# sahhermans/vae-diffusion-toy-crystals

Measured on NVIDIA B200. Metric: samples_per_sec_64x64_sde300_cfg1.5, higher is better.
Workload: dtype bf16

## Files before the change

include/tcs.h:

```cpp
#ifndef TCS_H_
#define TCS_H_

#include <stdint.h>

#ifdef __cplusplus
extern "C" {
#endif

typedef struct tcs_handle tcs_handle;

enum tcs_status {
  TCS_OK = 0,
  TCS_ERR_BAD_ARGUMENT = -1,
  TCS_ERR_UNSUPPORTED = -2,
  TCS_ERR_CUDA = -3,
  TCS_ERR_STATE = -4
};

enum tcs_precision { TCS_FP32 = 0, TCS_BF16 = 1 };
enum tcs_engine { TCS_ENGINE_AUTO = 0, TCS_ENGINE_SIMT = 1, TCS_ENGINE_TCGEN05 = 2 };
enum tcs_sampler { TCS_SAMPLER_ODE = 0, TCS_SAMPLER_SDE = 1 };

typedef struct tcs_config {
  int32_t n_types;
// ... 2 lines not shown
  int32_t emb_dim;
  int32_t cond_ch;
  int32_t time_ch;
  double beta_min;
  double beta_max;
  int32_t precision;
  int32_t engine;
  int32_t device;
  int32_t chunk;
  int32_t use_graph;
  int32_t fuse_gn;
} tcs_config;

void tcs_default_config(tcs_config* cfg);

int tcs_create(tcs_handle** out, const tcs_config* cfg);
void tcs_destroy(tcs_handle* h);

int tcs_set_weight(tcs_handle* h, const char* key, const float* data, const int64_t* shape, int32_t ndim);

int tcs_finalize_weights(tcs_handle* h);

int tcs_score(tcs_handle* h, const float* x, const float* t, const int64_t* y_cat, const float* y_cont,
              int32_t n, float guidance, float* eps_out, void* stream);

typedef struct tcs_sample_args {
  int32_t sampler;
  int32_t n;
  int32_t steps;
  float guidance;
  double t_end;
  const int64_t* y_cat;
  const float* y_cont;
  const float* x_init;
  const float* noise;
  uint64_t seed;
  uint64_t global_index_offset;
  float* x_out;
  float* trace_eps;
  float* trace_x;
  float* x0_hat;
  double beta_min;
  double beta_max;
} tcs_sample_args;

int tcs_sample(tcs_handle* h, const tcs_sample_args* args, void* stream);

int32_t tcs_nfe(int32_t sampler, int32_t steps);

int tcs_condition_grid(tcs_handle* h, int32_t n, int64_t offset, int64_t n_total, float theta_max,
                       int64_t* y_cat, float* y_cont, void* stream);

int tcs_sde_update(tcs_handle* h, float* x, const float* eps, const float* noise, int32_t n, float t, float t_next,
                   uint64_t seed, uint64_t global_index_offset, int32_t step, void* stream);

int tcs_ode_update(tcs_handle* h, int32_t mode, float* x, float* x_pred, float* d0, const float* eps, int32_t n,
                   float t, float t_next, void* stream);

int tcs_time_grid_host(int32_t steps, double t_end, float* ts_host);
int tcs_schedule_host(double beta_min, double beta_max, float t, float* beta, float* alpha, float* sigma);

int32_t tcs_check(tcs_handle* h);
int32_t tcs_launch_mode(const tcs_handle* h);

int64_t tcs_launch_count(const tcs_handle* h);
const char* tcs_build_info(void);
const char* tcs_last_error(void);

int64_t tcs_debug_layer(tcs_handle* h, const char* name, const float* x, const float* t, const int64_t* y_cat,
                        const float* y_cont, int32_t n, int32_t uncond, float* out, int64_t out_capacity,
                        void* stream);

int tcs_score_profiled(tcs_handle* h, const float* x, const float* t, const int64_t* y_cat, const float* y_cont,
                       int32_t n, float guidance, float* eps_out, float* conv_ms_host, float* total_ms_host,
                       void* stream);

int tcs_debug_conv(int32_t engine, int32_t precision, int32_t B, int32_t H_out, int32_t W_out, int32_t cin0,
                   int32_t cin1, int32_t cout, int32_t ksize, int32_t stride, const float* in0, const float* in1,
                   const float* weight, const float* bias, float* out, float* stats, int32_t epi, void* stream);

int tcs_debug_conv_ups(int32_t B, int32_t H_out, int32_t W_out, int32_t cin, int32_t cout, const float* in_lowres,
                       const float* weight, const float* bias, float* out, void* stream);

int64_t tcs_debug_attn_pack(const float* qkv_w, const float* proj_w, uint8_t* out, int64_t capacity);

int tcs_debug_attn_block(int32_t B, const float* x, const float* gn_w, const float* gn_b, const float* qkv_w,
                         const float* qkv_b, const float* proj_w, const float* proj_b, float* out, float* dbg,
                         void* stream);

#ifdef __cplusplus
}
#endif
#endif
```

vae-diffusion-toy-crystals_b200/csrc/common.cuh:

```cuda
#pragma once
#include <cuda.h>
#include <cuda_bf16.h>
#include <cuda_fp16.h>
#include <cuda_runtime.h>
#include <stdint.h>

#include <string>
#include <vector>

#include "../../include/tcs.h"

namespace tcs {

constexpr int IMG = 64;
constexpr int IMG_PIX = IMG * IMG;
constexpr int GN_GROUPS = 8;
constexpr float GN_EPS = 1e-5f;
constexpr int N_HEADS = 4;

void set_error(const std::string& msg);
int fail(int code, const std::string& msg);

#define TCS_CUDA(expr)                                                                          \
  do {                                                                                          \
    cudaError_t _e = (expr);                                                                    \
    if (_e != cudaSuccess)                                                                      \
      return ::tcs::fail(TCS_ERR_CUDA, std::string(#expr) + ": " + cudaGetErrorString(_e));     \
  } while (0)

#define TCS_CHECK(expr)                    \
  do {                                     \
    int _s = (expr);                       \
    if (_s != TCS_OK) return _s;           \
  } while (0)

enum Epilogue : int {
  EPI_RAW_STATS = 0,
  EPI_PADDED = 1,
  EPI_PLAIN = 2,
  EPI_GN_FUSED = 3,
  EPI_EPS = 4
};

struct ConvGeom {
  int B;
  int H, W;
  int ksize;
  int stride;
  int nsrc;
  int csrc[2];
  int in_pad[2];
  int ntot;
  int split3 = 0;
  int ups = 0;
  int kx_in_n = 0;
};

struct EpiArgs {
  const float* bias;
  void* out;
  float* partials;
  const void* residual;
  int ldo;
  int slots;
  const float* gamma;
  const float* beta;
  int* overflow;
};

struct DevBuf {
  void* p = nullptr;
  size_t bytes = 0;
  uint64_t* gen = nullptr;
  DevBuf() = default;
  DevBuf(const DevBuf&) = delete;
  DevBuf& operator=(const DevBuf&) = delete;
  ~DevBuf() { if (p) cudaFree(p); }
  int ensure(size_t b) {
    if (b <= bytes) return TCS_OK;
    if (p) cudaFree(p);
    p = nullptr; bytes = 0;
    TCS_CUDA(cudaMalloc(&p, b));
    bytes = b;
    if (gen) ++*gen;
    return TCS_OK;
  }
  template <typename U> U* as() const { return static_cast<U*>(p); }
};

struct HostTensor { std::vector<float> v; std::vector<int64_t> shape; };

inline int tc_slots(int H, int W) { return (H * W / 128) * 4; }
inline int simt_slots(int H, int W) { return H * W / 64; }

}
```

vae-diffusion-toy-crystals_b200/csrc/conv_tc.cu:

```cuda
#include "conv_tc.cuh"
#include "tc_ptx.cuh"

#include <cstdio>
#include <cstdlib>
#include <cstring>
#include <type_traits>
#include <vector>

#ifndef TCS_KERNEL_PROFILE
#define TCS_KERNEL_PROFILE 0
#endif

namespace tcs {


constexpr int EPI_WARPS = 16;
constexpr int GRP_WARPS = EPI_WARPS / 2;
constexpr int UC = 96;
constexpr int BLK = 32;
constexpr int TC_THREADS = 64 + 32 * EPI_WARPS + 32;
constexpr int UPS_EXTRA_THREADS = 4 * 32;
constexpr int MAX_STAGES = 12;
constexpr int MAX_A_STAGES = 4;
constexpr int KB = 64;
constexpr uint32_t ROWB = KB * 2;
constexpr int SLAB_BUFS = 2;
constexpr uint32_t EPI_WARP_SLAB = SLAB_BUFS * 32 * BLK * 2;
constexpr uint32_t EPI_SLAB_BYTES = EPI_WARPS * EPI_WARP_SLAB;
constexpr uint32_t EPI_BIAS_BYTES = 576 * 4;
constexpr size_t TC_SMEM_MAX = 227 * 1024 - 512;
__host__ __device__ constexpr uint32_t bias_bytes_of(int ntot) { return (static_cast<uint32_t>(ntot) * 4u + 127u) & ~127u; }
struct EpiGroupSmem {
  float scale[192], shift[192];
  float red[GRP_WARPS][16];
  float mean[8], rstd[8];
};
struct EpiFusedSmem {
  float gamma[192], beta[192];
  EpiGroupSmem grp[2];
};
constexpr uint32_t EPI_FUSED_BYTES = sizeof(EpiFusedSmem);
constexpr long long EXCHANGE_TIMEOUT_CYCLES = 1000000000LL;

__device__ __forceinline__ void st_relaxed_gpu_u64(unsigned long long* p, unsigned long long v) {
  asm volatile("st.relaxed.gpu.global.b64 [%0], %1;" ::"l"(p), "l"(v) : "memory");
}
__device__ __forceinline__ unsigned long long ld_relaxed_gpu_u64(const unsigned long long* p) {
  unsigned long long v;
  asm volatile("ld.relaxed.gpu.global.b64 %0, [%1];" : "=l"(v) : "l"(p) : "memory");
  return v;
}
__device__ __forceinline__ void epi_bar_sync(int grp) { asm volatile("bar.sync %0, %1;" ::"r"(1 + grp), "n"(32 * GRP_WARPS) : "memory"); }
__device__ __forceinline__ uint32_t pack_f16x2_sat(float a, float b) {
  uint32_t r;
  asm("cvt.rn.satfinite.f16x2.f32 %0, %1, %2;" : "=r"(r) : "f"(b), "f"(a));
  return r;
}
__device__ __forceinline__ float2 unpack_f16x2(uint32_t v) {
  return __half22float2(*reinterpret_cast<const __half2*>(&v));
}
__device__ __forceinline__ uint32_t pack_bf16x2(float a, float b) {
  const __nv_bfloat162 h = __floats2bfloat162_rn(a, b);
  return *reinterpret_cast<const uint32_t*>(&h);
}
__device__ __forceinline__ float silu_fast(float y) {
  const float h = 0.5f * y;
  float t;
  asm("tanh.approx.f32 %0, %1;" : "=f"(t) : "f"(h));
  return fmaf(h, t, h);
}
__device__ __forceinline__ void store_with_halo(__nv_bfloat16* obase, size_t pix, int wy, int wx, int Wp, int ldo,
                                                int ch, const uint32_t* pk);

__device__ __forceinline__ void fma2(float& d0, float& d1, float a0, float a1, float b0, float b1, float c0, float c1) {
  asm("{\n\t.reg .b64 ra, rb, rc, rd;\n\tmov.b64 ra, {%2, %3};\n\tmov.b64 rb, {%4, %5};\n\tmov.b64 rc, {%6, %7};\n\t"
      "fma.rn.f32x2 rd, ra, rb, rc;\n\tmov.b64 {%0, %1}, rd;\n\t}"
      : "=f"(d0), "=f"(d1) : "f"(a0), "f"(a1), "f"(b0), "f"(b1), "f"(c0), "f"(c1));
}
__device__ __forceinline__ void add2(float& d0, float& d1, float a0, float a1, float b0, float b1) {
  asm("{\n\t.reg .b64 ra, rb, rd;\n\tmov.b64 ra, {%2, %3};\n\tmov.b64 rb, {%4, %5};\n\t"
      "add.rn.f32x2 rd, ra, rb;\n\tmov.b64 {%0, %1}, rd;\n\t}"
      : "=f"(d0), "=f"(d1) : "f"(a0), "f"(a1), "f"(b0), "f"(b1));
}
__device__ __forceinline__ float tanh_fast(float x) {
#ifdef TCS_NO_TANH
  return x * 0.25f;
#else
  float t;
  asm("tanh.approx.f32 %0, %1;" : "=f"(t) : "f"(x));
  return t;
#endif
}
__device__ __forceinline__ void st_shared_u4(uint32_t addr, uint32_t a, uint32_t b, uint32_t c, uint32_t d) {
  asm volatile("st.shared.v4.b32 [%0], {%1, %2, %3, %4};" ::"r"(addr), "r"(a), "r"(b), "r"(c), "r"(d) : "memory");
}
__device__ __forceinline__ void ld_shared_u4(uint32_t addr, uint32_t& a, uint32_t& b, uint32_t& c, uint32_t& d) {
  asm volatile("ld.shared.v4.b32 {%0, %1, %2, %3}, [%4];" : "=r"(a), "=r"(b), "=r"(c), "=r"(d) : "r"(addr) : "memory");
}
__device__ __forceinline__ void tma_store_4d(const CUtensorMap* map, uint32_t src, int c0, int c1, int c2, int c3) {
  asm volatile("cp.async.bulk.tensor.4d.global.shared::cta.bulk_group [%0, {%2, %3, %4, %5}], [%1];"
               ::"l"(reinterpret_cast<uint64_t>(map)), "r"(src), "r"(c0), "r"(c1), "r"(c2), "r"(c3)
               : "memory");
}
template <int GEO = 0, int SB = SLAB_BUFS>
// ... 9 lines not shown
  long long c0 = tacc ? clock64() : 0;
  if (lane == 0) ptx::bulk_wait_read<SB - 1>();
  __syncwarp();
  if (tacc) { const long long c1 = clock64(); tacc[0] += c1 - c0; c0 = c1; }
  const uint32_t base = slab + (SB == 2 ? slab_buf * 2048 : 0);
  const uint32_t dst = base + lane * 64;
  const int sw = (lane >> 1) & 3;
#pragma unroll
  for (int j = 0; j < 4; ++j) st_shared_u4(dst + ((j ^ sw) << 4), pk[4 * j], pk[4 * j + 1], pk[4 * j + 2], pk[4 * j + 3]);
  ptx::fence_proxy_async();
  __syncwarp();
  if (tacc) { const long long c1 = clock64(); tacc[1] += c1 - c0; c0 = c1; }
  if (lane == 0) {
    if (GEO == 1) {
      tma_store_4d(mapO, base, ch, x + 1, y + 1, img);
      if (y == 0) tma_store_4d(mapO1, base, ch, x + 1, geo_H + 1, img);
      if (y + 4 == geo_H) tma_store_4d(mapO1, base + 3 * 512, ch, x + 1, 0, img);
    } else if (h16 == 0) {
      tma_store_4d(mapO, base, ch, x + 1, y + 1, img);
      if (wy) tma_store_4d(mapO, base, ch, x + 1, y + 1 + wy, img);
    } else {
      tma_store_4d(mapO, base, ch, 1, y + 1, img);
      tma_store_4d(mapO, base + 1024, ch, 1, y + 2, img);
      if (y == 0) tma_store_4d(mapO, base, ch, 1, h16 + 1, img);
      if (y + 1 == h16 - 1) tma_store_4d(mapO, base + 1024, ch, 1, 0, img);
    }
    ptx::bulk_commit();
  }
  __syncwarp();
  if (tacc) { const long long c1 = clock64(); tacc[2] += c1 - c0; c0 = c1; }
  slab_buf ^= 1;
  if (wx) {
    uint4* d0 = reinterpret_cast<uint4*>(obase + (pix + wx) * ldo + ch);
#pragma unroll
    for (int i = 0; i < 4; ++i) d0[i] = make_uint4(pk[4 * i], pk[4 * i + 1], pk[4 * i + 2], pk[4 * i + 3]);
    if (wy) {
      uint4* d1 = reinterpret_cast<uint4*>(obase + (pix + static_cast<long long>(wy) * Wp + wx) * ldo + ch);
#pragma unroll
      for (int i = 0; i < 4; ++i) d1[i] = make_uint4(pk[4 * i], pk[4 * i + 1], pk[4 * i + 2], pk[4 * i + 3]);
    }
  }
}

__device__ __forceinline__ void store_with_halo(__nv_bfloat16* obase, size_t pix, int wy, int wx, int Wp, int ldo,
                                                int ch, const uint32_t* pk) {
#pragma unroll
  for (int cy = 0; cy < 2; ++cy) {
    if (cy == 1 && wy == 0) continue;
#pragma unroll
    for (int cx = 0; cx < 2; ++cx) {
      if (cx == 1 && wx == 0) continue;
      const size_t dp = pix + static_cast<long long>(cy ? wy : 0) * Wp + (cx ? wx : 0);
      uint4* dst = reinterpret_cast<uint4*>(obase + dp * ldo + ch);
#pragma unroll
      for (int i = 0; i < BLK / 8; ++i) dst[i] = make_uint4(pk[4 * i], pk[4 * i + 1], pk[4 * i + 2], pk[4 * i + 3]);
    }
  }
}

template <int CG>
__device__ __forceinline__ void tile_to_mn(int tile, int n_ntiles, int& mt, int& nt) {
  if (CG == 2) {
    const int pt = tile >> 1;
    nt = pt % n_ntiles;
    mt = ((pt / n_ntiles) << 1) | (tile & 1);
  } else {
    mt = tile / n_ntiles;
    nt = tile - mt * n_ntiles;
  }
}

struct __align__(8) TcBarriers {
  uint64_t full[MAX_STAGES];
  uint64_t empty[MAX_STAGES];
  uint64_t fullA[MAX_A_STAGES];
  uint64_t emptyA[MAX_A_STAGES];
  uint64_t fullL[2];
  uint64_t emptyL[2];
  uint64_t tmem_full[2];
  uint64_t tmem_empty[2];
  uint32_t tmem_base;
};

template <int N, int EPI, int MSUB, int CG, int GEO, int UPS = 0>
__global__ void __launch_bounds__(TC_THREADS + UPS_EXTRA_THREADS * UPS, 1)
conv_tc_kernel(const __grid_constant__ CUtensorMap mapA0, const __grid_constant__ CUtensorMap mapA1,
               const __grid_constant__ CUtensorMap mapA2, const __grid_constant__ CUtensorMap mapA3,
               const __grid_constant__ CUtensorMap mapW, const __grid_constant__ CUtensorMap mapO,
               const __grid_constant__ CUtensorMap mapO1, const ConvTcParams p) {
  static_assert(GEO == 0 || (EPI != EPI_EPS && EPI != EPI_PLAIN), "tap-shift geometry: padded / fp32 outputs only");
  static_assert(UPS == 0 || (GEO == 1 && CG == 2 && EPI == EPI_PADDED), "fused upsample: tap-shift CTA pairs, padded output");
  constexpr int ACC_STRIDE = (N * MSUB <= 128) ? 128 : 256;
  static_assert(N * MSUB <= 256, "accumulator does not fit a double-buffered TMEM stage");

  extern __shared__ uint8_t smem_raw[];
  __shared__ TcBarriers bars;

  const int warp = __shfl_sync(0xffffffffu, threadIdx.x >> 5, 0);
  const int lane = threadIdx.x & 31;
  const uint32_t smem_base = (ptx::smem_u32(smem_raw) + 1023u) & ~1023u;
  const int n_tiles = p.n_mtiles * p.n_ntiles;
  const uint32_t l_ring = smem_base + (GEO == 1 ? p.a_stages * p.a_bytes : 0u);
  const uint32_t b_ring = l_ring + (UPS ? p.l_stages * p.l_bytes : 0u);
  const uint32_t slab_base = b_ring + p.nstage * p.stage_bytes;
  constexpr int SB = UPS ? 1 : SLAB_BUFS;
  constexpr uint32_t WARP_SLAB = SB * 32 * BLK * 2, SLAB_BYTES = EPI_WARPS * WARP_SLAB;
  float* bias_s = reinterpret_cast<float*>(smem_raw + (slab_base - ptx::smem_u32(smem_raw)) + SLAB_BYTES);
  for (int i = threadIdx.x; i < p.ntot; i += blockDim.x) {
    float b = p.epi.bias[i];
    if constexpr (EPI == EPI_GN_FUSED) {
      constexpr int CPGN = N / 8;
      const int g0 = i - i % CPGN;
      float k = 0.f;
#pragma unroll
      for (int j = 0; j < CPGN; ++j) k += p.epi.bias[g0 + j];
      b -= k * (1.0f / CPGN);
    }
    bias_s[i] = b;
  }
  EpiFusedSmem* fs = reinterpret_cast<EpiFusedSmem*>(reinterpret_cast<uint8_t*>(bias_s) + (GEO == 1 ? bias_bytes_of(p.ntot) : EPI_BIAS_BYTES));
  if constexpr (EPI == EPI_GN_FUSED)
    for (int i = threadIdx.x; i < N; i += blockDim.x) { fs->gamma[i] = p.epi.gamma[i]; fs->beta[i] = p.epi.beta[i]; }

  if (warp == 0 && lane == 0) {
    ptx::prefetch_tmap(&mapA0);
    ptx::prefetch_tmap(&mapA1);
    if (p.nsrc > 2) { ptx::prefetch_tmap(&mapA2); ptx::prefetch_tmap(&mapA3); }
    ptx::prefetch_tmap(&mapW);
    if (EPI != EPI_EPS) ptx::prefetch_tmap(&mapO);
    if (GEO == 1) ptx::prefetch_tmap(&mapO1);
    for (int s = 0; s < p.nstage; ++s) {
      ptx::mbar_init(ptx::smem_u32(&bars.full[s]), 1);
      ptx::mbar_init(ptx::smem_u32(&bars.empty[s]), p.issuers);
    }
    if (GEO == 1)
      for (int s = 0; s < p.a_stages; ++s) {
        ptx::mbar_init(ptx::smem_u32(&bars.fullA[s]), UPS ? 4 * CG : 1);
        ptx::mbar_init(ptx::smem_u32(&bars.emptyA[s]), p.issuers);
      }
    if (UPS)
      for (int s = 0; s < p.l_stages; ++s) {
        ptx::mbar_init(ptx::smem_u32(&bars.fullL[s]), 1);
        ptx::mbar_init(ptx::smem_u32(&bars.emptyL[s]), 4);
      }
    for (int a = 0; a < 2; ++a) {
      ptx::mbar_init(ptx::smem_u32(&bars.tmem_full[a]), p.issuers);
      ptx::mbar_init(ptx::smem_u32(&bars.tmem_empty[a]), GRP_WARPS * CG);
    }
    ptx::fence_barrier_init();
  }
  const uint32_t cta_rank = (CG == 2) ? ptx::cluster_ctarank() : 0u;
  constexpr int NB = N / CG;
  if (warp == 1) {
    if (CG == 2) ptx::tmem_alloc_512_2sm(ptx::smem_u32(&bars.tmem_base));
    else ptx::tmem_alloc_512(ptx::smem_u32(&bars.tmem_base));
  }
  ptx::tc_fence_before();
  __syncthreads();
  if (CG == 2) ptx::cluster_sync_all();
  ptx::tc_fence_after();
  const uint32_t tmem_base = bars.tmem_base;

  if (warp == 0 && GEO == 1) {
    uint32_t sa = 0, pa = 0, sb = 0, pb = 0;
    const int b_stages_per_kx = 3 / p.tb;
    const int b_rows_full = 3 * NB / 4;
    for (int tile = blockIdx.x; tile < n_tiles; tile += gridDim.x) {
      int mt, nt;
      tile_to_mn<CG>(tile, p.n_ntiles, mt, nt);
      const int b = mt / p.tiles_per_img, t = mt - b * p.tiles_per_img;
      const int ty = t / p.tiles_x, tx = t - ty * p.tiles_x;
      int ks = 0;
      for (int src = 0; src < p.nsrc; ++src) {
        const int ms = p.msel[src];
        const CUtensorMap* mapA = ms == 0 ? &mapA0 : (ms == 1 ? &mapA1 : (ms == 2 ? &mapA2 : &mapA3));
        for (int cb = 0; cb < p.cblk[src]; ++cb) {
          if constexpr (UPS) {
            auto issue_low = [&](int tl, int cbx) {
              int mt2, nt2;
              tile_to_mn<CG>(tl, p.n_ntiles, mt2, nt2);
              const int b2 = mt2 / p.tiles_per_img, t2 = mt2 - b2 * p.tiles_per_img;
              const int ty2 = t2 / p.tiles_x, tx2 = t2 - ty2 * p.tiles_x;
              ptx::mbar_wait(ptx::smem_u32(&bars.emptyL[sa]), pa ^ 1);
              if (lane == 0) {
                const uint32_t full = ptx::smem_u32(&bars.fullL[sa]);
                ptx::mbar_expect_tx(full, p.l_load_bytes);
                ptx::tma_load_4d(l_ring + sa * p.l_bytes, mapA, full, cbx * KB, tx2 * 4 * MSUB + p.base_off[0], ty2 * 8 + p.base_off[0], b2);
              }
              __syncwarp();
              if (++sa == static_cast<uint32_t>(p.l_stages)) { sa = 0; pa ^= 1; }
            };
            if (tile == static_cast<int>(blockIdx.x) && cb == 0) issue_low(tile, 0);
            int ntile = tile, ncb = cb + 1;
            if (ncb == p.cblk[0]) { ncb = 0; ntile = tile + static_cast<int>(gridDim.x); }
            if (ntile < n_tiles) issue_low(ntile, ncb);
          } else {
          ptx::mbar_wait(ptx::smem_u32(&bars.emptyA[sa]), pa ^ 1);
          const bool stale = (p.debug & 8) && (pa || tile != static_cast<int>(blockIdx.x));
          if (lane == 0) {
            const uint32_t full = ptx::smem_u32(&bars.fullA[sa]);
            const uint32_t a_dst = smem_base + sa * p.a_bytes;
            if (stale) {
              if (CG == 1 || cta_rank == 0) ptx::mbar_arrive(full);
            } else if (CG == 2) {
              if (cta_rank == 0) ptx::mbar_expect_tx(full, 2 * p.a_load_bytes);
              ptx::tma_load_4d_2sm(a_dst, mapA, full, cb * KB, tx * 8 * MSUB + p.base_off[src], ty * 16 + p.base_off[src], b);
            } else {
              ptx::mbar_expect_tx(full, p.a_load_bytes);
              ptx::tma_load_4d(a_dst, mapA, full, cb * KB, tx * 8 * MSUB + p.base_off[src], ty * 16 + p.base_off[src], b);
            }
          }
          __syncwarp();
          if (++sa == static_cast<uint32_t>(p.a_stages)) { sa = 0; pa ^= 1; }
          }
          for (int kx = 0; kx < 3; ++kx, ++ks)
            for (int jb = 0; jb < b_stages_per_kx; ++jb) {
              ptx::mbar_wait(ptx::smem_u32(&bars.empty[sb]), pb ^ 1);
              const bool stale_b = (p.debug & 8) && (pb || tile != static_cast<int>(blockIdx.x));
              if (lane == 0) {
                const uint32_t full = ptx::smem_u32(&bars.full[sb]);
                const uint32_t b_dst = b_ring + sb * p.stage_bytes;
                const int row0 = ((ks * p.n_ntiles + nt) * CG + static_cast<int>(cta_rank)) * b_rows_full + jb * p.b_rows;
                if (stale_b) {
                  if (CG == 1 || cta_rank == 0) ptx::mbar_arrive(full);
                } else if (CG == 2) {
                  if (cta_rank == 0) ptx::mbar_expect_tx(full, 2 * p.tb * NB * ROWB);
                  ptx::tma_load_2d_2sm(b_dst, &mapW, full, 0, row0);
                } else {
                  ptx::mbar_expect_tx(full, p.tb * NB * ROWB);
                  ptx::tma_load_2d(b_dst, &mapW, full, 0, row0);
                }
              }
              __syncwarp();
              if (++sb == static_cast<uint32_t>(p.nstage)) { sb = 0; pb ^= 1; }
            }
        }
      }
    }
  } else if (warp == 0) {
    uint32_t stage = 0, phase = 0;
    for (int tile = blockIdx.x; tile < n_tiles; tile += gridDim.x) {
      int mt, nt;
      tile_to_mn<CG>(tile, p.n_ntiles, mt, nt);
      const int rows_per_tile = p.pair ? p.Rt : p.Rt * MSUB;
      const int b = (mt / p.tiles_per_img) * (p.pair ? 2 : 1);
      const int y0 = (mt % p.tiles_per_img) * rows_per_tile;
      int ks = 0;
      for (int src = 0; src < p.nsrc; ++src) {
        const int ms = p.msel[src];
        const CUtensorMap* mapA = ms == 0 ? &mapA0 : (ms == 1 ? &mapA1 : (ms == 2 ? &mapA2 : &mapA3));
        for (int cb = 0; cb < p.cblk[src]; ++cb)
          for (int kyg = 0; kyg < p.KYG; ++kyg)
            for (int kx = 0; kx < p.KW; ++kx, ++ks) {
              ptx::mbar_wait(ptx::smem_u32(&bars.empty[stage]), phase ^ 1);
              if ((p.debug & 8) && (phase || tile != static_cast<int>(blockIdx.x))) {
                if (lane == 0 && (CG == 1 || cta_rank == 0)) ptx::mbar_arrive(ptx::smem_u32(&bars.full[stage]));
                __syncwarp();
                if (++stage == static_cast<uint32_t>(p.nstage)) { stage = 0; phase ^= 1; }
                continue;
              }
              if (lane == 0) {
                const uint32_t full = ptx::smem_u32(&bars.full[stage]);
                const uint32_t a_dst = smem_base + stage * p.stage_bytes;
                const uint32_t b_dst = a_dst + p.a_bytes;
                if (CG == 2) {
                  if (cta_rank == 0) ptx::mbar_expect_tx(full, 2 * (p.a_bytes + p.T * NB * ROWB));
                  ptx::tma_load_4d_2sm(a_dst, mapA, full, cb * KB, kx + p.kxn + p.base_off[src],
                                       p.stride * y0 + kyg + p.base_off[src], b);
                  if (p.pair)
                    ptx::tma_load_4d_2sm(a_dst + p.a_bytes / 2, mapA, full, cb * KB, kx + p.kxn + p.base_off[src],
                                         p.stride * y0 + kyg + p.base_off[src], b + 1);
                  ptx::tma_load_2d_2sm(b_dst, &mapW, full, 0,
                                       ((ks * p.n_ntiles + nt) * 2 + static_cast<int>(cta_rank)) * p.b_rows);
                } else {
                  ptx::mbar_expect_tx(full, p.a_bytes + p.T * N * ROWB);
                  ptx::tma_load_4d(a_dst, mapA, full, cb * KB, kx + p.kxn + p.base_off[src],
                                   p.stride * y0 + kyg + p.base_off[src], b);
                  if (p.pair)
                    ptx::tma_load_4d(a_dst + p.a_bytes / 2, mapA, full, cb * KB, kx + p.kxn + p.base_off[src],
                                     p.stride * y0 + kyg + p.base_off[src], b + 1);
                  ptx::tma_load_2d(b_dst, &mapW, full, 0, (ks * p.n_ntiles + nt) * p.b_rows);
                }
              }
              __syncwarp();
              if (++stage == static_cast<uint32_t>(p.nstage)) { stage = 0; phase ^= 1; }
            }
      }
    }
  } else if ((warp == 1 || (warp == 2 + EPI_WARPS && p.issuers == 2)) && cta_rank == 0) {
    constexpr uint32_t idesc = make_idesc(128 * CG, N);
    if constexpr (GEO == 1) {
      auto run1 = [&](auto sub_lo_c, auto sub_hi_c) {
        constexpr int SUB_LO = decltype(sub_lo_c)::value, SUB_HI = decltype(sub_hi_c)::value;
        uint32_t sa = 0, pa = 0, sb = 0, pb = 0, acc = 0, acc_phase = 0;
        const int b_stages_per_kx = 3 / p.tb;
        const uint32_t ky_inc = static_cast<uint32_t>(p.P) * (ROWB >> 4);
        int nblk = 0;
        for (int src = 0; src < p.nsrc; ++src) nblk += p.cblk[src];
        for (int tile = blockIdx.x; tile < n_tiles; tile += gridDim.x) {
          ptx::mbar_wait(ptx::smem_u32(&bars.tmem_empty[acc]), acc_phase ^ 1);
          ptx::tc_fence_after();
          const uint32_t d_tmem = tmem_base + acc * ACC_STRIDE;
          int blk = 0;
          for (int src = 0; src < p.nsrc; ++src)
            for (int cb = 0; cb < p.cblk[src]; ++cb, ++blk) {
              const int ksteps = (cb == p.cblk[src] - 1 && p.ctail[src]) ? 2 : 4;
              if (UPS) ptx::mbar_wait_cluster(ptx::smem_u32(&bars.fullA[sa]), pa);
              else ptx::mbar_wait(ptx::smem_u32(&bars.fullA[sa]), pa);
              const uint64_t adesc = make_desc_sw128_sbo(smem_base + sa * p.a_bytes, static_cast<uint32_t>(p.P) * ROWB) +
                                     static_cast<uint64_t>(SUB_LO * 8 * (ROWB >> 4));
              for (int kx = 0; kx < 3; ++kx)
                for (int jb = 0; jb < b_stages_per_kx; ++jb) {
                  ptx::mbar_wait(ptx::smem_u32(&bars.full[sb]), pb);
                  ptx::tc_fence_after();
                  if (lane == 0) {
                    uint64_t bdj = make_desc_sw128(b_ring + sb * p.stage_bytes);
                    uint64_t adj = adesc + static_cast<uint64_t>(kx * (ROWB >> 4) + jb * p.tb * ky_inc);
                    for (int j = 0; j < p.tb; ++j) {
                      uint64_t ad = adj;
#pragma unroll
                      for (int sub = SUB_LO; sub < SUB_HI; ++sub) {
                        const uint32_t first = (blk | kx | jb | j) != 0 ? 1u : 0u;
                        if (CG == 2) {
                          ptx::umma_bf16_2sm(d_tmem + sub * N, ad, bdj, idesc, first);
                          ptx::umma_bf16_2sm(d_tmem + sub * N, ad + 2, bdj + 2, idesc, 1u);
                          if (ksteps == 4) {
                            ptx::umma_bf16_2sm(d_tmem + sub * N, ad + 4, bdj + 4, idesc, 1u);
                            ptx::umma_bf16_2sm(d_tmem + sub * N, ad + 6, bdj + 6, idesc, 1u);
                          }
                        } else {
                          ptx::umma_bf16(d_tmem + sub * N, ad, bdj, idesc, first);
                          ptx::umma_bf16(d_tmem + sub * N, ad + 2, bdj + 2, idesc, 1u);
                          if (ksteps == 4) {
                            ptx::umma_bf16(d_tmem + sub * N, ad + 4, bdj + 4, idesc, 1u);
                            ptx::umma_bf16(d_tmem + sub * N, ad + 6, bdj + 6, idesc, 1u);
                          }
                        }
                        ad += 8 * (ROWB >> 4);
                      }
                      adj += ky_inc;
                      bdj += (NB * ROWB) >> 4;
                    }
                    const bool last_of_blk = kx == 2 && jb == b_stages_per_kx - 1;
                    if (CG == 2) {
                      ptx::umma_commit_2sm(ptx::smem_u32(&bars.empty[sb]));
                      if (last_of_blk) ptx::umma_commit_2sm(ptx::smem_u32(&bars.emptyA[sa]));
                      if (last_of_blk && blk == nblk - 1) ptx::umma_commit_2sm(ptx::smem_u32(&bars.tmem_full[acc]));
                    } else {
                      ptx::umma_commit(ptx::smem_u32(&bars.empty[sb]));
                      if (last_of_blk) ptx::umma_commit(ptx::smem_u32(&bars.emptyA[sa]));
                      if (last_of_blk && blk == nblk - 1) ptx::umma_commit(ptx::smem_u32(&bars.tmem_full[acc]));
                    }
                  }
                  __syncwarp();
                  if (++sb == static_cast<uint32_t>(p.nstage)) { sb = 0; pb ^= 1; }
                }
              if (++sa == static_cast<uint32_t>(p.a_stages)) { sa = 0; pa ^= 1; }
            }
          if (++acc == 2) { acc = 0; acc_phase ^= 1; }
        }
      };
      using J0 = std::integral_constant<int, 0>;
      using J1 = std::integral_constant<int, 1>;
      using JM = std::integral_constant<int, MSUB>;
      using JL = std::integral_constant<int, MSUB - 1>;
      if (p.issuers == 2) {
        if (warp == 1) run1(J0{}, J1{});
        else run1(JL{}, JM{});
      } else {
        run1(J0{}, JM{});
      }
    } else {
    const uint32_t row_shift = p.W * ROWB;
    const uint32_t sub_stride = p.pair ? p.a_bytes / 2 : p.Rt * row_shift;
    const uint32_t a_inc_j = row_shift >> 4, a_inc_sub = sub_stride >> 4;
    auto run = [&](auto sub_lo_c, auto sub_hi_c) {
      constexpr int SUB_LO = decltype(sub_lo_c)::value, SUB_HI = decltype(sub_hi_c)::value;
      uint32_t stage = 0, phase = 0, acc = 0, acc_phase = 0;
      const bool prof = TCS_KERNEL_PROFILE && (p.debug & 128) && blockIdx.x == 0 && warp == 1;
      long long w_empty = 0, w_full = 0, t_begin = prof ? clock64() : 0;
      int ntile = 0;
      const int stages_per_cb = p.KYG * p.KW;
      for (int tile = blockIdx.x; tile < n_tiles; tile += gridDim.x) {
        long long c0 = prof ? clock64() : 0;
        ptx::mbar_wait(ptx::smem_u32(&bars.tmem_empty[acc]), acc_phase ^ 1);
        ptx::tc_fence_after();
        if (prof) { w_empty += clock64() - c0; ++ntile; }
        int ks = 0;
        for (int src = 0; src < p.nsrc; ++src)
          for (int cb = 0; cb < p.cblk[src]; ++cb) {
// ... 55 lines not shown
    using I0 = std::integral_constant<int, 0>;
    using I1 = std::integral_constant<int, 1>;
    using IM = std::integral_constant<int, MSUB>;
    using IL = std::integral_constant<int, MSUB - 1>;
    if (p.issuers == 2) {
      if (warp == 1) run(I0{}, I1{});
      else run(IL{}, IM{});
    } else {
      run(I0{}, IM{});
    }
    }
  } else if (UPS && warp >= 3 + EPI_WARPS) {
    if constexpr (UPS) {
      constexpr int P = 8 * MSUB + 2, CW = P / 2, LP = CW + 1;
      const int t128 = (warp - (3 + EPI_WARPS)) * 32 + lane;
      uint32_t sa = 0, pa = 0, sl = 0, pl = 0;
      auto blend_cell = [&](uint32_t lbase, uint32_t abase, uint32_t k, int cm, int cn, float wy0, float wy1, float wx0, float wx1) {
        const uint32_t pa = lbase + (cm * LP + cn) * 128 + (k << 4);
        uint32_t a[4], bq[4], c[4], d[4];
        ld_shared_u4(pa, a[0], a[1], a[2], a[3]);
        ld_shared_u4(pa + 128, bq[0], bq[1], bq[2], bq[3]);
        ld_shared_u4(pa + LP * 128, c[0], c[1], c[2], c[3]);
        ld_shared_u4(pa + LP * 128 + 128, d[0], d[1], d[2], d[3]);
        uint32_t o00[4], o01[4], o10[4], o11[4];
#pragma unroll
        for (int w = 0; w < 4; ++w) {
          const float al = __uint_as_float(a[w] << 16), ah = __uint_as_float(a[w] & 0xffff0000u);
          const float bl = __uint_as_float(bq[w] << 16), bh = __uint_as_float(bq[w] & 0xffff0000u);
          const float cl = __uint_as_float(c[w] << 16), ch = __uint_as_float(c[w] & 0xffff0000u);
          const float dl = __uint_as_float(d[w] << 16), dh = __uint_as_float(d[w] & 0xffff0000u);
          float el, eh, fl, fh, t0l, t0h, t1l, t1h, u0l, u0h, u1l, u1h, gl, gh, hl, hh, r0, r1;
          add2(el, eh, bl, bh, -al, -ah);
          add2(fl, fh, dl, dh, -cl, -ch);
          fma2(t0l, t0h, wx0, wx0, el, eh, al, ah);
          fma2(t1l, t1h, wx1, wx1, el, eh, al, ah);
          fma2(u0l, u0h, wx0, wx0, fl, fh, cl, ch);
          fma2(u1l, u1h, wx1, wx1, fl, fh, cl, ch);
          add2(gl, gh, u0l, u0h, -t0l, -t0h);
          add2(hl, hh, u1l, u1h, -t1l, -t1h);
          fma2(r0, r1, wy0, wy0, gl, gh, t0l, t0h); o00[w] = pack_bf16x2(r0, r1);
          fma2(r0, r1, wy0, wy0, hl, hh, t1l, t1h); o01[w] = pack_bf16x2(r0, r1);
          fma2(r0, r1, wy1, wy1, gl, gh, t0l, t0h); o10[w] = pack_bf16x2(r0, r1);
          fma2(r0, r1, wy1, wy1, hl, hh, t1l, t1h); o11[w] = pack_bf16x2(r0, r1);
        }
        const uint32_t q00 = (2 * cm) * P + 2 * cn, q01 = q00 + 1, q10 = q00 + P, q11 = q10 + 1;
        st_shared_u4(abase + q00 * 128 + ((k ^ (q00 & 7)) << 4), o00[0], o00[1], o00[2], o00[3]);
        st_shared_u4(abase + q01 * 128 + ((k ^ (q01 & 7)) << 4), o01[0], o01[1], o01[2], o01[3]);
        st_shared_u4(abase + q10 * 128 + ((k ^ (q10 & 7)) << 4), o10[0], o10[1], o10[2], o10[3]);
        st_shared_u4(abase + q11 * 128 + ((k ^ (q11 & 7)) << 4), o11[0], o11[1], o11[2], o11[3]);
      };
      for (int tile = blockIdx.x; tile < n_tiles; tile += gridDim.x) {
        int mt, nt;
        tile_to_mn<CG>(tile, p.n_ntiles, mt, nt);
        const int t = mt % p.tiles_per_img;
        const int ty = t / p.tiles_x, tx = t - ty * p.tiles_x;
        const int edge_r0 = ty == 0 ? 0 : -1, edge_r1 = ty == p.H / 16 - 1 ? 8 : -1;
        const int edge_c0 = tx == 0 ? 0 : -1, edge_c1 = tx == p.tiles_x - 1 ? CW - 1 : -1;
        for (int src = 0; src < p.nsrc; ++src)
          for (int cb = 0; cb < p.cblk[src]; ++cb) {
            const bool tail = cb == p.cblk[src] - 1 && p.ctail[src];
            ptx::mbar_wait_sleep(ptx::smem_u32(&bars.fullL[sl]), pl);
            ptx::mbar_wait_sleep(ptx::smem_u32(&bars.emptyA[sa]), pa ^ 1);
            const uint32_t lbase = l_ring + sl * p.l_bytes, abase = smem_base + sa * p.a_bytes;
            if (!(p.debug & 64)) {
              const uint32_t k = tail ? (t128 & 3) : (t128 & 7);
              const int slot = tail ? (t128 >> 2) : (t128 >> 3), nslot = tail ? 32 : 16;
              for (int ci = slot; ci < 9 * CW; ci += nslot) {
                const int cm = ci / CW, cn = ci - cm * CW;
                const bool ey = cm == edge_r0 || cm == edge_r1, ex = cn == edge_c0 || cn == edge_c1;
                blend_cell(lbase, abase, k, cm, cn, ey ? 0.f : 0.25f, ey ? 1.f : 0.75f, ex ? 0.f : 0.25f, ex ? 1.f : 0.75f);
              }
            }
            ptx::fence_proxy_async();
            __syncwarp();
            if (lane == 0) {
              ptx::mbar_arrive(ptx::smem_u32(&bars.emptyL[sl]));
              ptx::mbar_arrive_release_rank0(ptx::smem_u32(&bars.fullA[sa]));
            }
            if (++sl == static_cast<uint32_t>(p.l_stages)) { sl = 0; pl ^= 1; }
            if (++sa == static_cast<uint32_t>(p.a_stages)) { sa = 0; pa ^= 1; }
          }
      }
    }
  } else if (warp >= 2 && warp < 2 + EPI_WARPS) {
    const int e = warp - 2, grp = e / GRP_WARPS, ew = e % GRP_WARPS, q = warp & 3, h = ew >> 2;
    const int row = q * 32 + lane;
    const int HW = p.H * p.W;
    const int Wp = p.W + 2, Hp = p.H + 2;
    (void)Hp; (void)Wp; (void)HW;
    const uint32_t acc = grp;
    uint32_t acc_phase = 0, slab_buf = 0;
    (void)slab_buf;
    EpiGroupSmem* gsm = &fs->grp[grp];
    (void)gsm;
    const uint32_t slab = slab_base + static_cast<uint32_t>(e) * WARP_SLAB;
    const bool use_tma_out = !(p.debug & 4);
    const int h16 = p.W == 16 ? p.H : 0;
    (void)h16;
    (void)use_tma_out; (void)slab;
    const int sub = (MSUB == 2) ? h : 0;
    const int col0 = (MSUB == 2) ? 0 : h * UC;
    auto pixel_of = [&](int mt_, int& img_, int& y_, int& x_) {
      if (GEO == 1) {
        img_ = mt_ / p.tiles_per_img;
        const int t_ = mt_ - img_ * p.tiles_per_img;
        const int ty_ = t_ / p.tiles_x, tx_ = t_ - ty_ * p.tiles_x;
        y_ = ty_ * 16 + (row >> 3);
        x_ = (tx_ * MSUB + sub) * 8 + (row & 7);
      } else {
        const int m_ = (mt_ * MSUB + sub) * 128 + row;
        img_ = m_ / HW;
        const int rem_ = m_ - img_ * HW;
        y_ = rem_ / p.W;
        x_ = rem_ - y_ * p.W;
      }
    };
    uint32_t it = 0;
    const bool prof = TCS_KERNEL_PROFILE && (p.debug & 128) && blockIdx.x == 0 && e == 0;
    long long pw_full = 0, p_ld = 0, p_a = 0, p_b = 0, p_c = 0, pc0 = 0, pc1 = 0, q_post = 0, q_poll = 0, q_npoll = 0, r_math = 0;
    (void)p_ld;
    long long tacc[3] = {0, 0, 0};
    auto release_tmem = [&]() {
      ptx::tc_fence_before();
      __syncwarp();
      if (lane == 0) {
        if (CG == 2) ptx::mbar_arrive_rank0(ptx::smem_u32(&bars.tmem_empty[acc]));
        else ptx::mbar_arrive(ptx::smem_u32(&bars.tmem_empty[acc]));
      }
    };
    for (int tile = blockIdx.x + grp * gridDim.x; tile < n_tiles; tile += 2 * gridDim.x, acc_phase ^= 1, ++it) {
      int mt, nt;
      tile_to_mn<CG>(tile, p.n_ntiles, mt, nt);
      const uint32_t tbase = tmem_base + (static_cast<uint32_t>(q * 32) << 16) + acc * ACC_STRIDE;
      const uint32_t taddr = tbase + h * UC;
      if (prof) { pc1 = clock64(); if (it) p_c += pc1 - pc0; pc0 = pc1; }
      ptx::mbar_wait(ptx::smem_u32(&bars.tmem_full[acc]), acc_phase);
      ptx::tc_fence_after();
      if (prof) { pc1 = clock64(); pw_full += pc1 - pc0; pc0 = pc1; }
      if (p.debug & 16) { release_tmem(); continue; }

      if constexpr (EPI == EPI_EPS) {
        float e0 = 0.f, e1 = 0.f;
        if (h == 0) {
          if (p.kxn) {
            float a0[4], a1[4];
            ptx::tmem_ld4(tbase, a0);
            ptx::tmem_ld4(tbase + N, a1);
            ptx::tmem_ld_wait();
            release_tmem();
            float* xch = reinterpret_cast<float*>(fs) + grp * 32;
            const int qq = q;
            if (lane == 31) { xch[qq * 4 + 0] = a0[0]; xch[qq * 4 + 1] = a1[0]; }
            if (lane == 0) { xch[qq * 4 + 2] = a0[2]; xch[qq * 4 + 3] = a1[2]; }
            asm volatile("bar.sync %0, 128;" ::"r"(3 + grp) : "memory");
            float l0 = __shfl_up_sync(0xffffffffu, a0[0], 1), l1 = __shfl_up_sync(0xffffffffu, a1[0], 1);
            float r0 = __shfl_down_sync(0xffffffffu, a0[2], 1), r1 = __shfl_down_sync(0xffffffffu, a1[2], 1);
            const int pq = qq ^ 1;
            if (lane == 0) { l0 = xch[pq * 4 + 0]; l1 = xch[pq * 4 + 1]; }
            if (lane == 31) { r0 = xch[pq * 4 + 2]; r1 = xch[pq * 4 + 3]; }
            e0 = (l0 + a0[1]) + r0;
            e1 = (l1 + a1[1]) + r1;
            asm volatile("bar.sync %0, 128;" ::"r"(3 + grp) : "memory");
          } else {
            ptx::tmem_ld1(tbase, &e0);
            ptx::tmem_ld1(tbase + N, &e1);
            ptx::tmem_ld_wait();
// ... 401 lines not shown

typedef CUresult (*PFN_encodeTiled)(CUtensorMap*, CUtensorMapDataType, cuuint32_t, void*, const cuuint64_t*,
                                    const cuuint64_t*, const cuuint32_t*, const cuuint32_t*, CUtensorMapInterleave,
                                    CUtensorMapSwizzle, CUtensorMapL2promotion, CUtensorMapFloatOOBfill);

static PFN_encodeTiled get_encode() {
  static PFN_encodeTiled fn = nullptr;
  if (!fn) {
    void* p = nullptr;
    cudaDriverEntryPointQueryResult q;
    if (cudaGetDriverEntryPoint("cuTensorMapEncodeTiled", &p, cudaEnableDefault, &q) == cudaSuccess &&
        q == cudaDriverEntryPointSuccess)
      fn = reinterpret_cast<PFN_encodeTiled>(p);
  }
  return fn;
}

int conv_tc_make_pair(ConvTcPlan* pl, const void* src, int B) {
  ConvTcParams& p = pl->p;
  if (pl->epi != EPI_EPS || pl->msub != 2 || B % 2) return fail(TCS_ERR_BAD_ARGUMENT, "conv_tc_make_pair: needs the eps plan and an even batch");
  PFN_encodeTiled encode = get_encode();
  p.pair = 1;
  p.WR = p.Rt + p.T - 1;
  p.tiles_per_img = p.H / p.Rt;
  p.n_mtiles = (B / 2) * p.tiles_per_img;
  p.a_bytes = 2u * static_cast<uint32_t>(p.WR) * p.W * ROWB;
  p.stage_bytes = (p.a_bytes + p.T * (pl->N / pl->cg) * ROWB + 1023u) & ~1023u;
  const size_t budget = 227 * 1024 - 2048 - 1024 - EPI_SLAB_BYTES - EPI_BIAS_BYTES - EPI_FUSED_BYTES;
  p.nstage = static_cast<int>(budget / p.stage_bytes);
  if (p.nstage > MAX_STAGES) p.nstage = MAX_STAGES;
  pl->smem = static_cast<size_t>(p.nstage) * p.stage_bytes + 1024 + EPI_SLAB_BYTES + EPI_BIAS_BYTES + EPI_FUSED_BYTES;
  const cuuint64_t C = static_cast<cuuint64_t>(pl->cin[0]);
  const int Hin = p.H + 2, Win = p.W + 2;
  cuuint64_t dims[4] = {C, static_cast<cuuint64_t>(Win), static_cast<cuuint64_t>(Hin), static_cast<cuuint64_t>(B)};
  cuuint64_t strides[3] = {C * 2, C * 2 * Win, C * 2 * Win * Hin};
  cuuint32_t box[4] = {KB, static_cast<cuuint32_t>(p.W), static_cast<cuuint32_t>(p.WR), 1};
  cuuint32_t estr[4] = {1, 1, 1, 1};
  CUresult r = encode(&pl->mapA[0], CU_TENSOR_MAP_DATA_TYPE_BFLOAT16, 4, const_cast<void*>(src), dims, strides, box, estr,
                      CU_TENSOR_MAP_INTERLEAVE_NONE, CU_TENSOR_MAP_SWIZZLE_128B, CU_TENSOR_MAP_L2_PROMOTION_L2_256B,
                      CU_TENSOR_MAP_FLOAT_OOB_FILL_NONE);
  if (r != CUDA_SUCCESS) return fail(TCS_ERR_CUDA, "cuTensorMapEncodeTiled(A pair) failed: " + std::to_string(r));
  for (int i = 1; i < 4; ++i) pl->mapA[i] = pl->mapA[0];
  return TCS_OK;
}

int conv_tc_grid(const ConvTcPlan& pl, int B, int sm_count) {
  const int tiles = (pl.p.pair ? B / 2 : B) * pl.p.tiles_per_img * pl.p.n_ntiles;
  int grid = tiles < sm_count ? tiles : sm_count;
  if (pl.max_ctas > 0 && grid > pl.max_ctas) grid = pl.max_ctas;
  static const bool group_grid = getenv("TCS_GN_GROUP_GRID") && atoi(getenv("TCS_GN_GROUP_GRID")) == 1;
  if (pl.epi == EPI_GN_FUSED && (group_grid || grid < pl.p.tiles_per_img * 2))
    grid = grid / pl.p.tiles_per_img * pl.p.tiles_per_img;
  if (pl.cg == 2) grid &= ~1;
  return grid;
}

__global__ void coop_cluster_probe_kernel() {}
static bool coop_cluster_supported() {
  static int state = -1;
  if (state < 0) {
    cudaLaunchConfig_t cfg{};
    cfg.gridDim = dim3(2); cfg.blockDim = dim3(32); cfg.dynamicSmemBytes = 0; cfg.stream = nullptr;
    cudaLaunchAttribute at[2];
    at[0].id = cudaLaunchAttributeCooperative; at[0].val.cooperative = 1;
    at[1].id = cudaLaunchAttributeClusterDimension;
    at[1].val.clusterDim.x = 2; at[1].val.clusterDim.y = 1; at[1].val.clusterDim.z = 1;
    cfg.attrs = at; cfg.numAttrs = 2;
    cudaStreamCaptureStatus cs = cudaStreamCaptureStatusNone;
    if (cudaStreamIsCapturing(nullptr, &cs) != cudaSuccess || cs != cudaStreamCaptureStatusNone) { cudaGetLastError(); return false; }
    const cudaError_t e = cudaLaunchKernelEx(&cfg, coop_cluster_probe_kernel);
    cudaGetLastError();
    state = (e == cudaSuccess && cudaDeviceSynchronize() == cudaSuccess) ? 1 : 0;
    if (getenv("TCS_NO_COOP_CLUSTER")) state = 0;
  }
  return state == 1;
}

static int conv_tc_geo(const ConvGeom& g, int epi) {
  const char* e = getenv("TCS_GEO");
  if (e && atoi(e) == 0) return 0;
  return (g.ksize == 3 && g.stride == 1 && !g.kx_in_n && epi != EPI_EPS && epi != EPI_PLAIN && g.H % 16 == 0) ? 1 : 0;
}

template <int N, int EPI, int MSUB, int CG, int GEO, int UPS = 0>
static int set_smem_attr() {
  static bool attr_done = false;
  if (!attr_done) {
    TCS_CUDA(cudaFuncSetAttribute(conv_tc_kernel<N, EPI, MSUB, CG, GEO, UPS>, cudaFuncAttributeMaxDynamicSharedMemorySize, static_cast<int>(TC_SMEM_MAX)));
    attr_done = true;
  }
  return TCS_OK;
}

template <int N, int EPI, int MSUB, int CG, int GEO, int UPS = 0>
static int max_ctas_t(const ConvTcPlan& pl, int* out) {
  TCS_CHECK((set_smem_attr<N, EPI, MSUB, CG, GEO, UPS>()));
  auto kern = conv_tc_kernel<N, EPI, MSUB, CG, GEO, UPS>;
  if (CG == 2) {
    cudaLaunchConfig_t cfg{};
    cfg.gridDim = dim3(2); cfg.blockDim = dim3(TC_THREADS + UPS_EXTRA_THREADS * UPS); cfg.dynamicSmemBytes = pl.smem; cfg.stream = nullptr;
    cudaLaunchAttribute at[1];
    at[0].id = cudaLaunchAttributeClusterDimension;
    at[0].val.clusterDim.x = 2; at[0].val.clusterDim.y = 1; at[0].val.clusterDim.z = 1;
    cfg.attrs = at; cfg.numAttrs = 1;
    int nclusters = 0;
    TCS_CUDA(cudaOccupancyMaxActiveClusters(&nclusters, kern, &cfg));
    *out = 2 * nclusters;
  } else {
    int per_sm = 0, dev = 0, sms = 0;
    TCS_CUDA(cudaOccupancyMaxActiveBlocksPerMultiprocessor(&per_sm, kern, TC_THREADS, pl.smem));
    TCS_CUDA(cudaGetDevice(&dev));
    TCS_CUDA(cudaDeviceGetAttribute(&sms, cudaDevAttrMultiProcessorCount, dev));
    *out = per_sm * sms;
  }
  return TCS_OK;
}

template <int N, int EPI, int MSUB, int CG, int GEO, int UPS = 0>
static int launch_t(const ConvTcPlan& pl, cudaStream_t st) {
  auto kern = conv_tc_kernel<N, EPI, MSUB, CG, GEO, UPS>;
  TCS_CHECK((set_smem_attr<N, EPI, MSUB, CG, GEO, UPS>()));
  if (EPI == EPI_GN_FUSED)
    TCS_CUDA(cudaMemsetAsync(pl.p.epi.partials, 0, sizeof(unsigned long long) * 16 * pl.p.n_mtiles, st));
  cudaLaunchConfig_t cfg{};
  cfg.gridDim = dim3(pl.grid); cfg.blockDim = dim3(TC_THREADS + UPS_EXTRA_THREADS * UPS); cfg.dynamicSmemBytes = pl.smem; cfg.stream = st;
  cudaLaunchAttribute at[2];
  int na = 0;
  if (EPI == EPI_GN_FUSED && (CG == 1 || pl.coop_cluster)) {
    at[na].id = cudaLaunchAttributeCooperative;
    at[na].val.cooperative = 1;
    ++na;
  }
  if (CG == 2) {
    at[na].id = cudaLaunchAttributeClusterDimension;
    at[na].val.clusterDim.x = 2; at[na].val.clusterDim.y = 1; at[na].val.clusterDim.z = 1;
    ++na;
  }
  cfg.attrs = at; cfg.numAttrs = na;
  TCS_CUDA(cudaLaunchKernelEx(&cfg, kern, pl.mapA[0], pl.mapA[1], pl.mapA[2], pl.mapA[3], pl.mapW, pl.mapO, pl.mapO1, pl.p));
  TCS_CUDA(cudaGetLastError());
  return TCS_OK;
}

static int conv_tc_max_ctas(const ConvTcPlan& pl, int* out) {
#define TCS_TC_CASE(NN, EE, MM)                                                        \
  if (pl.geo == 0 && pl.N == NN && pl.epi == EE && pl.msub == MM) {                     \
    if (pl.cg == 2) { if constexpr (NN >= 96 || EE == EPI_EPS) return max_ctas_t<NN, EE, MM, 2, 0>(pl, out); } \
    else return max_ctas_t<NN, EE, MM, 1, 0>(pl, out);                                  \
  }
#define TCS_TC_GEO1(NN, EE, MM)                                                        \
  if (pl.geo == 1 && pl.cg == 2 && !pl.ups && pl.N == NN && pl.epi == EE && pl.msub == MM) return max_ctas_t<NN, EE, MM, 2, 1>(pl, out);
  if (pl.geo == 1 && pl.cg == 2 && pl.ups && pl.epi == EPI_PADDED && pl.N == 96 && pl.msub == 2) return max_ctas_t<96, EPI_PADDED, 2, 2, 1, 1>(pl, out);
  if (pl.geo == 1 && pl.cg == 2 && pl.ups && pl.epi == EPI_PADDED && pl.N == 192 && pl.msub == 1) return max_ctas_t<192, EPI_PADDED, 1, 2, 1, 1>(pl, out);
  TCS_TC_CASE(96, EPI_RAW_STATS, 2)
  TCS_TC_CASE(96, EPI_PADDED, 2)
  TCS_TC_CASE(96, EPI_PLAIN, 2)
  TCS_TC_CASE(96, EPI_GN_FUSED, 2)
  TCS_TC_CASE(192, EPI_RAW_STATS, 1)
  TCS_TC_CASE(192, EPI_PADDED, 1)
  TCS_TC_CASE(192, EPI_PLAIN, 1)
  TCS_TC_CASE(192, EPI_GN_FUSED, 1)
  TCS_TC_CASE(16, EPI_EPS, 2)
  TCS_TC_GEO1(96, EPI_RAW_STATS, 2)
  TCS_TC_GEO1(96, EPI_PADDED, 2)
  TCS_TC_GEO1(96, EPI_GN_FUSED, 2)
  TCS_TC_GEO1(192, EPI_RAW_STATS, 1)
  TCS_TC_GEO1(192, EPI_PADDED, 1)
  TCS_TC_GEO1(192, EPI_GN_FUSED, 1)
#undef TCS_TC_CASE
#undef TCS_TC_GEO1
  return fail(TCS_ERR_UNSUPPORTED, "conv_tc: no kernel instance for this (N, epilogue, msub)");
}

int conv_tc_launch(const ConvTcPlan& pl, cudaStream_t st) {
  if (!pl.valid) return fail(TCS_ERR_STATE, "conv_tc_launch: plan not built");
#define TCS_TC_CASE(NN, EE, MM)                                                        \
  if (pl.geo == 0 && pl.N == NN && pl.epi == EE && pl.msub == MM) {                     \
    if (pl.cg == 2) { if constexpr (NN >= 96 || EE == EPI_EPS) return launch_t<NN, EE, MM, 2, 0>(pl, st); } \
    else return launch_t<NN, EE, MM, 1, 0>(pl, st);                                     \
  }
#define TCS_TC_GEO1(NN, EE, MM)                                                        \
  if (pl.geo == 1 && pl.cg == 2 && !pl.ups && pl.N == NN && pl.epi == EE && pl.msub == MM) return launch_t<NN, EE, MM, 2, 1>(pl, st);
  if (pl.geo == 1 && pl.cg == 2 && pl.ups && pl.epi == EPI_PADDED && pl.N == 96 && pl.msub == 2) return launch_t<96, EPI_PADDED, 2, 2, 1, 1>(pl, st);
  if (pl.geo == 1 && pl.cg == 2 && pl.ups && pl.epi == EPI_PADDED && pl.N == 192 && pl.msub == 1) return launch_t<192, EPI_PADDED, 1, 2, 1, 1>(pl, st);
  TCS_TC_CASE(96, EPI_RAW_STATS, 2)
  TCS_TC_CASE(96, EPI_PADDED, 2)
  TCS_TC_CASE(96, EPI_PLAIN, 2)
  TCS_TC_CASE(96, EPI_GN_FUSED, 2)
  TCS_TC_CASE(192, EPI_RAW_STATS, 1)
  TCS_TC_CASE(192, EPI_PADDED, 1)
  TCS_TC_CASE(192, EPI_PLAIN, 1)
  TCS_TC_CASE(192, EPI_GN_FUSED, 1)
  TCS_TC_CASE(16, EPI_EPS, 2)
  TCS_TC_GEO1(96, EPI_RAW_STATS, 2)
  TCS_TC_GEO1(96, EPI_PADDED, 2)
  TCS_TC_GEO1(96, EPI_GN_FUSED, 2)
  TCS_TC_GEO1(192, EPI_RAW_STATS, 1)
  TCS_TC_GEO1(192, EPI_PADDED, 1)
  TCS_TC_GEO1(192, EPI_GN_FUSED, 1)
#undef TCS_TC_CASE
#undef TCS_TC_GEO1
  return fail(TCS_ERR_UNSUPPORTED, "conv_tc_launch: no kernel instance for this (N, epilogue, msub)");
}

int conv_tc_make_plan(ConvTcPlan* plan, const ConvGeom& g, const void* src0, const void* src1,
                      const __nv_bfloat16* wpacked, int epi, const EpiArgs& ea, int sm_count, const void* lo0,
                      const void* lo1) {
  PFN_encodeTiled encode = get_encode();
  if (!encode) return fail(TCS_ERR_CUDA, "cuTensorMapEncodeTiled entry point not available");
  if (g.W != 64 && g.W != 32 && g.W != 16) return fail(TCS_ERR_UNSUPPORTED, "conv_tc: output width must be 64/32/16");
  if ((g.H * g.W) % 128) return fail(TCS_ERR_UNSUPPORTED, "conv_tc: image must be a multiple of 128 pixels");
  ConvTcPlan& pl = *plan;
  pl = ConvTcPlan();
  ConvTcParams& p = pl.p;
  conv_tc_tile_shape(g, epi, &pl.N, &pl.cg);
  if (g.ntot % pl.N) return fail(TCS_ERR_UNSUPPORTED, "conv_tc: C_out must be a multiple of 96");
  pl.epi = epi;
  pl.msub = pl.N == 192 ? 1 : 2;
  if (epi == EPI_EPS && pl.cg == 2 && (g.B * (g.H / (2 * (128 / g.W)))) % 2)
    return fail(TCS_ERR_UNSUPPORTED, "conv_tc: the output conv runs as CTA pairs and needs an even number of tiles");
  if (g.H % (pl.msub * (128 / g.W))) return fail(TCS_ERR_UNSUPPORTED, "conv_tc: image height not a multiple of the tile");
  p.debug = getenv("TCS_DEBUG") ? atoi(getenv("TCS_DEBUG")) : 0;
  p.gn_inv_cnt = 1.0 / (static_cast<double>(g.H) * g.W * (pl.N / 8));
  p.exch_timeout = getenv("TCS_EXCHANGE_TIMEOUT") ? atoll(getenv("TCS_EXCHANGE_TIMEOUT")) : EXCHANGE_TIMEOUT_CYCLES;
  {
    const char* e = getenv("TCS_ISSUERS");
    p.issuers = (pl.msub == 2 && !(e && atoi(e) == 1)) ? 2 : 1;
  }
  stage_shape(g, &p.T, &p.KYG, &p.KW);
  p.H = g.H; p.W = g.W; p.Rt = 128 / g.W;
  p.stride = g.stride;
  p.pair = 0;
  p.kxn = g.kx_in_n ? 1 : 0;
  p.guidance = 0.f;
  p.WR = p.Rt * pl.msub + p.T - 1;
  p.nsrc = g.nsrc * (g.split3 ? 3 : 1);
  pl.cin[0] = g.csrc[0]; pl.cin[1] = g.csrc[g.nsrc > 1 ? 1 : 0];
  if (g.split3 && (!lo0 || (g.nsrc == 2 && !lo1))) return fail(TCS_ERR_BAD_ARGUMENT, "conv_tc: bf16x3 mode needs the lo parts of its sources");
  if (g.split3 && epi != EPI_RAW_STATS) return fail(TCS_ERR_UNSUPPORTED, "conv_tc: bf16x3 mode writes fp32 (EPI_RAW_STATS) only");
  p.ntot = g.ntot;
  p.tiles_per_img = g.H / (p.Rt * pl.msub);
  p.n_mtiles = g.B * p.tiles_per_img;
  p.n_ntiles = g.ntot / pl.N;
  p.kstages = conv_tc_kstages(g);
  p.a_bytes = static_cast<uint32_t>(p.WR) * g.W * ROWB;
  p.stage_bytes = (p.a_bytes + p.T * (pl.N / pl.cg) * ROWB + 1023u) & ~1023u;
  const size_t budget = 227 * 1024 - 2048 - 1024 - EPI_SLAB_BYTES - EPI_BIAS_BYTES - EPI_FUSED_BYTES;
  p.nstage = static_cast<int>(budget / p.stage_bytes);
  if (p.nstage > MAX_STAGES) p.nstage = MAX_STAGES;
  pl.geo = (pl.cg == 2) ? conv_tc_geo(g, epi) : 0;
  if (!pl.geo && p.nstage < 2) return fail(TCS_ERR_UNSUPPORTED, "conv_tc: stage does not fit shared memory twice");
  pl.smem = static_cast<size_t>(p.nstage) * p.stage_bytes + 1024 + EPI_SLAB_BYTES + EPI_BIAS_BYTES + EPI_FUSED_BYTES;
  p.geo = pl.geo;
  p.P = p.tiles_x = p.a_stages = p.tb = 0;
  p.a_load_bytes = 0;
  p.ups = p.l_stages = 0;
  p.l_bytes = p.l_load_bytes = 0;
  if (pl.geo) {
    if (g.W % (8 * pl.msub) || g.H % 16) return fail(TCS_ERR_UNSUPPORTED, "conv_tc: image is not a multiple of the 16 x 8 tile");
    const int NB = pl.N / pl.cg;
    p.P = 8 * pl.msub + 2;
    p.tiles_x = g.W / (8 * pl.msub);
    p.WR = 18;
    p.tiles_per_img = (g.H / 16) * p.tiles_x;
    p.n_mtiles = g.B * p.tiles_per_img;
    p.a_load_bytes = static_cast<uint32_t>(p.WR) * p.P * ROWB;
    p.a_bytes = (p.a_load_bytes + 1023u) & ~1023u;
    p.a_stages = 2;
    if (g.ups) {
      p.ups = pl.ups = 1;
      p.l_stages = 2;
      p.l_load_bytes = 10u * static_cast<uint32_t>(p.P / 2 + 1) * ROWB;
      p.l_bytes = (p.l_load_bytes + 1023u) & ~1023u;
    }
    const size_t slab_bytes = g.ups ? EPI_SLAB_BYTES / SLAB_BUFS : EPI_SLAB_BYTES;
    const size_t budget1 = TC_SMEM_MAX - 1024 - slab_bytes - bias_bytes_of(g.ntot) - EPI_FUSED_BYTES -
                           static_cast<size_t>(p.l_stages) * p.l_bytes;
    const bool want3 = getenv("TCS_UPS_A_STAGES") ? atoi(getenv("TCS_UPS_A_STAGES")) == 3 : pl.msub == 2;
    if (g.ups && want3 && budget1 >= 3 * static_cast<size_t>(p.a_bytes) + 2 * static_cast<size_t>(3u * NB * ROWB))
      p.a_stages = 3;
    const size_t rest = budget1 - static_cast<size_t>(p.a_stages) * p.a_bytes;
    p.tb = (rest / (3u * NB * ROWB) >= (g.ups ? 2u : 3u)) ? 3 : 1;
    if (getenv("TCS_TB")) p.tb = atoi(getenv("TCS_TB")) == 3 ? 3 : 1;
    p.stage_bytes = (static_cast<uint32_t>(p.tb) * NB * ROWB + 1023u) & ~1023u;
    p.nstage = static_cast<int>(rest / p.stage_bytes);
    if (p.nstage > MAX_STAGES) p.nstage = MAX_STAGES;
    if (getenv("TCS_NSTAGE") && atoi(getenv("TCS_NSTAGE")) < p.nstage) p.nstage = atoi(getenv("TCS_NSTAGE"));
    if (getenv("TCS_PLAN_LOG")) fprintf(stderr, "[conv_tc plan] H=%d N=%d K=%d ups=%d tb=%d nstage=%d stage_bytes=%u a_bytes=%u l_bytes=%u\n", g.H, pl.N, p.kstages, p.ups, p.tb, p.nstage, p.stage_bytes, p.a_bytes, p.l_bytes);
    if (p.nstage < 2) return fail(TCS_ERR_UNSUPPORTED, "conv_tc: weight stage does not fit shared memory twice");
    pl.smem = static_cast<size_t>(p.a_stages) * p.a_bytes + static_cast<size_t>(p.l_stages) * p.l_bytes +
              static_cast<size_t>(p.nstage) * p.stage_bytes + 1024 + slab_bytes + bias_bytes_of(g.ntot) + EPI_FUSED_BYTES;
  }
  if (g.ups && !(pl.geo == 1 && pl.cg == 2 && epi == EPI_PADDED && g.nsrc == 1 && !g.split3))
    return fail(TCS_ERR_UNSUPPORTED, "conv_tc: the fused upsample needs a 3x3 stride-1 layer with one padded bf16 source and a padded output");
  p.epi = ea;
  TCS_CHECK(conv_tc_max_ctas(pl, &pl.max_ctas));
  if (getenv("TCS_MAX_CTAS")) pl.max_ctas = atoi(getenv("TCS_MAX_CTAS"));
  pl.coop_cluster = pl.cg == 2 && epi == EPI_GN_FUSED && coop_cluster_supported();
  pl.grid = conv_tc_grid(pl, g.B, sm_count);
  if (epi == EPI_GN_FUSED && (p.n_ntiles != 1 || pl.grid < p.tiles_per_img))
    return fail(TCS_ERR_UNSUPPORTED,
                "conv_tc: fused GroupNorm needs one N tile and a whole image group (" + std::to_string(p.tiles_per_img) +
                    " CTAs) resident at once; the device can hold " + std::to_string(pl.max_ctas));

  const void* srcs[4] = {src0, src1, src0, src1};
  int lsrc[4] = {0, 1, 0, 1};
  if (g.split3) {
    srcs[0] = src0; srcs[1] = lo0; srcs[2] = src1; srcs[3] = lo1;
    lsrc[0] = lsrc[1] = 0; lsrc[2] = lsrc[3] = 1;
  }
  for (int ps = 0; ps < 6; ++ps) {
    const int ls = g.split3 ? ps / 3 : ps;
    const int li = ls < g.nsrc ? ls : 0;
    const int conv_pad = (g.ksize == 1) ? 0 : 1;
    p.base_off[ps] = g.in_pad[li] - conv_pad;
    if (p.base_off[ps] < 0) return fail(TCS_ERR_BAD_ARGUMENT, "conv_tc: a 3x3/4x4 conv needs a padded source");
    p.cblk[ps] = (g.csrc[li] + KB - 1) / KB;
    p.ctail[ps] = (g.csrc[li] % KB) ? 1 : 0;
    if (g.csrc[li] % 32) return fail(TCS_ERR_UNSUPPORTED, "conv_tc: source channels must be a multiple of 32");
    p.msel[ps] = g.split3 ? 2 * li + (ps % 3 == 2 ? 1 : 0) : li;
  }
  for (int s = 0; s < 4; ++s) {
    int si = lsrc[s] < g.nsrc ? lsrc[s] : 0;
    if (!srcs[s] || lsrc[s] >= g.nsrc) { srcs[s] = srcs[0]; si = 0; }
    const int pad = g.in_pad[si];
    const int Hin = g.H * g.stride + 2 * pad, Win = g.W * g.stride + 2 * pad;
    const cuuint64_t C = g.csrc[si];
    cuuint64_t dims[4] = {C, static_cast<cuuint64_t>(Win), static_cast<cuuint64_t>(Hin), static_cast<cuuint64_t>(g.B)};
    cuuint64_t strides[3] = {C * 2, C * 2 * Win, C * 2 * Win * Hin};
    cuuint32_t box[4] = {KB, static_cast<cuuint32_t>(g.W * g.stride), static_cast<cuuint32_t>(p.WR * g.stride), 1};
    cuuint32_t estr[4] = {1, static_cast<cuuint32_t>(g.stride), static_cast<cuuint32_t>(g.stride), 1};
    if (pl.geo) { box[1] = static_cast<cuuint32_t>(p.P); box[2] = static_cast<cuuint32_t>(p.WR); }
    if (pl.ups) {
      dims[1] = static_cast<cuuint64_t>(g.W / 2 + 2); dims[2] = static_cast<cuuint64_t>(g.H / 2 + 2);
      strides[1] = C * 2 * dims[1]; strides[2] = strides[1] * dims[2];
      box[1] = static_cast<cuuint32_t>(p.P / 2 + 1); box[2] = 10;
    }
    CUresult r = encode(&pl.mapA[s], CU_TENSOR_MAP_DATA_TYPE_BFLOAT16, 4, const_cast<void*>(srcs[s]), dims, strides,
                        box, estr, CU_TENSOR_MAP_INTERLEAVE_NONE, pl.ups ? CU_TENSOR_MAP_SWIZZLE_NONE : CU_TENSOR_MAP_SWIZZLE_128B,
                        CU_TENSOR_MAP_L2_PROMOTION_L2_256B, CU_TENSOR_MAP_FLOAT_OOB_FILL_NONE);
    if (r != CUDA_SUCCESS) return fail(TCS_ERR_CUDA, "cuTensorMapEncodeTiled(A) failed: " + std::to_string(r));
  }
  {
    const uint32_t stage_b = static_cast<uint32_t>(p.T) * (pl.N / pl.cg) * ROWB;
    if (stage_b % 512) return fail(TCS_ERR_UNSUPPORTED, "conv_tc: weight stage is not a multiple of 512 bytes");
    p.b_rows = static_cast<int>(stage_b / 512);
    const cuuint64_t total_rows = static_cast<cuuint64_t>(p.kstages) * p.n_ntiles * pl.cg * p.b_rows;
    if (pl.geo) p.b_rows = p.b_rows * p.tb / 3;
    cuuint64_t dims[2] = {256, total_rows};
    cuuint64_t strides[1] = {512};
    cuuint32_t box[2] = {256, static_cast<cuuint32_t>(p.b_rows)};
    cuuint32_t estr[2] = {1, 1};
    CUresult r = encode(&pl.mapW, CU_TENSOR_MAP_DATA_TYPE_BFLOAT16, 2, const_cast<__nv_bfloat16*>(wpacked), dims,
                        strides, box, estr, CU_TENSOR_MAP_INTERLEAVE_NONE, CU_TENSOR_MAP_SWIZZLE_NONE,
                        CU_TENSOR_MAP_L2_PROMOTION_L2_256B, CU_TENSOR_MAP_FLOAT_OOB_FILL_NONE);
    if (r != CUDA_SUCCESS) return fail(TCS_ERR_CUDA, "cuTensorMapEncodeTiled(W) failed: " + std::to_string(r));
  }
  pl.mapO = pl.mapW;
  pl.mapO1 = pl.mapW;
  if (epi == EPI_PLAIN) {
    const cuuint64_t C = static_cast<cuuint64_t>(ea.ldo);
    cuuint64_t dims[2] = {C, static_cast<cuuint64_t>(g.B) * g.H * g.W};
    cuuint64_t strides[1] = {C * 2};
    cuuint32_t box[2] = {BLK, 32};
    cuuint32_t estr[2] = {1, 1};
    CUresult r = encode(&pl.mapO, CU_TENSOR_MAP_DATA_TYPE_BFLOAT16, 2, ea.out, dims, strides, box, estr,
                        CU_TENSOR_MAP_INTERLEAVE_NONE, CU_TENSOR_MAP_SWIZZLE_64B, CU_TENSOR_MAP_L2_PROMOTION_L2_256B,
                        CU_TENSOR_MAP_FLOAT_OOB_FILL_NONE);
    if (r != CUDA_SUCCESS) return fail(TCS_ERR_CUDA, "cuTensorMapEncodeTiled(O plain) failed: " + std::to_string(r));
  }
  if (epi == EPI_GN_FUSED || epi == EPI_PADDED) {
    const cuuint64_t C = static_cast<cuuint64_t>(ea.ldo);
    cuuint64_t dims[4] = {C, static_cast<cuuint64_t>(g.W + 2), static_cast<cuuint64_t>(g.H + 2), static_cast<cuuint64_t>(g.B)};
    cuuint64_t strides[3] = {C * 2, C * 2 * (g.W + 2), C * 2 * (g.W + 2) * (g.H + 2)};
    cuuint32_t box[4] = {BLK, static_cast<cuuint32_t>(g.W >= 32 ? 32 : 16), 1, 1};
// ... 19 lines not shown
```

vae-diffusion-toy-crystals_b200/csrc/conv_tc.cuh:

```cuda
#pragma once
#include <vector>

#include "common.cuh"

namespace tcs {

struct ConvTcParams {
  int n_mtiles, n_ntiles;
  int tiles_per_img;
  int H, W;
  int Rt;
  int T, KYG, KW;
  int stride, WR;
  int nsrc, cblk[6], base_off[6];
  int msel[6];
  int ctail[6];
  int ntot;
  int kstages;
  int b_rows;
  int nstage;
  uint32_t a_bytes, stage_bytes;
  int pair;
  int kxn;
  float guidance;
  double gn_inv_cnt;
  long long exch_timeout;
  int issuers;
  int geo;
  int P;
  int tiles_x;
  int a_stages, tb;
  uint32_t a_load_bytes;
  int ups;
  int l_stages;
  uint32_t l_bytes, l_load_bytes;
  int debug;
  EpiArgs epi;
};

struct ConvTcPlan {
  CUtensorMap mapA[4];
  CUtensorMap mapW;
  CUtensorMap mapO;
  CUtensorMap mapO1;
  int geo = 0;
  int ups = 0;
  ConvTcParams p;
  int N;
  int epi;
  int msub;
  int cg;
  int grid;
  int cin[2] = {0, 0};
  int max_ctas = 0;
  bool coop_cluster = false;
  size_t smem;
  bool valid = false;
};

int conv_tc_kstages(const ConvGeom& g);
size_t conv_tc_packed_elems(const ConvGeom& g);
void conv_tc_pack_weights(const ConvGeom& g, int epi, const float* w, __nv_bfloat16* out_host);
void conv_tc_tile_shape(const ConvGeom& g, int epi, int* N, int* cg);

int conv_tc_make_plan(ConvTcPlan* plan, const ConvGeom& g, const void* src0, const void* src1,
                      const __nv_bfloat16* wpacked, int epi, const EpiArgs& ea, int sm_count,
                      const void* lo0 = nullptr, const void* lo1 = nullptr);
int conv_tc_launch(const ConvTcPlan& plan, cudaStream_t stream);
int conv_tc_make_pair(ConvTcPlan* plan, const void* src, int B);
int conv_tc_grid(const ConvTcPlan& plan, int B, int sm_count);

}
```

vae-diffusion-toy-crystals_b200/csrc/kernels.cuh:

```cuda
#pragma once
#include "common.cuh"

namespace tcs {

struct EmbedWeights {
  const float *cat_emb;
  const float *cm0_w, *cm0_b;
  const float *cm2_w, *cm2_b;
  const float *co_w, *co_b;
  const float *tm0_w, *tm0_b;
  const float *tm2_w, *tm2_b;
  const float *tc_w, *tc_b;
  const float *tt_w, *tt_b;
  const float *wsum;
  const float *b0;
  int n_types, y_cont_dim;
};
int launch_cond_embed(const EmbedWeights& w, const int64_t* y_cat, const float* y_cont, int n, int dup, float* cvec,
                      cudaStream_t st);
int launch_time_embed(const EmbedWeights& w, const float* t, int nt, float* tvec, cudaStream_t st);

int launch_first_conv(const float* x, const float* w9 , const float* tvec, int tvec_stride,
                      const int* step_ptr, int trow_off, const float* cvec, int n, int dup, float* raw,
                      float* partials, cudaStream_t st);
constexpr int FIRST_CONV_SLOTS = 32;
template <typename T>
int launch_first_conv_gn(const float* x, const float* w9, const float* tvec, int tvec_stride, const int* step_ptr,
                         int trow_off, const float* cvec, int n, int dup, const float* gamma, const float* beta, T* out,
                         cudaStream_t st);

template <typename T>
int launch_gn_apply(const void* in, int in_padded, const float* partials, int slots, const float* gamma,
                    const float* beta, int B, int H, int W, int C, int silu, T* out_padded, float2* stats_scratch ,
                    cudaStream_t st);
template <typename T>
int launch_gn_image16(const T* in_padded, int B, const float* gamma, const float* beta, T* out_padded, cudaStream_t st);
template <typename T>
int launch_gn_stats(const T* in_padded, int B, int H, int W, int C, float* partials, cudaStream_t st);

template <typename T>
int launch_upsample2x(const T* in, int B, int h, int w, int C, T* out, cudaStream_t st);

template <typename T>
int launch_attention(const T* qkv, int B, T* y, cudaStream_t st);

template <typename T>
int launch_conv_simt(const ConvGeom& g, const T* src0, const T* src1, const float* wpacked, int epi,
                     const EpiArgs& ea, cudaStream_t st);
void conv_simt_pack_weights(const ConvGeom& g, const float* w, float* out_host, bool round_bf16);

template <typename T>
int launch_out_conv(const T* act, const float* w , float bias, int n, int dup, float guidance,
                    float* eps, cudaStream_t st);

template <typename T>
int launch_pad_from_plain(const float* in, int B, int H, int W, int C, int pad, T* out, cudaStream_t st);
template <typename T>
int launch_unpad_to_f32(const T* in, int B, int H, int W, int C, int pad, float* out, cudaStream_t st);

int launch_split(const float* in, size_t elems, __nv_bfloat16* out, size_t lo_off, cudaStream_t st);
int launch_raw_to_padded(int mode, const float* raw, const float2* stats, const float* gamma, const float* beta,
                         const float* residual, int B, int H, int W, int C, void* out, size_t lo_off, cudaStream_t st);
int launch_unsplit_to_f32(const __nv_bfloat16* in, size_t lo_off, int B, int H, int W, int C, int pad, float* out,
                          cudaStream_t st);
int launch_gn_finalize(const float* partials, int slots, int B, int H, int W, int C, float2* stats, cudaStream_t st);

struct StepCoef {
  float t, beta, sigma, alpha, dt, g_sqrt_dt, pad0, pad1;
};
enum StepMode : int { STEP_SDE = 0, STEP_ODE_PREDICT = 1, STEP_ODE_CORRECT = 2, STEP_FINAL = 3 };
struct StepArgs {
  const StepCoef* coef;
  const int* step_ptr;
  int row_off;
  int mode;
  float* x;
  float* x_pred;
  float* d0;
  const float* eps;
  const float* noise;
  long long noise_step_stride;
  float* out_img;
  float* out_x0;
  unsigned long long seed, gidx0;
  int n;
};
int launch_step(const StepArgs& a, cudaStream_t st);
int launch_philox_normal(float* x, int n, unsigned long long seed, unsigned long long gidx0, cudaStream_t st);
int launch_advance(int* step_ptr, int delta, cudaStream_t st);
int launch_copy_f32(float* dst, const float* src, size_t n, cudaStream_t st);

}
```

vae-diffusion-toy-crystals_b200/csrc/kernels_simt.cu:

```cuda
#include "kernels.cuh"

#include <cstdlib>

namespace tcs {

template <typename T> struct Vec8;
template <> struct Vec8<float> {
  float4 a, b;
  __device__ __forceinline__ void load(const float* p) { a = *reinterpret_cast<const float4*>(p); b = *reinterpret_cast<const float4*>(p + 4); }
  __device__ __forceinline__ void store(float* p) const { *reinterpret_cast<float4*>(p) = a; *reinterpret_cast<float4*>(p + 4) = b; }
  __device__ __forceinline__ void get(float* f) const { f[0]=a.x; f[1]=a.y; f[2]=a.z; f[3]=a.w; f[4]=b.x; f[5]=b.y; f[6]=b.z; f[7]=b.w; }
  __device__ __forceinline__ void set(const float* f) { a = make_float4(f[0],f[1],f[2],f[3]); b = make_float4(f[4],f[5],f[6],f[7]); }
};
template <> struct Vec8<__nv_bfloat16> {
  uint4 u;
  __device__ __forceinline__ void load(const __nv_bfloat16* p) { u = *reinterpret_cast<const uint4*>(p); }
  __device__ __forceinline__ void store(__nv_bfloat16* p) const { *reinterpret_cast<uint4*>(p) = u; }
  __device__ __forceinline__ void get(float* f) const {
    const __nv_bfloat162* h = reinterpret_cast<const __nv_bfloat162*>(&u);
#pragma unroll
    for (int i = 0; i < 4; ++i) { const float2 t = __bfloat1622float2(h[i]); f[2*i] = t.x; f[2*i+1] = t.y; }
  }
  __device__ __forceinline__ void set(const float* f) {
    __nv_bfloat162* h = reinterpret_cast<__nv_bfloat162*>(&u);
// ... 4 lines not shown

template <typename T> __device__ __forceinline__ float to_f(T v);
template <> __device__ __forceinline__ float to_f<float>(float v) { return v; }
template <> __device__ __forceinline__ float to_f<__nv_bfloat16>(__nv_bfloat16 v) { return __bfloat162float(v); }
template <typename T> __device__ __forceinline__ T from_f(float v);
template <> __device__ __forceinline__ float from_f<float>(float v) { return v; }
template <> __device__ __forceinline__ __nv_bfloat16 from_f<__nv_bfloat16>(float v) { return __float2bfloat16(v); }

__device__ __forceinline__ int halo_wrap(int v, int n) { return v == 0 ? n : (v == n - 1 ? -n : 0); }

__global__ void __launch_bounds__(192) first_conv_kernel(const float* __restrict__ x, const float* __restrict__ w9,
                                                        const float* __restrict__ tvec, int tvec_stride,
                                                        const int* __restrict__ step_ptr, int trow_off,
                                                        const float* __restrict__ cvec, int dup,
                                                        float* __restrict__ raw, float* __restrict__ partials) {
  __shared__ float xs[4][IMG + 2];
  __shared__ float red[2][96][2][2];
  const int i = blockIdx.x >> 5, rp = blockIdx.x & 31, y0 = rp * 2;
  const int t = threadIdx.x, oc = t % 96, half = t / 96;
  for (int e = t; e < 4 * (IMG + 2); e += 192) {
    const int r = e / (IMG + 2), c = e % (IMG + 2);
    const int yy = (y0 - 1 + r + IMG) & (IMG - 1), xx = (c - 1 + IMG) & (IMG - 1);
    xs[r][c] = x[(static_cast<size_t>(i) * IMG + yy) * IMG + xx];
  }
  float w[9];
#pragma unroll
  for (int k = 0; k < 9; ++k) w[k] = w9[oc * 9 + k];
  const int trow = (step_ptr ? *step_ptr : 0) + trow_off + i * tvec_stride;
  const float tb = tvec[static_cast<size_t>(trow) * 96 + oc];
  float bias[2], s[2] = {0.f, 0.f}, q[2] = {0.f, 0.f};
  for (int u = 0; u < dup; ++u) bias[u] = tb + cvec[(static_cast<size_t>(i) * dup + u) * 96 + oc];
  __syncthreads();
  for (int p = half; p < 128; p += 2) {
    const int r = p >> 6, c = p & 63;
    float acc = 0.f;
#pragma unroll
    for (int ky = 0; ky < 3; ++ky)
#pragma unroll
      for (int kx = 0; kx < 3; ++kx) acc = fmaf(w[ky * 3 + kx], xs[r + ky][c + kx], acc);
    for (int u = 0; u < dup; ++u) {
      const float v = acc + bias[u];
      raw[((static_cast<size_t>(i) * dup + u) * IMG_PIX + (y0 + r) * IMG + c) * 96 + oc] = v;
      s[u] += v;
      q[u] += v * v;
    }
  }
  for (int u = 0; u < dup; ++u) { red[half][oc][u][0] = s[u]; red[half][oc][u][1] = q[u]; }
  __syncthreads();
  if (t < 8 * dup) {
    const int g = t % 8, u = t / 8;
    float ss = 0.f, qq = 0.f;
    for (int h = 0; h < 2; ++h)
      for (int c = 0; c < 12; ++c) { ss += red[h][g * 12 + c][u][0]; qq += red[h][g * 12 + c][u][1]; }
    float* dst = partials + ((static_cast<size_t>(i) * dup + u) * FIRST_CONV_SLOTS + rp) * 16 + 2 * g;
    dst[0] = ss;
    dst[1] = qq;
  }
}

int launch_first_conv(const float* x, const float* w9, const float* tvec, int tvec_stride, const int* step_ptr,
                      int trow_off, const float* cvec, int n, int dup, float* raw, float* partials,
                      cudaStream_t st) {
  if (n <= 0) return TCS_OK;
  first_conv_kernel<<<n * 32, 192, 0, st>>>(x, w9, tvec, tvec_stride, step_ptr, trow_off, cvec, dup, raw, partials);
  TCS_CUDA(cudaGetLastError());
  return TCS_OK;
}

template <bool FAST> __device__ __forceinline__ float silu_f(float v);

__device__ __forceinline__ float2 pk_fma2v(float2 a, float2 b, float2 c) {
  float2 d;
  asm("{\n\t.reg .b64 ra, rb, rc, rd;\n\tmov.b64 ra, {%2, %3};\n\tmov.b64 rb, {%4, %5};\n\tmov.b64 rc, {%6, %7};\n\t"
      "fma.rn.f32x2 rd, ra, rb, rc;\n\tmov.b64 {%0, %1}, rd;\n\t}"
      : "=f"(d.x), "=f"(d.y) : "f"(a.x), "f"(a.y), "f"(b.x), "f"(b.y), "f"(c.x), "f"(c.y));
  return d;
}
template <typename T> __device__ __forceinline__ void store_pair(T* p, float a, float b);
template <> __device__ __forceinline__ void store_pair<float>(float* p, float a, float b) { *reinterpret_cast<float2*>(p) = make_float2(a, b); }
template <> __device__ __forceinline__ void store_pair<__nv_bfloat16>(__nv_bfloat16* p, float a, float b) {
  *reinterpret_cast<__nv_bfloat162*>(p) = __floats2bfloat162_rn(a, b);
}

constexpr int FC_SPLIT = 2;
template <typename T>
__global__ void __launch_bounds__(384, 2) first_conv_gn_kernel(const float* __restrict__ x, const float* __restrict__ w9,
                                                           const float* __restrict__ tvec, int tvec_stride,
                                                           const int* __restrict__ step_ptr, int trow_off,
                                                           const float* __restrict__ cvec, int dup,
                                                           const float* __restrict__ gamma, const float* __restrict__ beta,
                                                           T* __restrict__ out) {
  constexpr bool FAST = sizeof(T) == 2;
  constexpr int P = IMG + 4;
  __shared__ float2 xs[P][P];
  __shared__ double racc[12][14];
  __shared__ double R[5][5];
  __shared__ double S1;
  __shared__ double csum[96][2][2];
  __shared__ float s_mean[2][GN_GROUPS], s_rstd[2][GN_GROUPS];
  const int i = blockIdx.x / FC_SPLIT, band = blockIdx.x % FC_SPLIT;
  const int t = threadIdx.x, op = t % 48, pg = t / 48, oc = 2 * op;
  const int warp = t >> 5, lane = t & 31;
  for (int e = t; e < P * P; e += 384) {
    const int r = e / P, c = e - r * P;
    const float xval = x[(static_cast<size_t>(i) * IMG + ((r - 2 + IMG) & (IMG - 1))) * IMG + ((c - 2 + IMG) & (IMG - 1))];
    xs[r][c] = make_float2(xval, xval);
  }
  __syncthreads();
  {
    double acc[14];
#pragma unroll
    for (int k = 0; k < 14; ++k) acc[k] = 0.0;
    for (int p = t; p < IMG_PIX; p += 384) {
      const int yy = (p >> 6) + 2, xx = (p & 63) + 2;
      const double x0 = xs[yy][xx].x;
      acc[13] += x0;
#pragma unroll
      for (int k = 0; k < 13; ++k) {
        const int dy = (k + 2) / 5, dx = (k + 2) % 5 - 2;
        acc[k] += x0 * static_cast<double>(xs[yy + dy][xx + dx].x);
      }
    }
#pragma unroll
    for (int k = 0; k < 14; ++k) {
#pragma unroll
      for (int o = 16; o > 0; o >>= 1) acc[k] += __shfl_xor_sync(0xffffffffu, acc[k], o);
      if (lane == 0) racc[warp][k] = acc[k];
    }
  }
  __syncthreads();
  if (t < 14) {
    double v = 0.0;
    for (int w = 0; w < 12; ++w) v += racc[w][t];
    if (t == 13) S1 = v;
    else {
      const int dy = (t + 2) / 5, dx = (t + 2) % 5 - 2;
      R[2 + dy][2 + dx] = v;
      R[2 - dy][2 - dx] = v;
    }
  }
  const int trow = (step_ptr ? *step_ptr : 0) + trow_off + i * tvec_stride;
  __syncthreads();
  if (t < 96) {
    double wk[9], A = 0.0, Q = 0.0;
#pragma unroll
    for (int k = 0; k < 9; ++k) { wk[k] = w9[t * 9 + k]; A += wk[k]; }
#pragma unroll
    for (int k = 0; k < 9; ++k)
#pragma unroll
      for (int l = 0; l < 9; ++l) Q += wk[k] * wk[l] * R[2 + k / 3 - l / 3][2 + k % 3 - l % 3];
    for (int u = 0; u < dup; ++u) {
      const double bb = static_cast<double>(tvec[static_cast<size_t>(trow) * 96 + t] + cvec[(static_cast<size_t>(i) * dup + u) * 96 + t]);
      csum[t][u][0] = A * S1 + IMG_PIX * bb;
      csum[t][u][1] = Q + 2.0 * bb * A * S1 + IMG_PIX * bb * bb;
    }
  }
  __syncthreads();
  if (t < GN_GROUPS * dup) {
    const int g = t & 7, u = t >> 3;
    double sd = 0.0, qd = 0.0;
    for (int j = 0; j < 12; ++j) { sd += csum[g * 12 + j][u][0]; qd += csum[g * 12 + j][u][1]; }
    const double cnt = static_cast<double>(IMG_PIX) * 12.0;
    const double mean = sd / cnt;
    double var = qd / cnt - mean * mean;
    var = var < 0.0 ? 0.0 : var;
    s_mean[u][g] = static_cast<float>(mean);
    s_rstd[u][g] = static_cast<float>(1.0 / sqrt(var + static_cast<double>(GN_EPS)));
  }
  float w0[9], w1[9];
#pragma unroll
  for (int k = 0; k < 9; ++k) { w0[k] = w9[oc * 9 + k]; w1[k] = w9[(oc + 1) * 9 + k]; }
  float b0[2], b1[2];
  for (int u = 0; u < 2; ++u) {
    const int uu = u < dup ? u : 0;
    b0[u] = tvec[static_cast<size_t>(trow) * 96 + oc] + cvec[(static_cast<size_t>(i) * dup + uu) * 96 + oc];
    b1[u] = tvec[static_cast<size_t>(trow) * 96 + oc + 1] + cvec[(static_cast<size_t>(i) * dup + uu) * 96 + oc + 1];
  }
  __syncthreads();
  const int g = op / 6;
  float sc0[2], sh0[2], sc1[2], sh1[2];
  {
    const float ga0 = gamma[oc], ga1 = gamma[oc + 1], be0 = beta[oc], be1 = beta[oc + 1];
#pragma unroll
    for (int u = 0; u < 2; ++u) {
      sc0[u] = s_rstd[u][g] * ga0; sh0[u] = (b0[u] - s_mean[u][g]) * sc0[u] + be0;
      sc1[u] = s_rstd[u][g] * ga1; sh1[u] = (b1[u] - s_mean[u][g]) * sc1[u] + be1;
    }
  }
  constexpr int PO = IMG + 2;
  const int p_begin = band * (IMG_PIX / FC_SPLIT), p_end = p_begin + IMG_PIX / FC_SPLIT;
  (void)p_end;
  if constexpr (FAST) {
    float2 w2[9], sc2[2], sh2[2];
#pragma unroll
    for (int k = 0; k < 9; ++k) w2[k] = make_float2(w0[k], w1[k]);
#pragma unroll
    for (int u = 0; u < 2; ++u) { sc2[u] = make_float2(0.5f * sc0[u], 0.5f * sc1[u]); sh2[u] = make_float2(0.5f * sh0[u], 0.5f * sh1[u]); }
    for (int qd = pg; qd < IMG_PIX / FC_SPLIT / 4; qd += 8) {
      const int p = p_begin + qd * 4;
      const int yy = p >> 6, xx = p & 63;
      float2 c[4];
#pragma unroll
      for (int j = 0; j < 4; ++j) c[j] = make_float2(0.f, 0.f);
#pragma unroll
      for (int ky = 0; ky < 3; ++ky) {
        float2 xv[6];
#pragma unroll
        for (int k = 0; k < 6; ++k) xv[k] = xs[yy + 1 + ky][xx + 1 + k];
#pragma unroll
        for (int kx = 0; kx < 3; ++kx)
#pragma unroll
          for (int j = 0; j < 4; ++j) c[j] = pk_fma2v(w2[ky * 3 + kx], xv[j + kx], c[j]);
      }
      T* const o_run = out + ((static_cast<size_t>(i) * dup * PO + yy + 1) * PO + xx + 1) * 96 + oc;
      constexpr long long IMG_STRIDE = static_cast<long long>(PO) * PO * 96, COL_WRAP = static_cast<long long>(IMG) * 96;
      const long long wyo = static_cast<long long>(halo_wrap(yy, IMG)) * PO * 96;
      const bool left = xx == 0, right = xx == IMG - 4;
#pragma unroll
      for (int j = 0; j < 4; ++j) {
#pragma unroll
        for (int u = 0; u < 2; ++u) {
          if (u >= dup) break;
          const float2 hh = pk_fma2v(c[j], sc2[u], sh2[u]);
          float t0, t1;
          asm("tanh.approx.f32 %0, %1;" : "=f"(t0) : "f"(hh.x));
          asm("tanh.approx.f32 %0, %1;" : "=f"(t1) : "f"(hh.y));
          const float2 yv = pk_fma2v(hh, make_float2(t0, t1), hh);
          T* const o = o_run + j * 96 + u * IMG_STRIDE;
          store_pair<T>(o, yv.x, yv.y);
          if (wyo) store_pair<T>(o + wyo, yv.x, yv.y);
          if (j == 0 && left) {
            store_pair<T>(o + COL_WRAP, yv.x, yv.y);
            if (wyo) store_pair<T>(o + wyo + COL_WRAP, yv.x, yv.y);
          }
          if (j == 3 && right) {
            store_pair<T>(o - COL_WRAP, yv.x, yv.y);
            if (wyo) store_pair<T>(o + wyo - COL_WRAP, yv.x, yv.y);
          }
        }
      }
    }
    return;
  }
  for (int qd = pg; qd < IMG_PIX / FC_SPLIT / 4; qd += 8) {
    const int p = p_begin + qd * 4;
    const int yy = p >> 6, xx = p & 63;
    float xv[3][6];
#pragma unroll
    for (int ky = 0; ky < 3; ++ky)
#pragma unroll
      for (int k = 0; k < 6; ++k) xv[ky][k] = xs[yy + 1 + ky][xx + 1 + k].x;
    float c[4][2];
#pragma unroll
    for (int j = 0; j < 4; ++j) c[j][0] = c[j][1] = 0.f;
#pragma unroll
    for (int ky = 0; ky < 3; ++ky)
#pragma unroll
      for (int kx = 0; kx < 3; ++kx)
#pragma unroll
        for (int j = 0; j < 4; ++j) {
          c[j][0] = fmaf(w0[ky * 3 + kx], xv[ky][j + kx], c[j][0]);
          c[j][1] = fmaf(w1[ky * 3 + kx], xv[ky][j + kx], c[j][1]);
        }
    const int wy = halo_wrap(yy, IMG);
#pragma unroll
    for (int j = 0; j < 4; ++j) {
      const int wx = halo_wrap(xx + j, IMG);
#pragma unroll
      for (int u = 0; u < 2; ++u) {
        if (u >= dup) break;
        const float y0 = silu_f<FAST>(fmaf(c[j][0], sc0[u], sh0[u]));
        const float y1 = silu_f<FAST>(fmaf(c[j][1], sc1[u], sh1[u]));
        const size_t base = ((static_cast<size_t>(i) * dup + u) * PO + yy + 1) * PO + xx + j + 1;
        store_pair<T>(out + base * 96 + oc, y0, y1);
        if (wy) store_pair<T>(out + (base + static_cast<long long>(wy) * PO) * 96 + oc, y0, y1);
        if (wx) store_pair<T>(out + (base + wx) * 96 + oc, y0, y1);
        if (wy && wx) store_pair<T>(out + (base + static_cast<long long>(wy) * PO + wx) * 96 + oc, y0, y1);
      }
    }
  }
}

template <typename T>
int launch_first_conv_gn(const float* x, const float* w9, const float* tvec, int tvec_stride, const int* step_ptr,
                         int trow_off, const float* cvec, int n, int dup, const float* gamma, const float* beta, T* out,
                         cudaStream_t st) {
  if (n <= 0) return TCS_OK;
  first_conv_gn_kernel<T><<<n * FC_SPLIT, 384, 0, st>>>(x, w9, tvec, tvec_stride, step_ptr, trow_off, cvec, dup, gamma,
                                                        beta, out);
  TCS_CUDA(cudaGetLastError());
  return TCS_OK;
}
template int launch_first_conv_gn<float>(const float*, const float*, const float*, int, const int*, int, const float*, int, int, const float*, const float*, float*, cudaStream_t);
template int launch_first_conv_gn<__nv_bfloat16>(const float*, const float*, const float*, int, const int*, int, const float*, int, int, const float*, const float*, __nv_bfloat16*, cudaStream_t);

__global__ void __launch_bounds__(256) gn_finalize_kernel(const float* __restrict__ partials, int slots, double count,
                                                         float2* __restrict__ stats) {
  const int b = blockIdx.x, warp = threadIdx.x >> 5, lane = threadIdx.x & 31;
  const float* part = partials + static_cast<size_t>(b) * slots * 16;
  double s = 0.0, q = 0.0;
  for (int k = lane; k < slots; k += 32) {
    s += static_cast<double>(part[k * 16 + 2 * warp]);
    q += static_cast<double>(part[k * 16 + 2 * warp + 1]);
  }
#pragma unroll
  for (int o = 16; o > 0; o >>= 1) {
    s += __shfl_xor_sync(0xffffffffu, s, o);
    q += __shfl_xor_sync(0xffffffffu, q, o);
  }
  if (lane == 0) {
    const double mean = s / count;
    double var = q / count - mean * mean;
    var = var < 0.0 ? 0.0 : var;
    stats[b * GN_GROUPS + warp] = make_float2(static_cast<float>(mean),
                                              static_cast<float>(1.0 / sqrt(var + static_cast<double>(GN_EPS))));
  }
}

template <bool FAST> __device__ __forceinline__ float silu_f(float v) {
  if constexpr (FAST) {
    const float h = 0.5f * v;
    float t;
    asm("tanh.approx.f32 %0, %1;" : "=f"(t) : "f"(h));
    return fmaf(h, t, h);
  }
  return v / (1.0f + expf(-v));
}

template <typename T, bool IN_PADDED, bool SILU>
__global__ void __launch_bounds__(256) gn_apply_kernel(const void* __restrict__ in_, const float2* __restrict__ stats,
                                                      const float* __restrict__ gamma, const float* __restrict__ beta,
                                                      int H, int W, int C, T* __restrict__ out) {
  constexpr bool FAST = sizeof(T) == 2;
  __shared__ float s_mean[GN_GROUPS], s_rstd[GN_GROUPS];
  const int b = blockIdx.y;
  if (threadIdx.x < GN_GROUPS) {
    const float2 st = stats[b * GN_GROUPS + threadIdx.x];
    s_mean[threadIdx.x] = st.x;
    s_rstd[threadIdx.x] = st.y;
  }
  __syncthreads();
  const int cv = C / 8, cpg = C / GN_GROUPS;
  const int nvec = H * W * cv;
  const int Wp = W + 2, Hp = H + 2;
  const int e0 = blockIdx.x * 1024 + threadIdx.x;
  float v[4][8];
#pragma unroll
  for (int k = 0; k < 4; ++k) {
    const int e = e0 + k * 256;
    if (e >= nvec) continue;
    const int pix = e / cv, c = (e - pix * cv) * 8;
    if constexpr (IN_PADDED) {
      const int y = pix / W, x = pix - y * W;
      Vec8<T> iv;
      iv.load(static_cast<const T*>(in_) + ((static_cast<size_t>(b) * Hp + y + 1) * Wp + x + 1) * C + c);
      iv.get(v[k]);
    } else {
      Vec8<float> iv;
      iv.load(static_cast<const float*>(in_) + (static_cast<size_t>(b) * H * W + pix) * C + c);
      iv.get(v[k]);
    }
  }
#pragma unroll
  for (int k = 0; k < 4; ++k) {
    const int e = e0 + k * 256;
    if (e >= nvec) continue;
    const int pix = e / cv, c = (e - pix * cv) * 8;
    const int y = pix / W, x = pix - y * W;
    const float4 g0 = __ldg(reinterpret_cast<const float4*>(gamma + c)), g1 = __ldg(reinterpret_cast<const float4*>(gamma + c + 4));
    const float4 b0 = __ldg(reinterpret_cast<const float4*>(beta + c)), b1 = __ldg(reinterpret_cast<const float4*>(beta + c + 4));
    const float gm[8] = {g0.x, g0.y, g0.z, g0.w, g1.x, g1.y, g1.z, g1.w};
    const float bt[8] = {b0.x, b0.y, b0.z, b0.w, b1.x, b1.y, b1.z, b1.w};
#pragma unroll
    for (int j = 0; j < 8; ++j) {
      const int g = (c + j) / cpg;
      float yv = (v[k][j] - s_mean[g]) * s_rstd[g] * gm[j] + bt[j];
      if constexpr (SILU) yv = silu_f<FAST>(yv);
// ... 751 lines not shown
```

vae-diffusion-toy-crystals_b200/csrc/tcs_api.cu:

```cuda
#include <cmath>
#include <cstdio>
#include <cstdlib>
#include <cstring>
#include <map>
#include <memory>
#include <string>
#include <vector>

#include "attn_tc.cuh"
#include "conv_tc.cuh"
#include "kernels.cuh"

namespace tcs {

static thread_local std::string g_err;
void set_error(const std::string& m) { g_err = m; }
int fail(int code, const std::string& m) {
  g_err = m;
  return code;
}

static void time_grid_host(int steps, double t_end, float* ts) {
  const int n = steps + 1;
  const float step = n > 1 ? (1.0f - 0.0f) / static_cast<float>(n - 1) : 0.f;
  const int halfway = n / 2;
  const float te = static_cast<float>(t_end);
  const float ome = static_cast<float>(1.0 - t_end);
  for (int i = 0; i < n; ++i) {
    const float u = i < halfway ? 0.0f + step * static_cast<float>(i) : 1.0f - step * static_cast<float>(n - i - 1);
    const float om = 1.0f - u;
    const float sq = om * om;
    ts[i] = te + ome * sq;
  }
}
struct Sched {
  double bmin, bmax;
  float beta(float t) const { return static_cast<float>(bmin) + t * static_cast<float>(bmax - bmin); }
  float int_beta(float t) const {
    return static_cast<float>(bmin) * t + static_cast<float>(0.5 * (bmax - bmin)) * (t * t);
  }
  float alpha(float t) const { return expf(-0.5f * int_beta(t)); }
  float sigma(float t) const {
    const float a = alpha(t);
    const float v = 1.0f - a * a;
    return sqrtf(v < 1e-8f ? 1e-8f : v);
  }
};


enum ConvId { C_D1B, C_DS1, C_D2A, C_D2B, C_DS2, C_MA, C_MB, C_QKV, C_PROJ, C_US2, C_U2A, C_U2B, C_US1, C_U1A, C_U1B, C_COUNT };
struct ConvSpec { const char* key; int cin0, cin1, cout, k, stride, res; };
static const ConvSpec kConv[C_COUNT] = {
    {"down1.net.3", 96, 0, 96, 3, 1, 64},  {"ds1", 96, 0, 96, 4, 2, 32},       {"down2.net.0", 96, 0, 192, 3, 1, 32},
    {"down2.net.3", 192, 0, 192, 3, 1, 32}, {"ds2", 192, 0, 192, 4, 2, 16},     {"mid.net.0", 192, 0, 192, 3, 1, 16},
    {"mid.net.3", 192, 0, 192, 3, 1, 16},   {"attn.qkv", 192, 0, 576, 1, 1, 16}, {"attn.proj", 192, 0, 192, 1, 1, 16},
    {"us2_conv", 192, 0, 192, 3, 1, 32},    {"up2.net.0", 192, 192, 96, 3, 1, 32}, {"up2.net.3", 96, 0, 96, 3, 1, 32},
    {"us1_conv", 96, 0, 96, 3, 1, 64},      {"up1.net.0", 96, 96, 96, 3, 1, 64}, {"up1.net.3", 96, 0, 96, 3, 1, 64}};

static ConvGeom geom_of(int id, int B, int in_pad) {
  const ConvSpec& s = kConv[id];
  ConvGeom g;
  g.B = B; g.H = g.W = s.res; g.ksize = s.k; g.stride = s.stride;
  g.nsrc = s.cin1 ? 2 : 1;
  g.csrc[0] = s.cin0; g.csrc[1] = s.cin1 ? s.cin1 : s.cin0;
  g.in_pad[0] = g.in_pad[1] = in_pad;
  g.ntot = s.cout;
  return g;
}

static const char* kTapNames[] = {
    "down1.net.0.raw", "down1.net.0.act", "down1.net.3.raw", "down1.net.3.act", "ds1",
    "down2.net.0.raw", "down2.net.0.act", "down2.net.3.raw", "down2.net.3.act", "ds2",
    "mid.net.0.raw", "mid.net.0.act", "mid.net.3.raw", "mid.net.3.act", "attn.qkv", "attn.y", "attn",
    "us2.up", "us2_conv", "up2.net.0.raw", "up2.net.0.act", "up2.net.3.raw", "up2.net.3.act",
    "us1.up", "us1_conv", "up1.net.0.raw", "up1.net.0.act", "up1.net.3.raw", "up1.net.3.act", "eps"};
constexpr int kNumTaps = sizeof(kTapNames) / sizeof(kTapNames[0]);

struct TapRequest {
  int id = -1;
  float* out = nullptr;
  int64_t capacity = 0;
  int64_t written = 0;
};

}

using namespace tcs;

struct tcs_handle {
  tcs_config cfg;
  int sm_count = 148;
  bool bf16 = false, use_tc = false, fuse_gn = false, fuse_first = true;
  bool fuse_attn = false;
  DevBuf attn_wpack;
  bool fuse_ups = false;
  ConvTcPlan plan_us[2];
  bool split3 = false;
  size_t esz = 4;
  cudaStream_t stream = nullptr;
  cudaEvent_t ev_in = nullptr, ev_out = nullptr;
  int64_t launches = 0;
  cudaEvent_t prof_ev[2 * 16] = {};
  bool profiling = false;

  std::map<std::string, HostTensor> host_w;
  bool finalized = false;
  DevBuf arena;
  std::map<std::string, const float*> dw;
  EmbedWeights ew{};
  const float *d_w9 = nullptr, *d_wout = nullptr;
  float out_bias = 0.f;
  DevBuf wpack[C_COUNT];

  int chunk = 0;
  DevBuf raw64, raw32, raw16, partials, gnstats;
  DevBuf p64_h1, p64_a, p64_b;
  DevBuf p32_96a, p32_96b, p32_192a, p32_192h2, p32_192b;
  DevBuf p16_a, p16_b, p16_c, qkv, atty;
  DevBuf split_s;
  ConvTcPlan plan[C_COUNT];
  ConvTcPlan plan_eps, plan_eps_pair;
  DevBuf wpack_out;
  const float* d_bias16 = nullptr;
  bool tc_out = false, eps_kxn = true;

  DevBuf cvec, tvec, tvals, coef, x, xpred, d0, eps, step_ctr, ycat_tmp, ycont_tmp;
  DevBuf status;
  void* pinned = nullptr; size_t pinned_bytes = 0;
  cudaEvent_t ev_pinned = nullptr;

  cudaGraphExec_t gexec = nullptr;
  uint64_t ws_gen = 0;
  struct GKey { int n = -1, dup, sampler; const void *noise, *teps, *tx; float guidance; uint64_t seed, gidx, gen; } gkey;
  int64_t graph_kernels = 0;

  tcs_handle() {
    for (DevBuf* b : {&cvec, &tvec, &tvals, &coef, &x, &xpred, &d0, &eps, &step_ctr}) b->gen = &ws_gen;
  }

  ~tcs_handle() {
    if (gexec) cudaGraphExecDestroy(gexec);
    if (pinned) cudaFreeHost(pinned);
    if (ev_in) cudaEventDestroy(ev_in);
    if (ev_out) cudaEventDestroy(ev_out);
    if (ev_pinned) cudaEventDestroy(ev_pinned);
    for (cudaEvent_t e : prof_ev) if (e) cudaEventDestroy(e);
    if (stream) cudaStreamDestroy(stream);
  }
};

namespace tcs {

static std::vector<std::pair<std::string, std::vector<int64_t>>> expected_weights(const tcs_config& c) {
  std::vector<std::pair<std::string, std::vector<int64_t>>> v;
  const int64_t e = c.emb_dim, b = c.base_ch, cin = 1 + c.cond_ch + c.time_ch;
  auto lin = [&](const std::string& k, int64_t i, int64_t o) { v.push_back({k + ".weight", {o, i}}); v.push_back({k + ".bias", {o}}); };
  auto conv = [&](const std::string& k, int64_t i, int64_t o, int64_t ks) { v.push_back({k + ".weight", {o, i, ks, ks}}); v.push_back({k + ".bias", {o}}); };
  auto gn = [&](const std::string& k, int64_t ch) { v.push_back({k + ".weight", {ch}}); v.push_back({k + ".bias", {ch}}); };
  auto block = [&](const std::string& k, int64_t i, int64_t o) { conv(k + ".net.0", i, o, 3); gn(k + ".net.1", o); conv(k + ".net.3", o, o, 3); gn(k + ".net.4", o); };
  v.push_back({"cond_emb.cat_emb.weight", {c.n_types + 1, e}});
  lin("cond_emb.cont_mlp.0", c.y_cont_dim, e); lin("cond_emb.cont_mlp.2", e, e); lin("cond_emb.out.1", 2 * e, e);
  lin("time_mlp.0", e, e); lin("time_mlp.2", e, e);
  lin("to_cond_map", e, c.cond_ch); lin("to_time_map", e, c.time_ch);
  block("down1", cin, b); conv("ds1", b, b, 4); block("down2", b, 2 * b); conv("ds2", 2 * b, 2 * b, 4);
  block("mid", 2 * b, 2 * b); gn("attn.norm", 2 * b); conv("attn.qkv", 2 * b, 6 * b, 1); conv("attn.proj", 2 * b, 2 * b, 1);
  conv("us2_conv", 2 * b, 2 * b, 3); block("up2", 4 * b, b); conv("us1_conv", b, b, 3); block("up1", 2 * b, b);
  conv("out", b, 1, 3);
  return v;
}

static int enter(tcs_handle* h, cudaStream_t user) {
  TCS_CUDA(cudaSetDevice(h->cfg.device));
  TCS_CUDA(cudaEventRecord(h->ev_in, user));
  TCS_CUDA(cudaStreamWaitEvent(h->stream, h->ev_in, 0));
  return TCS_OK;
}
static int leave(tcs_handle* h, cudaStream_t user) {
  TCS_CUDA(cudaEventRecord(h->ev_out, h->stream));
  TCS_CUDA(cudaStreamWaitEvent(user, h->ev_out, 0));
  return TCS_OK;
}

static int ensure_pinned(tcs_handle* h, size_t bytes) {
  if (h->pinned_bytes >= bytes) {
    TCS_CUDA(cudaEventSynchronize(h->ev_pinned));
    return TCS_OK;
  }
  TCS_CUDA(cudaEventSynchronize(h->ev_pinned));
  if (h->pinned) cudaFreeHost(h->pinned);
  h->pinned = nullptr; h->pinned_bytes = 0;
  TCS_CUDA(cudaMallocHost(&h->pinned, bytes));
  h->pinned_bytes = bytes;
  return TCS_OK;
}

static int alloc_workspace(tcs_handle* h) {
  const size_t MB = h->chunk, e = h->esz;
  TCS_CHECK(h->raw64.ensure(MB * 4096 * 96 * 4));
  TCS_CHECK(h->raw32.ensure(MB * 1024 * 192 * 4));
  TCS_CHECK(h->raw16.ensure(MB * 256 * 192 * 4));
  TCS_CHECK(h->partials.ensure(MB * 128 * 16 * 4));
  TCS_CHECK(h->gnstats.ensure(MB * 8 * 8));
  const size_t P64 = MB * 66 * 66 * 96 * e, P32a = MB * 34 * 34 * 96 * e, P32b = MB * 34 * 34 * 192 * e,
               P16 = MB * 18 * 18 * 192 * e;
  TCS_CHECK(h->p64_h1.ensure(P64)); TCS_CHECK(h->p64_a.ensure(P64)); TCS_CHECK(h->p64_b.ensure(P64));
  TCS_CHECK(h->p32_96a.ensure(P32a)); TCS_CHECK(h->p32_96b.ensure(P32a));
  TCS_CHECK(h->p32_192a.ensure(P32b)); TCS_CHECK(h->p32_192h2.ensure(P32b)); TCS_CHECK(h->p32_192b.ensure(P32b));
  TCS_CHECK(h->p16_a.ensure(P16)); TCS_CHECK(h->p16_b.ensure(P16)); TCS_CHECK(h->p16_c.ensure(P16));
  TCS_CHECK(h->qkv.ensure(MB * 256 * 576 * e));
  TCS_CHECK(h->atty.ensure(MB * 256 * 192 * e));
  if (h->split3) TCS_CHECK(h->split_s.ensure(P64));
  return TCS_OK;
}

struct ConvWiring { const void *s0, *s1; void* out; int epi; const void* residual; int ldo; int in_pad;
                    const char* gn; void* act; };
static ConvWiring wiring(tcs_handle* h, int id) {
  ConvWiring w{};
  switch (id) {
    case C_D1B: w = {h->p64_a.p, nullptr, h->raw64.p, EPI_RAW_STATS, nullptr, 96, 1, "down1.net.4", h->p64_h1.p}; break;
    case C_DS1: w = {h->p64_h1.p, nullptr, h->p32_96a.p, EPI_PADDED, nullptr, 96, 1, nullptr, nullptr}; break;
    case C_D2A: w = {h->p32_96a.p, nullptr, h->raw32.p, EPI_RAW_STATS, nullptr, 192, 1, "down2.net.1", h->p32_192a.p}; break;
    case C_D2B: w = {h->p32_192a.p, nullptr, h->raw32.p, EPI_RAW_STATS, nullptr, 192, 1, "down2.net.4", h->p32_192h2.p}; break;
    case C_DS2: w = {h->p32_192h2.p, nullptr, h->p16_a.p, EPI_PADDED, nullptr, 192, 1, nullptr, nullptr}; break;
    case C_MA: w = {h->p16_a.p, nullptr, h->raw16.p, EPI_RAW_STATS, nullptr, 192, 1, "mid.net.1", h->p16_b.p}; break;
    case C_MB: w = {h->p16_b.p, nullptr, h->raw16.p, EPI_RAW_STATS, nullptr, 192, 1, "mid.net.4", h->p16_a.p}; break;
    case C_QKV: w = {h->p16_b.p, nullptr, h->qkv.p, EPI_PLAIN, nullptr, 576, 1, nullptr, nullptr}; break;
    case C_PROJ: w = {h->atty.p, nullptr, h->p16_c.p, EPI_PADDED, h->p16_a.p, 192, 0, nullptr, nullptr}; break;
    case C_US2: w = {h->p32_192a.p, nullptr, h->p32_192b.p, EPI_PADDED, nullptr, 192, 1, nullptr, nullptr}; break;
    case C_U2A: w = {h->p32_192b.p, h->p32_192h2.p, h->raw32.p, EPI_RAW_STATS, nullptr, 96, 1, "up2.net.1", h->p32_96a.p}; break;
    case C_U2B: w = {h->p32_96a.p, nullptr, h->raw32.p, EPI_RAW_STATS, nullptr, 96, 1, "up2.net.4", h->p32_96b.p}; break;
    case C_US1: w = {h->p64_a.p, nullptr, h->p64_b.p, EPI_PADDED, nullptr, 96, 1, nullptr, nullptr}; break;
    case C_U1A: w = {h->p64_b.p, h->p64_h1.p, h->raw64.p, EPI_RAW_STATS, nullptr, 96, 1, "up1.net.1", h->p64_a.p}; break;
    default: w = {h->p64_a.p, nullptr, h->raw64.p, EPI_RAW_STATS, nullptr, 96, 1, "up1.net.4", h->p64_b.p}; break;
  }
  if (h->fuse_gn && w.gn) {
    w.out = w.act;
    w.epi = EPI_GN_FUSED;
  }
  return w;
}

static int slots_of(tcs_handle* h, int id) {
  const int r = kConv[id].res;
  return h->use_tc ? tc_slots(r, r) : simt_slots(r, r);
}

struct SplitSrc { const void* p; size_t lo; };
struct SplitWiring { SplitSrc s0, s1; float* raw; int ldo; int in_pad; };
static size_t padded_elems(const tcs_handle* h, int res, int C) { return static_cast<size_t>(h->chunk) * (res + 2) * (res + 2) * C; }
static SplitWiring split_wiring(tcs_handle* h, int id) {
  const SplitSrc S64{h->split_s.p, padded_elems(h, 64, 96)}, S32{h->split_s.p, padded_elems(h, 32, 192)},
      S16{h->split_s.p, padded_elems(h, 16, 192)}, SY{h->split_s.p, static_cast<size_t>(h->chunk) * 256 * 192};
  const SplitSrc h1{h->p64_h1.p, padded_elems(h, 64, 96)}, h2{h->p32_192h2.p, padded_elems(h, 32, 192)};
  const SplitSrc none{nullptr, 0};
  float *r64 = h->raw64.as<float>(), *r32 = h->raw32.as<float>(), *r16 = h->raw16.as<float>();
  switch (id) {
    case C_D1B: return {S64, none, r64, 96, 1};
    case C_DS1: return {h1, none, r32, 96, 1};
    case C_D2A: return {{h->p32_96a.p, padded_elems(h, 32, 96)}, none, r32, 192, 1};
    case C_D2B: return {{h->p32_192a.p, padded_elems(h, 32, 192)}, none, r32, 192, 1};
    case C_DS2: return {h2, none, r16, 192, 1};
    case C_MA: return {{h->p16_c.p, padded_elems(h, 16, 192)}, none, r16, 192, 1};
    case C_MB: return {{h->p16_b.p, padded_elems(h, 16, 192)}, none, r16, 192, 1};
    case C_QKV: return {S16, none, h->qkv.as<float>(), 576, 1};
    case C_PROJ: return {SY, none, r16, 192, 0};
    case C_US2: return {S32, none, r32, 192, 1};
    case C_U2A: return {{h->p32_192b.p, padded_elems(h, 32, 192)}, h2, r32, 96, 1};
    case C_U2B: return {{h->p32_96a.p, padded_elems(h, 32, 96)}, none, r32, 96, 1};
    case C_US1: return {S64, none, r64, 96, 1};
    case C_U1A: return {{h->p64_b.p, padded_elems(h, 64, 96)}, h1, r64, 96, 1};
    default: return {{h->p64_a.p, padded_elems(h, 64, 96)}, none, r64, 96, 1};
  }
}

static int build_plans(tcs_handle* h) {
  if (!h->use_tc) return TCS_OK;
  if (h->split3) {
    for (int id = 0; id < C_COUNT; ++id) {
      const SplitWiring w = split_wiring(h, id);
      ConvGeom g = geom_of(id, h->chunk, w.in_pad);
      g.split3 = 1;
      EpiArgs ea{};
      ea.bias = h->dw.at(std::string(kConv[id].key) + ".bias");
      ea.out = w.raw; ea.partials = h->partials.as<float>(); ea.ldo = w.ldo; ea.slots = slots_of(h, id);
      auto lo = [](const SplitSrc& s) { return s.p ? static_cast<const void*>(static_cast<const __nv_bfloat16*>(s.p) + s.lo) : nullptr; };
      TCS_CHECK(conv_tc_make_plan(&h->plan[id], g, w.s0.p, w.s1.p, h->wpack[id].as<__nv_bfloat16>(), EPI_RAW_STATS, ea,
                                  h->sm_count, lo(w.s0), lo(w.s1)));
    }
    return TCS_OK;
  }
  {
    const char* e = getenv("TCS_TC_OUT");
    h->tc_out = !(e && atoi(e) == 0);
    ConvGeom g = geom_of(C_U1B, h->chunk, 1);
    g.ntot = 16;
    g.kx_in_n = h->eps_kxn ? 1 : 0;
    EpiArgs ea{};
    ea.bias = h->d_bias16; ea.out = nullptr; ea.ldo = 1;
    TCS_CHECK(conv_tc_make_plan(&h->plan_eps, g, h->p64_b.p, nullptr, h->wpack_out.as<__nv_bfloat16>(), EPI_EPS, ea, h->sm_count));
    h->plan_eps_pair = h->plan_eps;
    TCS_CHECK(conv_tc_make_pair(&h->plan_eps_pair, h->p64_b.p, h->chunk));
  }
  for (int id = 0; id < C_COUNT; ++id) {
    const ConvWiring w = wiring(h, id);
    const ConvGeom g = geom_of(id, h->chunk, w.in_pad);
    EpiArgs ea{};
    ea.bias = h->dw.at(std::string(kConv[id].key) + ".bias");
    ea.out = w.out; ea.partials = h->partials.as<float>(); ea.residual = w.residual; ea.ldo = w.ldo;
    ea.slots = slots_of(h, id);
    ea.overflow = h->status.as<int>();
    if (w.epi == EPI_GN_FUSED) {
      ea.gamma = h->dw.at(std::string(w.gn) + ".weight");
      ea.beta = h->dw.at(std::string(w.gn) + ".bias");
    }
    TCS_CHECK(conv_tc_make_plan(&h->plan[id], g, w.s0, w.s1, h->wpack[id].as<__nv_bfloat16>(), w.epi, ea, h->sm_count));
  }
  if (h->fuse_ups) {
    const int ids[2] = {C_US2, C_US1};
    const void* lowres[2] = {h->p16_c.p, h->p32_96b.p};
    for (int k = 0; k < 2; ++k) {
      const ConvWiring w = wiring(h, ids[k]);
      ConvGeom g = geom_of(ids[k], h->chunk, w.in_pad);
      g.ups = 1;
      EpiArgs ea{};
      ea.bias = h->dw.at(std::string(kConv[ids[k]].key) + ".bias");
      ea.out = w.out; ea.partials = h->partials.as<float>(); ea.residual = nullptr; ea.ldo = w.ldo;
      ea.slots = slots_of(h, ids[k]);
      ea.overflow = h->status.as<int>();
      const int rc = conv_tc_make_plan(&h->plan_us[k], g, lowres[k], nullptr, h->wpack[ids[k]].as<__nv_bfloat16>(), EPI_PADDED, ea, h->sm_count);
      if (rc == TCS_ERR_UNSUPPORTED) { h->fuse_ups = false; break; }
      TCS_CHECK(rc);
    }
  }
  for (int id = 0; id < C_COUNT; ++id) {
    if (!h->plan[id].coop_cluster) continue;
    ConvTcPlan pl = h->plan[id];
    const int B = h->chunk < 16 ? h->chunk : 16;
    pl.p.n_mtiles = B * pl.p.tiles_per_img;
    pl.grid = conv_tc_grid(pl, B, h->sm_count);
    const int rc = conv_tc_launch(pl, h->stream);
    const cudaError_t se = cudaStreamSynchronize(h->stream);
    if (rc != TCS_OK || se != cudaSuccess) {
      cudaGetLastError();
      if (se != cudaSuccess && se != cudaErrorCooperativeLaunchTooLarge && se != cudaErrorInvalidValue)
        return fail(TCS_ERR_CUDA, std::string("trial launch of a fused conv failed: ") + cudaGetErrorString(se));
      for (int j = 0; j < C_COUNT; ++j) h->plan[j].coop_cluster = false;
      break;
    }
  }
  TCS_CUDA(cudaMemsetAsync(h->status.p, 0, 4, h->stream));
  return TCS_OK;
}

template <typename T>
static int run_conv_inner(tcs_handle* h, int id, int B, cudaStream_t st);

template <typename T>
static int run_conv(tcs_handle* h, int id, int B, cudaStream_t st) {
  if (!h->profiling) return run_conv_inner<T>(h, id, B, st);
  TCS_CUDA(cudaEventRecord(h->prof_ev[2 * id], st));
  TCS_CHECK(run_conv_inner<T>(h, id, B, st));
  TCS_CUDA(cudaEventRecord(h->prof_ev[2 * id + 1], st));
  return TCS_OK;
}

template <typename T>
static int run_conv_inner(tcs_handle* h, int id, int B, cudaStream_t st) {
  ++h->launches;
  if (h->use_tc) {
    ConvTcPlan pl = h->plan[id];
    pl.p.n_mtiles = B * pl.p.tiles_per_img;
    pl.grid = conv_tc_grid(pl, B, h->sm_count);
    return conv_tc_launch(pl, st);
  }
  const ConvWiring w = wiring(h, id);
  const ConvGeom g = geom_of(id, B, w.in_pad);
  EpiArgs ea{};
  ea.bias = h->dw.at(std::string(kConv[id].key) + ".bias");
  ea.out = w.out; ea.partials = h->partials.as<float>(); ea.residual = w.residual; ea.ldo = w.ldo;
  ea.slots = slots_of(h, id);
  return launch_conv_simt<T>(g, static_cast<const T*>(w.s0), static_cast<const T*>(w.s1), h->wpack[id].as<float>(),
                             w.epi, ea, st);
}

struct PassArgs {
  const float* x;
  const float* cvec;
  const float* tvec;
  int tvec_stride;
  const int* step_ptr;
  int trow_off;
  int ns, dup;
  float guidance;
  float* eps;
};

template <typename T>
static int forward_chunk(tcs_handle* h, const PassArgs& a, cudaStream_t st, TapRequest* tap) {
  const int B = a.ns * a.dup;
  float* part = h->partials.as<float>();
  auto gnw = [&](const char* k) { return h->dw.at(std::string(k) + ".weight"); };
  auto gnb = [&](const char* k) { return h->dw.at(std::string(k) + ".bias"); };
  int tap_idx = 0;
  auto tapout = [&](int kind, const void* p, int H, int W, int C) -> int {
    const int my = tap_idx++;
    if (!tap || tap->id != my) return 0;
    const int64_t cnt = static_cast<int64_t>(B) * H * W * C;
    if (cnt > tap->capacity) return fail(TCS_ERR_BAD_ARGUMENT, "tcs_debug_layer: output buffer too small");
    if (kind == 0) { TCS_CUDA(cudaMemcpyAsync(tap->out, p, cnt * 4, cudaMemcpyDeviceToDevice, st)); }
    else TCS_CHECK(launch_unpad_to_f32<T>(static_cast<const T*>(p), B, H, W, C, kind == 1 ? 1 : 0, tap->out, st));
    tap->written = cnt;
    return 1;
  };
#define TAP(kind, p, H, W, C) { int _r = tapout(kind, p, H, W, C); if (_r != 0) return _r < 0 ? _r : TCS_OK; }
#define CONV_GN(cid, raw, res, C)                                                                         \
  {                                                                                                      \
    const ConvWiring _w = wiring(h, cid);                                                                 \
    TCS_CHECK(run_conv<T>(h, cid, B, st));                                                                \
    if (_w.epi == EPI_GN_FUSED) {                                                                        \
      if (tap && tap->id == tap_idx) return fail(TCS_ERR_UNSUPPORTED, "raw conv output does not exist when GroupNorm is fused"); \
      ++tap_idx;                                                                                         \
    } else {                                                                                             \
      TAP(0, raw, res, res, C);                                                                          \
      GN(_w.gn, raw, slots_of(h, cid), res, C, static_cast<T*>(_w.act));                                  \
    }                                                                                                    \
    TAP(1, _w.act, res, res, C);                                                                         \
  }
#define GN(key, raw, slots, res, C, out) \
  { h->launches += 2; TCS_CHECK(launch_gn_apply<T>(raw, 0, part, slots, gnw(key), gnb(key), B, res, res, C, 1, out, h->gnstats.as<float2>(), st)); }

  if (h->fuse_first && !(tap && tap->id == 0)) {
    ++h->launches;
    TCS_CHECK(launch_first_conv_gn<T>(a.x, h->d_w9, a.tvec, a.tvec_stride, a.step_ptr, a.trow_off, a.cvec, a.ns, a.dup,
                                      gnw("down1.net.1"), gnb("down1.net.1"), h->p64_a.as<T>(), st));
    ++tap_idx;
  } else {
    ++h->launches;
    TCS_CHECK(launch_first_conv(a.x, h->d_w9, a.tvec, a.tvec_stride, a.step_ptr, a.trow_off, a.cvec, a.ns, a.dup,
                                h->raw64.as<float>(), part, st));
    TAP(0, h->raw64.p, 64, 64, 96);
    GN("down1.net.1", h->raw64.p, FIRST_CONV_SLOTS, 64, 96, h->p64_a.as<T>());
  }
  TAP(1, h->p64_a.p, 64, 64, 96);
  CONV_GN(C_D1B, h->raw64.p, 64, 96);
  TCS_CHECK(run_conv<T>(h, C_DS1, B, st));
  TAP(1, h->p32_96a.p, 32, 32, 96);
  CONV_GN(C_D2A, h->raw32.p, 32, 192);
  CONV_GN(C_D2B, h->raw32.p, 32, 192);
  TCS_CHECK(run_conv<T>(h, C_DS2, B, st));
  TAP(1, h->p16_a.p, 16, 16, 192);
  CONV_GN(C_MA, h->raw16.p, 16, 192);
  CONV_GN(C_MB, h->raw16.p, 16, 192);
  if (h->fuse_attn && sizeof(T) == 2 && !(tap && (tap->id == tap_idx || tap->id == tap_idx + 1))) {
    ++h->launches;
    AttnTcParams ap{};
    ap.x = h->p16_a.as<__nv_bfloat16>(); ap.out = h->p16_c.as<__nv_bfloat16>();
    ap.wpack = h->attn_wpack.as<uint8_t>();
    ap.bias_qkv = h->dw.at("attn.qkv.bias"); ap.bias_proj = h->dw.at("attn.proj.bias");
    ap.gamma = gnw("attn.norm"); ap.beta = gnb("attn.norm");
    ap.B = B;
    if (h->profiling) {
      TCS_CUDA(cudaEventRecord(h->prof_ev[2 * C_QKV], st));
    }
    TCS_CHECK(launch_attn_block_tc(ap, h->sm_count, st));
    if (h->profiling) {
      TCS_CUDA(cudaEventRecord(h->prof_ev[2 * C_QKV + 1], st));
      TCS_CUDA(cudaEventRecord(h->prof_ev[2 * C_PROJ], st));
      TCS_CUDA(cudaEventRecord(h->prof_ev[2 * C_PROJ + 1], st));
    }
    tap_idx += 2;
  } else {
    ++h->launches;
    TCS_CHECK(launch_gn_image16<T>(h->p16_a.as<T>(), B, gnw("attn.norm"), gnb("attn.norm"), h->p16_b.as<T>(), st));
    TCS_CHECK(run_conv<T>(h, C_QKV, B, st));
    TAP(2, h->qkv.p, 16, 16, 576);
    ++h->launches;
    TCS_CHECK(launch_attention<T>(h->qkv.as<T>(), B, h->atty.as<T>(), st));
    TAP(2, h->atty.p, 16, 16, 192);
    TCS_CHECK(run_conv<T>(h, C_PROJ, B, st));
  }
  TAP(1, h->p16_c.p, 16, 16, 192);
  auto us_conv = [&](int k, int id) -> int {
    ++h->launches;
    ConvTcPlan pl = h->plan_us[k];
    pl.p.n_mtiles = B * pl.p.tiles_per_img;
    pl.grid = conv_tc_grid(pl, B, h->sm_count);
    if (h->profiling) TCS_CUDA(cudaEventRecord(h->prof_ev[2 * id], st));
    TCS_CHECK(conv_tc_launch(pl, st));
    if (h->profiling) TCS_CUDA(cudaEventRecord(h->prof_ev[2 * id + 1], st));
    return TCS_OK;
  };
  if (h->fuse_ups && sizeof(T) == 2 && !(tap && tap->id == tap_idx)) {
    ++tap_idx;
    TCS_CHECK(us_conv(0, C_US2));
  } else {
    ++h->launches;
    TCS_CHECK(launch_upsample2x<T>(h->p16_c.as<T>(), B, 16, 16, 192, h->p32_192a.as<T>(), st));
    TAP(1, h->p32_192a.p, 32, 32, 192);
    TCS_CHECK(run_conv<T>(h, C_US2, B, st));
  }
  TAP(1, h->p32_192b.p, 32, 32, 192);
  CONV_GN(C_U2A, h->raw32.p, 32, 96);
  CONV_GN(C_U2B, h->raw32.p, 32, 96);
  if (h->fuse_ups && sizeof(T) == 2 && !(tap && tap->id == tap_idx)) {
    ++tap_idx;
    TCS_CHECK(us_conv(1, C_US1));
  } else {
    ++h->launches;
    TCS_CHECK(launch_upsample2x<T>(h->p32_96b.as<T>(), B, 32, 32, 96, h->p64_a.as<T>(), st));
    TAP(1, h->p64_a.p, 64, 64, 96);
    TCS_CHECK(run_conv<T>(h, C_US1, B, st));
  }
  TAP(1, h->p64_b.p, 64, 64, 96);
  CONV_GN(C_U1A, h->raw64.p, 64, 96);
  CONV_GN(C_U1B, h->raw64.p, 64, 96);
  ++h->launches;
  if (h->use_tc && h->tc_out) {
    ConvTcPlan pl = a.dup == 2 ? h->plan_eps_pair : h->plan_eps;
    pl.p.n_mtiles = (a.dup == 2 ? B / 2 : B) * pl.p.tiles_per_img;
    pl.p.guidance = a.guidance;
    pl.p.epi.out = a.eps;
    pl.grid = conv_tc_grid(pl, B, h->sm_count);
    TCS_CHECK(conv_tc_launch(pl, st));
  } else {
    TCS_CHECK(launch_out_conv<T>(h->p64_b.as<T>(), h->d_wout, h->out_bias, a.ns, a.dup, a.guidance, a.eps, st));
  }
  if (tap && tap->id == kNumTaps - 1) {
    const int64_t cnt = static_cast<int64_t>(a.ns) * 4096;
    if (cnt > tap->capacity) return fail(TCS_ERR_BAD_ARGUMENT, "tcs_debug_layer: output buffer too small");
    TCS_CUDA(cudaMemcpyAsync(tap->out, a.eps, cnt * 4, cudaMemcpyDeviceToDevice, st));
    tap->written = cnt;
  }
#undef TAP
#undef GN
#undef CONV_GN
  return TCS_OK;
}

static int forward_chunk_split3(tcs_handle* h, const PassArgs& a, cudaStream_t st, TapRequest* tap) {
  const int B = a.ns * a.dup;
  float* part = h->partials.as<float>();
  float2* stats = h->gnstats.as<float2>();
  auto gnw = [&](const char* k) { return h->dw.at(std::string(k) + ".weight"); };
  auto gnb = [&](const char* k) { return h->dw.at(std::string(k) + ".bias"); };
  auto bf = [](void* p) { return static_cast<__nv_bfloat16*>(p); };
  int tap_idx = 0;
  auto tapout = [&](int kind, const void* p, size_t lo, int res, int C) -> int {
    const int my = tap_idx++;
    if (!tap || tap->id != my) return 0;
    if (kind < 0) return fail(TCS_ERR_UNSUPPORTED, "this activation is not materialised in bf16x3 mode");
    const int64_t cnt = static_cast<int64_t>(B) * res * res * C;
    if (cnt > tap->capacity) return fail(TCS_ERR_BAD_ARGUMENT, "tcs_debug_layer: output buffer too small");
    if (kind == 0 || kind == 2) { TCS_CUDA(cudaMemcpyAsync(tap->out, p, cnt * 4, cudaMemcpyDeviceToDevice, st)); }
    else if (kind == 1) TCS_CHECK(launch_unpad_to_f32<float>(static_cast<const float*>(p), B, res, res, C, 1, tap->out, st));
    else TCS_CHECK(launch_unsplit_to_f32(static_cast<const __nv_bfloat16*>(p), lo, B, res, res, C, 1, tap->out, st));
    tap->written = cnt;
    return 1;
  };
#define TAP(kind, p, lo, res, C) { int _r = tapout(kind, p, lo, res, C); if (_r != 0) return _r < 0 ? _r : TCS_OK; }
  auto conv = [&](int id) -> int {
    ++h->launches;
    ConvTcPlan pl = h->plan[id];
    pl.p.n_mtiles = B * pl.p.tiles_per_img;
    pl.grid = conv_tc_grid(pl, B, h->sm_count);
    if (h->profiling) TCS_CUDA(cudaEventRecord(h->prof_ev[2 * id], st));
    TCS_CHECK(conv_tc_launch(pl, st));
    if (h->profiling) TCS_CUDA(cudaEventRecord(h->prof_ev[2 * id + 1], st));
    return TCS_OK;
  };
  auto split_in = [&](const float* src, size_t elems_per_img, size_t lo) -> int {
    ++h->launches;
    return launch_split(src, static_cast<size_t>(B) * elems_per_img, bf(h->split_s.p), lo, st);
  };
  auto gn_split = [&](const char* key, int id, const float* raw, int res, int C, void* out) -> int {
    h->launches += 2;
    TCS_CHECK(launch_gn_finalize(part, slots_of(h, id), B, res, res, C, stats, st));
    return launch_raw_to_padded(0, raw, stats, gnw(key), gnb(key), nullptr, B, res, res, C, out, padded_elems(h, res, C), st);
  };
  auto gn_f32 = [&](const char* key, int id, const float* raw, int res, int C, float* out) -> int {
    h->launches += 2;
    return launch_gn_apply<float>(raw, 0, part, slots_of(h, id), gnw(key), gnb(key), B, res, res, C, 1, out, stats, st);
  };
  auto pad_split = [&](const float* raw, int res, int C, void* out) -> int {
    ++h->launches;
    return launch_raw_to_padded(1, raw, nullptr, nullptr, nullptr, nullptr, B, res, res, C, out, padded_elems(h, res, C), st);
  };
  float *r64 = h->raw64.as<float>(), *r32 = h->raw32.as<float>(), *r16 = h->raw16.as<float>();
  const size_t E64 = padded_elems(h, 64, 96), E32a = padded_elems(h, 32, 96), E32b = padded_elems(h, 32, 192),
               E16 = padded_elems(h, 16, 192);
  if (!(tap && tap->id == 0)) {
    ++h->launches;
    TCS_CHECK(launch_first_conv_gn<float>(a.x, h->d_w9, a.tvec, a.tvec_stride, a.step_ptr, a.trow_off, a.cvec, a.ns, a.dup,
                                          gnw("down1.net.1"), gnb("down1.net.1"), h->p64_a.as<float>(), st));
    ++tap_idx;
  } else {
    ++h->launches;
    TCS_CHECK(launch_first_conv(a.x, h->d_w9, a.tvec, a.tvec_stride, a.step_ptr, a.trow_off, a.cvec, a.ns, a.dup, r64, part, st));
    TAP(0, r64, 0, 64, 96);
  }
  TAP(1, h->p64_a.p, 0, 64, 96);
  TCS_CHECK(split_in(h->p64_a.as<float>(), 66 * 66 * 96, E64));
  TCS_CHECK(conv(C_D1B));
  TAP(0, r64, 0, 64, 96);
  TCS_CHECK(gn_split("down1.net.4", C_D1B, r64, 64, 96, h->p64_h1.p));
  TAP(3, h->p64_h1.p, E64, 64, 96);
  TCS_CHECK(conv(C_DS1));
  TCS_CHECK(pad_split(r32, 32, 96, h->p32_96a.p));
  TAP(3, h->p32_96a.p, E32a, 32, 96);
  TCS_CHECK(conv(C_D2A));
  TAP(0, r32, 0, 32, 192);
  TCS_CHECK(gn_split("down2.net.1", C_D2A, r32, 32, 192, h->p32_192a.p));
  TAP(3, h->p32_192a.p, E32b, 32, 192);
  TCS_CHECK(conv(C_D2B));
  TAP(0, r32, 0, 32, 192);
  TCS_CHECK(gn_split("down2.net.4", C_D2B, r32, 32, 192, h->p32_192h2.p));
  TAP(3, h->p32_192h2.p, E32b, 32, 192);
  TCS_CHECK(conv(C_DS2));
  TCS_CHECK(pad_split(r16, 16, 192, h->p16_c.p));
  TAP(3, h->p16_c.p, E16, 16, 192);
  TCS_CHECK(conv(C_MA));
  TAP(0, r16, 0, 16, 192);
  TCS_CHECK(gn_split("mid.net.1", C_MA, r16, 16, 192, h->p16_b.p));
  TAP(3, h->p16_b.p, E16, 16, 192);
  TCS_CHECK(conv(C_MB));
  TAP(0, r16, 0, 16, 192);
  TCS_CHECK(gn_f32("mid.net.4", C_MB, r16, 16, 192, h->p16_a.as<float>()));
  TAP(1, h->p16_a.p, 0, 16, 192);
  ++h->launches;
  TCS_CHECK(launch_gn_image16<float>(h->p16_a.as<float>(), B, gnw("attn.norm"), gnb("attn.norm"), h->p16_b.as<float>(), st));
  TCS_CHECK(split_in(h->p16_b.as<float>(), 18 * 18 * 192, E16));
  TCS_CHECK(conv(C_QKV));
  TAP(2, h->qkv.p, 0, 16, 576);
  ++h->launches;
  TCS_CHECK(launch_attention<float>(h->qkv.as<float>(), B, h->atty.as<float>(), st));
  TAP(2, h->atty.p, 0, 16, 192);
  TCS_CHECK(split_in(h->atty.as<float>(), 256 * 192, static_cast<size_t>(h->chunk) * 256 * 192));
  TCS_CHECK(conv(C_PROJ));
  ++h->launches;
  TCS_CHECK(launch_raw_to_padded(2, r16, nullptr, nullptr, nullptr, h->p16_a.as<float>(), B, 16, 16, 192, h->p16_c.p, 0, st));
  TAP(1, h->p16_c.p, 0, 16, 192);
  ++h->launches;
  TCS_CHECK(launch_upsample2x<float>(h->p16_c.as<float>(), B, 16, 16, 192, h->p32_192a.as<float>(), st));
  TAP(1, h->p32_192a.p, 0, 32, 192);
  TCS_CHECK(split_in(h->p32_192a.as<float>(), 34 * 34 * 192, E32b));
  TCS_CHECK(conv(C_US2));
  TCS_CHECK(pad_split(r32, 32, 192, h->p32_192b.p));
  TAP(3, h->p32_192b.p, E32b, 32, 192);
  TCS_CHECK(conv(C_U2A));
  TAP(0, r32, 0, 32, 96);
  TCS_CHECK(gn_split("up2.net.1", C_U2A, r32, 32, 96, h->p32_96a.p));
  TAP(3, h->p32_96a.p, E32a, 32, 96);
  TCS_CHECK(conv(C_U2B));
  TAP(0, r32, 0, 32, 96);
  TCS_CHECK(gn_f32("up2.net.4", C_U2B, r32, 32, 96, h->p32_96b.as<float>()));
  TAP(1, h->p32_96b.p, 0, 32, 96);
  ++h->launches;
  TCS_CHECK(launch_upsample2x<float>(h->p32_96b.as<float>(), B, 32, 32, 96, h->p64_a.as<float>(), st));
  TAP(1, h->p64_a.p, 0, 64, 96);
  TCS_CHECK(split_in(h->p64_a.as<float>(), 66 * 66 * 96, E64));
  TCS_CHECK(conv(C_US1));
  TCS_CHECK(pad_split(r64, 64, 96, h->p64_b.p));
  TAP(3, h->p64_b.p, E64, 64, 96);
  TCS_CHECK(conv(C_U1A));
  TAP(0, r64, 0, 64, 96);
  TCS_CHECK(gn_split("up1.net.1", C_U1A, r64, 64, 96, h->p64_a.p));
  TAP(3, h->p64_a.p, E64, 64, 96);
  TCS_CHECK(conv(C_U1B));
  TAP(0, r64, 0, 64, 96);
  TCS_CHECK(gn_f32("up1.net.4", C_U1B, r64, 64, 96, h->p64_b.as<float>()));
  TAP(1, h->p64_b.p, 0, 64, 96);
  ++h->launches;
  TCS_CHECK(launch_out_conv<float>(h->p64_b.as<float>(), h->d_wout, h->out_bias, a.ns, a.dup, a.guidance, a.eps, st));
  if (tap && tap->id == kNumTaps - 1) {
    const int64_t cnt = static_cast<int64_t>(a.ns) * 4096;
    if (cnt > tap->capacity) return fail(TCS_ERR_BAD_ARGUMENT, "tcs_debug_layer: output buffer too small");
    TCS_CUDA(cudaMemcpyAsync(tap->out, a.eps, cnt * 4, cudaMemcpyDeviceToDevice, st));
// ... 63 lines not shown

extern "C" {

const char* tcs_last_error(void) { return g_err.c_str(); }
#ifndef TCS_SRC_HASH
#define TCS_SRC_HASH "unknown"
#endif
const char* tcs_build_info(void) {
  return "libtcs sm_100a: tcgen05 implicit-GEMM conv (bf16, bf16x3) + FFMA conv (fp32), built " __DATE__ " " __TIME__
         " TCS_SRC_HASH=" TCS_SRC_HASH;
}
int64_t tcs_launch_count(const tcs_handle* h) { return h ? h->launches : 0; }
int32_t tcs_check(tcs_handle* h) {
  if (!h) return fail(TCS_ERR_BAD_ARGUMENT, "tcs_check: null handle");
  TCS_CUDA(cudaSetDevice(h->cfg.device));
  int bits = 0;
  TCS_CUDA(cudaMemcpyAsync(&bits, h->status.p, 4, cudaMemcpyDeviceToHost, h->stream));
  TCS_CUDA(cudaStreamSynchronize(h->stream));
  if (bits) TCS_CUDA(cudaMemsetAsync(h->status.p, 0, 4, h->stream));
  return bits & 0x7fffffff;
}
int32_t tcs_launch_mode(const tcs_handle* h) {
  if (!h || !h->finalized || !h->use_tc) return 0;
  const ConvTcPlan& pl = h->plan[C_D1B];
  return (h->fuse_gn ? 1 : 0) | (pl.coop_cluster ? 2 : 0) | (pl.max_ctas << 8);
}
int32_t tcs_nfe(int32_t sampler, int32_t steps) { return sampler == TCS_SAMPLER_ODE ? 2 * steps + 1 : steps + 1; }

void tcs_default_config(tcs_config* c) {
  if (!c) return;
  memset(c, 0, sizeof(*c));
  c->n_types = 4; c->y_cont_dim = 4; c->base_ch = 96; c->emb_dim = 128; c->cond_ch = 8; c->time_ch = 8;
  c->beta_min = 0.1; c->beta_max = 30.0;
  c->precision = TCS_BF16; c->engine = TCS_ENGINE_AUTO; c->device = 0; c->chunk = 0; c->use_graph = 1; c->fuse_gn = 1;
}

int tcs_time_grid_host(int32_t steps, double t_end, float* ts) {
  if (steps < 1 || !ts) return fail(TCS_ERR_BAD_ARGUMENT, "tcs_time_grid_host: steps >= 1 and ts required");
  time_grid_host(steps, t_end, ts);
  return TCS_OK;
}
int tcs_schedule_host(double bmin, double bmax, float t, float* beta, float* alpha, float* sigma) {
  const Sched s{bmin, bmax};
  if (beta) *beta = s.beta(t);
  if (alpha) *alpha = s.alpha(t);
  if (sigma) *sigma = s.sigma(t);
  return TCS_OK;
}

int tcs_create(tcs_handle** out, const tcs_config* cfg) {
  if (!out || !cfg) return fail(TCS_ERR_BAD_ARGUMENT, "tcs_create: null argument");
  *out = nullptr;
  if (cfg->base_ch != 96 || cfg->emb_dim != 128 || cfg->cond_ch != 8 || cfg->time_ch != 8)
    return fail(TCS_ERR_UNSUPPORTED,
                "this build supports base_ch=96, emb_dim=128, cond_ch=8, time_ch=8 only (got " +
                    std::to_string(cfg->base_ch) + "/" + std::to_string(cfg->emb_dim) + "/" +
                    std::to_string(cfg->cond_ch) + "/" + std::to_string(cfg->time_ch) + ")");
  if (cfg->n_types < 1 || cfg->y_cont_dim < 3 || cfg->y_cont_dim > 16)
    return fail(TCS_ERR_BAD_ARGUMENT, "tcs_create: need n_types >= 1 and 3 <= y_cont_dim <= 16 (theta sin/cos uses columns 1,2)");
  if (cfg->precision != TCS_FP32 && cfg->precision != TCS_BF16) return fail(TCS_ERR_BAD_ARGUMENT, "tcs_create: bad precision");
  int ndev = 0;
  cudaError_t e = cudaGetDeviceCount(&ndev);
  if (e != cudaSuccess || ndev == 0)
    return fail(TCS_ERR_CUDA, std::string("no CUDA device: ") + cudaGetErrorString(e) + " (libtcs has no CPU fallback)");
  if (cfg->device < 0 || cfg->device >= ndev) return fail(TCS_ERR_BAD_ARGUMENT, "tcs_create: bad device ordinal");
  TCS_CUDA(cudaSetDevice(cfg->device));
  cudaDeviceProp prop;
  TCS_CUDA(cudaGetDeviceProperties(&prop, cfg->device));
  if (prop.major != 10)
    return fail(TCS_ERR_UNSUPPORTED, std::string("libtcs is built for sm_100a only; device is ") + prop.name);
  std::unique_ptr<tcs_handle> h(new tcs_handle());
  h->cfg = *cfg;
  h->sm_count = prop.multiProcessorCount;
  h->bf16 = cfg->precision == TCS_BF16;
  h->esz = h->bf16 ? 2 : 4;
  int eng = cfg->engine;
  if (eng == TCS_ENGINE_AUTO) eng = h->bf16 ? TCS_ENGINE_TCGEN05 : TCS_ENGINE_SIMT;
  h->use_tc = eng == TCS_ENGINE_TCGEN05;
  h->split3 = h->use_tc && !h->bf16;
  {
    const char* e = getenv("TCS_FUSE_GN");
    h->fuse_gn = h->use_tc && !h->split3 && cfg->fuse_gn != 0 && !(e && atoi(e) == 0);
    h->fuse_first = !(e && atoi(e) == 0);
    const char* eu = getenv("TCS_FUSE_UPS");
    h->fuse_ups = h->use_tc && !h->split3 && !(eu && atoi(eu) == 0);
    const char* ea = getenv("TCS_FUSE_ATTN");
    h->fuse_attn = h->use_tc && !h->split3 && !(ea && atoi(ea) == 0);
  }
  h->chunk = cfg->chunk > 0 ? cfg->chunk : 2048;
  if (h->chunk % 2) h->chunk += 1;
  TCS_CUDA(cudaStreamCreateWithFlags(&h->stream, cudaStreamNonBlocking));
  TCS_CUDA(cudaEventCreateWithFlags(&h->ev_in, cudaEventDisableTiming));
  TCS_CUDA(cudaEventCreateWithFlags(&h->ev_out, cudaEventDisableTiming));
  TCS_CUDA(cudaEventCreateWithFlags(&h->ev_pinned, cudaEventDisableTiming));
  TCS_CHECK(h->step_ctr.ensure(16));
  TCS_CHECK(h->status.ensure(16));
  TCS_CUDA(cudaMemset(h->status.p, 0, 16));
  *out = h.release();
  return TCS_OK;
}

void tcs_destroy(tcs_handle* h) {
  if (!h) return;
  cudaSetDevice(h->cfg.device);
  cudaStreamSynchronize(h->stream);
  delete h;
}

int tcs_set_weight(tcs_handle* h, const char* key, const float* data, const int64_t* shape, int32_t ndim) {
  if (!h || !key || !data || !shape || ndim < 1 || ndim > 4) return fail(TCS_ERR_BAD_ARGUMENT, "tcs_set_weight: bad argument");
  TCS_CUDA(cudaSetDevice(h->cfg.device));
  HostTensor t;
  size_t cnt = 1;
  for (int i = 0; i < ndim; ++i) { t.shape.push_back(shape[i]); cnt *= static_cast<size_t>(shape[i]); }
  t.v.resize(cnt);
  TCS_CUDA(cudaMemcpy(t.v.data(), data, cnt * 4, cudaMemcpyDefault));
  h->host_w[key] = std::move(t);
  h->finalized = false;
  return TCS_OK;
}

int tcs_finalize_weights(tcs_handle* h) {
  if (!h) return fail(TCS_ERR_BAD_ARGUMENT, "tcs_finalize_weights: null handle");
  TCS_CUDA(cudaSetDevice(h->cfg.device));
  const auto exp = expected_weights(h->cfg);
  size_t total = 0;
  for (const auto& kv : exp) {
    auto it = h->host_w.find(kv.first);
    if (it == h->host_w.end()) return fail(TCS_ERR_STATE, "missing state-dict tensor: " + kv.first);
    if (it->second.shape != kv.second) return fail(TCS_ERR_BAD_ARGUMENT, "state-dict tensor has the wrong shape: " + kv.first);
    total += (it->second.v.size() + 63) / 64 * 64;
  }
  if (h->host_w.size() != exp.size()) return fail(TCS_ERR_BAD_ARGUMENT, "unexpected extra state-dict tensors");
  const HostTensor& w0 = h->host_w.at("down1.net.0.weight");
  std::vector<float> wsum(96 * 16), w9(96 * 9), wout(9 * 96);
  for (int oc = 0; oc < 96; ++oc) {
    for (int k = 0; k < 9; ++k) w9[oc * 9 + k] = w0.v[(oc * 17 + 0) * 9 + k];
    for (int c = 0; c < 16; ++c) {
      float s = 0.f;
      for (int k = 0; k < 9; ++k) s += w0.v[(oc * 17 + 1 + c) * 9 + k];
      wsum[oc * 16 + c] = s;
    }
  }
  const HostTensor& wo = h->host_w.at("out.weight");
  for (int c = 0; c < 96; ++c)
    for (int k = 0; k < 9; ++k) wout[k * 96 + c] = wo.v[c * 9 + k];
  h->out_bias = h->host_w.at("out.bias").v[0];
  const size_t extra = 96 * 16 + 96 * 9 + 9 * 96 + 64 + 256;
  TCS_CHECK(h->arena.ensure((total + extra) * 4));
  float* base = h->arena.as<float>();
  size_t off = 0;
  h->dw.clear();
  for (const auto& kv : exp) {
    const HostTensor& t = h->host_w.at(kv.first);
    TCS_CUDA(cudaMemcpy(base + off, t.v.data(), t.v.size() * 4, cudaMemcpyHostToDevice));
    h->dw[kv.first] = base + off;
    off += (t.v.size() + 63) / 64 * 64;
  }
  auto put = [&](const std::vector<float>& v, const float** dst) -> int {
    TCS_CUDA(cudaMemcpy(base + off, v.data(), v.size() * 4, cudaMemcpyHostToDevice));
    *dst = base + off;
    off += (v.size() + 63) / 64 * 64;
    return TCS_OK;
  };
  const float* d_wsum = nullptr;
  std::vector<float> bias16(16, 0.f);
// ... 440 lines not shown
  g.split3 = 1;
  const int B = g.B, Hin = g.H * g.stride, Win = g.W * g.stride, pad = g.in_pad[0];
  DevBuf f32[2], sp[2], wp, db, part;
  const float* ins[2] = {in0, in1};
  size_t elems[2] = {0, 0};
  for (int s = 0; s < g.nsrc; ++s) {
    elems[s] = static_cast<size_t>(B) * (Hin + 2 * pad) * (Win + 2 * pad) * g.csrc[s];
    TCS_CHECK(f32[s].ensure(elems[s] * 4));
    TCS_CHECK(sp[s].ensure(elems[s] * 4));
    TCS_CHECK(launch_pad_from_plain<float>(ins[s], B, Hin, Win, g.csrc[s], pad, f32[s].as<float>(), st));
    TCS_CHECK(launch_split(f32[s].as<float>(), elems[s], sp[s].as<__nv_bfloat16>(), elems[s], st));
  }
  int cin = 0;
  for (int s = 0; s < g.nsrc; ++s) cin += g.csrc[s];
  const size_t wcount = static_cast<size_t>(g.ntot) * cin * g.ksize * g.ksize;
  std::vector<float> hw(wcount), hb(g.ntot);
  TCS_CUDA(cudaMemcpy(hw.data(), weight, wcount * 4, cudaMemcpyDefault));
  TCS_CUDA(cudaMemcpy(hb.data(), bias, g.ntot * 4, cudaMemcpyDefault));
  TCS_CHECK(db.ensure(g.ntot * 4));
  TCS_CUDA(cudaMemcpy(db.p, hb.data(), g.ntot * 4, cudaMemcpyHostToDevice));
  std::vector<__nv_bfloat16> pk(conv_tc_packed_elems(g));
  conv_tc_pack_weights(g, EPI_RAW_STATS, hw.data(), pk.data());
  TCS_CHECK(wp.ensure(pk.size() * 2));
  TCS_CUDA(cudaMemcpy(wp.p, pk.data(), pk.size() * 2, cudaMemcpyHostToDevice));
  const int slots = tc_slots(g.H, g.W);
  TCS_CHECK(part.ensure(static_cast<size_t>(B) * slots * 16 * 4));
  EpiArgs ea{};
  ea.bias = db.as<float>(); ea.ldo = g.ntot; ea.slots = slots; ea.out = out; ea.partials = part.as<float>();
  ConvTcPlan pl;
  int dev = 0, sms = 148;
  cudaGetDevice(&dev);
  cudaDeviceGetAttribute(&sms, cudaDevAttrMultiProcessorCount, dev);
  TCS_CHECK(conv_tc_make_plan(&pl, g, sp[0].p, g.nsrc == 2 ? sp[1].p : nullptr, wp.as<__nv_bfloat16>(), EPI_RAW_STATS, ea, sms,
                              sp[0].as<__nv_bfloat16>() + elems[0], g.nsrc == 2 ? sp[1].as<__nv_bfloat16>() + elems[1] : nullptr));
  TCS_CHECK(conv_tc_launch(pl, st));
  TCS_CUDA(cudaStreamSynchronize(st));
  if (stats && epi == EPI_RAW_STATS) {
    std::vector<float> hp(static_cast<size_t>(B) * slots * 16);
    TCS_CUDA(cudaMemcpy(hp.data(), part.p, hp.size() * 4, cudaMemcpyDeviceToHost));
    std::vector<float> hs(static_cast<size_t>(B) * 16);
    for (int b = 0; b < B; ++b)
      for (int k = 0; k < 16; ++k) {
        double acc = 0;
        for (int s = 0; s < slots; ++s) acc += hp[(static_cast<size_t>(b) * slots + s) * 16 + k];
        hs[b * 16 + k] = static_cast<float>(acc);
      }
    TCS_CUDA(cudaMemcpy(stats, hs.data(), hs.size() * 4, cudaMemcpyDefault));
  }
  return TCS_OK;
}

extern "C" {

int tcs_debug_conv(int32_t engine, int32_t precision, int32_t B, int32_t H_out, int32_t W_out, int32_t cin0,
                   int32_t cin1, int32_t cout, int32_t ksize, int32_t stride, const float* in0, const float* in1,
                   const float* weight, const float* bias, float* out, float* stats, int32_t epi, void* stream) {
  if (!in0 || !weight || !bias || !out || B < 1) return fail(TCS_ERR_BAD_ARGUMENT, "tcs_debug_conv: bad argument");
  if (epi < 0 || epi > 2) return fail(TCS_ERR_BAD_ARGUMENT, "tcs_debug_conv: bad epilogue");
  if (H_out != W_out) return fail(TCS_ERR_UNSUPPORTED, "tcs_debug_conv: square outputs only");
  const bool bf16 = precision == TCS_BF16;
  const int eng = engine == TCS_ENGINE_AUTO ? (bf16 ? TCS_ENGINE_TCGEN05 : TCS_ENGINE_SIMT) : engine;
  ConvGeom g;
  g.B = B; g.H = H_out; g.W = W_out; g.ksize = ksize; g.stride = stride;
  g.nsrc = cin1 > 0 ? 2 : 1;
  g.csrc[0] = cin0; g.csrc[1] = cin1 > 0 ? cin1 : cin0;
  g.in_pad[0] = g.in_pad[1] = ksize == 1 ? 0 : 1;
  g.ntot = cout;
  cudaStream_t st = static_cast<cudaStream_t>(stream);
  if (eng == TCS_ENGINE_TCGEN05 && !bf16) return debug_conv_split3(g, in0, in1, weight, bias, out, stats, epi, st);
  if (bf16) return debug_conv_t<__nv_bfloat16>(eng == TCS_ENGINE_TCGEN05, g, in0, in1, weight, bias, out, stats, epi, st);
  return debug_conv_t<float>(false, g, in0, in1, weight, bias, out, stats, epi, st);
}

int tcs_debug_conv_ups(int32_t B, int32_t H_out, int32_t W_out, int32_t cin, int32_t cout, const float* in_lowres,
                       const float* weight, const float* bias, float* out, void* stream) {
  if (!in_lowres || !weight || !bias || !out || B < 1) return fail(TCS_ERR_BAD_ARGUMENT, "tcs_debug_conv_ups: bad argument");
  if (H_out != W_out) return fail(TCS_ERR_UNSUPPORTED, "tcs_debug_conv_ups: square outputs only");
  ConvGeom g;
  g.B = B; g.H = H_out; g.W = W_out; g.ksize = 3; g.stride = 1;
  g.nsrc = 1; g.csrc[0] = g.csrc[1] = cin; g.in_pad[0] = g.in_pad[1] = 1; g.ntot = cout;
  g.ups = 1;
  return debug_conv_t<__nv_bfloat16>(true, g, in_lowres, nullptr, weight, bias, out, nullptr, EPI_PADDED,
                                     static_cast<cudaStream_t>(stream));
}

int64_t tcs_debug_attn_pack(const float* qkv_w, const float* proj_w, uint8_t* out, int64_t capacity) {
  const int64_t need = static_cast<int64_t>(attn_tc_wpack_bytes());
  if (!out) return need;
  if (!qkv_w || !proj_w || capacity < need) return fail(TCS_ERR_BAD_ARGUMENT, "tcs_debug_attn_pack: bad argument");
  attn_tc_pack_weights(qkv_w, proj_w, out);
  return need;
}

int tcs_debug_attn_block(int32_t B, const float* x, const float* gn_w, const float* gn_b, const float* qkv_w,
                         const float* qkv_b, const float* proj_w, const float* proj_b, float* out, float* dbg,
                         void* stream) {
  if (!x || !gn_w || !gn_b || !qkv_w || !qkv_b || !proj_w || !proj_b || !out || B < 1)
    return fail(TCS_ERR_BAD_ARGUMENT, "tcs_debug_attn_block: bad argument");
  cudaStream_t st = static_cast<cudaStream_t>(stream);
  using T = __nv_bfloat16;
  DevBuf din, dout, wp, small;
  const size_t pbytes = static_cast<size_t>(B) * 18 * 18 * 192 * sizeof(T);
  TCS_CHECK(din.ensure(pbytes));
  TCS_CHECK(dout.ensure(pbytes));
  TCS_CUDA(cudaMemsetAsync(dout.p, 0xff, pbytes, st));
  TCS_CHECK(launch_pad_from_plain<T>(x, B, 16, 16, 192, 1, din.as<T>(), st));
  std::vector<float> hq(576 * 192), hp(192 * 192);
  TCS_CUDA(cudaMemcpy(hq.data(), qkv_w, hq.size() * 4, cudaMemcpyDefault));
  TCS_CUDA(cudaMemcpy(hp.data(), proj_w, hp.size() * 4, cudaMemcpyDefault));
  std::vector<uint8_t> pk(attn_tc_wpack_bytes());
  attn_tc_pack_weights(hq.data(), hp.data(), pk.data());
  TCS_CHECK(wp.ensure(pk.size()));
  TCS_CUDA(cudaMemcpy(wp.p, pk.data(), pk.size(), cudaMemcpyHostToDevice));
  TCS_CHECK(small.ensure((576 + 192 * 3) * 4));
  float* sp = small.as<float>();
  TCS_CUDA(cudaMemcpy(sp, qkv_b, 576 * 4, cudaMemcpyDefault));
  TCS_CUDA(cudaMemcpy(sp + 576, proj_b, 192 * 4, cudaMemcpyDefault));
  TCS_CUDA(cudaMemcpy(sp + 768, gn_w, 192 * 4, cudaMemcpyDefault));
  TCS_CUDA(cudaMemcpy(sp + 960, gn_b, 192 * 4, cudaMemcpyDefault));
  AttnTcParams ap{};
  ap.x = din.as<T>(); ap.out = dout.as<T>(); ap.wpack = wp.as<uint8_t>();
  ap.bias_qkv = sp; ap.bias_proj = sp + 576; ap.gamma = sp + 768; ap.beta = sp + 960;
  ap.B = B; ap.dbg = dbg;
  int dev = 0, sms = 148;
  cudaGetDevice(&dev);
  cudaDeviceGetAttribute(&sms, cudaDevAttrMultiProcessorCount, dev);
  TCS_CHECK(launch_attn_block_tc(ap, sms, st));
  TCS_CHECK(launch_unpad_to_f32<T>(dout.as<T>(), B, 16, 16, 192, 1, out, st));
  DevBuf ref;
  TCS_CHECK(ref.ensure(pbytes));
  TCS_CHECK(launch_pad_from_plain<T>(out, B, 16, 16, 192, 1, ref.as<T>(), st));
  TCS_CUDA(cudaStreamSynchronize(st));
  std::vector<uint8_t> a(pbytes), b(pbytes);
  TCS_CUDA(cudaMemcpy(a.data(), dout.p, pbytes, cudaMemcpyDeviceToHost));
  TCS_CUDA(cudaMemcpy(b.data(), ref.p, pbytes, cudaMemcpyDeviceToHost));
  if (memcmp(a.data(), b.data(), pbytes) != 0)
    return fail(TCS_ERR_STATE, "tcs_debug_attn_block: circular halo of the padded output is wrong");
  return TCS_OK;
}

}
```

vae-diffusion-toy-crystals_b200/toycrystals_b200/_cabi.py:

```python
from __future__ import annotations

import ctypes as C
import os
from typing import Optional

_HERE = os.path.dirname(os.path.abspath(__file__))
LIB_PATH = os.path.join(_HERE, "libtcs.so")

TCS_OK, ERR_BAD_ARGUMENT, ERR_UNSUPPORTED, ERR_CUDA, ERR_STATE = 0, -1, -2, -3, -4
FP32, BF16 = 0, 1
ENGINE_AUTO, ENGINE_SIMT, ENGINE_TCGEN05 = 0, 1, 2
SAMPLER_ODE, SAMPLER_SDE = 0, 1


class TcsConfig(C.Structure):
    _fields_ = [("n_types", C.c_int32), ("y_cont_dim", C.c_int32), ("base_ch", C.c_int32), ("emb_dim", C.c_int32),
                ("cond_ch", C.c_int32), ("time_ch", C.c_int32), ("beta_min", C.c_double), ("beta_max", C.c_double),
                ("precision", C.c_int32), ("engine", C.c_int32), ("device", C.c_int32), ("chunk", C.c_int32),
                ("use_graph", C.c_int32), ("fuse_gn", C.c_int32)]


class TcsSampleArgs(C.Structure):
    _fields_ = [("sampler", C.c_int32), ("n", C.c_int32), ("steps", C.c_int32), ("guidance", C.c_float),
                ("t_end", C.c_double), ("y_cat", C.c_void_p), ("y_cont", C.c_void_p), ("x_init", C.c_void_p),
                ("noise", C.c_void_p), ("seed", C.c_uint64), ("global_index_offset", C.c_uint64),
                ("x_out", C.c_void_p), ("trace_eps", C.c_void_p), ("trace_x", C.c_void_p), ("x0_hat", C.c_void_p),
                ("beta_min", C.c_double), ("beta_max", C.c_double)]


class TcsPriorConfig(C.Structure):
    _fields_ = [("z_dim", C.c_int32), ("n_types", C.c_int32), ("y_cont_dim", C.c_int32), ("t_emb_dim", C.c_int32),
                ("width", C.c_int32), ("n_blocks", C.c_int32), ("y_cat_emb_dim", C.c_int32), ("T", C.c_int32),
                ("beta_start", C.c_double), ("beta_end", C.c_double), ("precision", C.c_int32), ("device", C.c_int32),
                ("use_graph", C.c_int32)]


class TcsDdimArgs(C.Structure):
    _fields_ = [("n", C.c_int32), ("n_steps", C.c_int32), ("y_cat", C.c_void_p), ("y_cont", C.c_void_p),
                ("z_init", C.c_void_p), ("seed", C.c_uint64), ("global_index_offset", C.c_uint64),
                ("z0_out", C.c_void_p), ("trace_eps", C.c_void_p), ("trace_z", C.c_void_p)]


class TcsVaeConfig(C.Structure):
    _fields_ = [("z_dim", C.c_int32), ("n_types", C.c_int32), ("y_cont_dim", C.c_int32), ("device", C.c_int32),
                ("precision", C.c_int32)]


SIGNATURES = {
    "tcs_default_config": (None, [C.POINTER(TcsConfig)]),
    "tcs_create": (C.c_int, [C.POINTER(C.c_void_p), C.POINTER(TcsConfig)]),
    "tcs_destroy": (None, [C.c_void_p]),
    "tcs_set_weight": (C.c_int, [C.c_void_p, C.c_char_p, C.c_void_p, C.POINTER(C.c_int64), C.c_int32]),
    "tcs_finalize_weights": (C.c_int, [C.c_void_p]),
    "tcs_score": (C.c_int, [C.c_void_p, C.c_void_p, C.c_void_p, C.c_void_p, C.c_void_p, C.c_int32, C.c_float,
                            C.c_void_p, C.c_void_p]),
    "tcs_sample": (C.c_int, [C.c_void_p, C.POINTER(TcsSampleArgs), C.c_void_p]),
    "tcs_nfe": (C.c_int32, [C.c_int32, C.c_int32]),
    "tcs_condition_grid": (C.c_int, [C.c_void_p, C.c_int32, C.c_int64, C.c_int64, C.c_float, C.c_void_p, C.c_void_p,
                                     C.c_void_p]),
    "tcs_sde_update": (C.c_int, [C.c_void_p, C.c_void_p, C.c_void_p, C.c_void_p, C.c_int32, C.c_float, C.c_float,
                                 C.c_uint64, C.c_uint64, C.c_int32, C.c_void_p]),
    "tcs_ode_update": (C.c_int, [C.c_void_p, C.c_int32, C.c_void_p, C.c_void_p, C.c_void_p, C.c_void_p, C.c_int32,
                                 C.c_float, C.c_float, C.c_void_p]),
    "tcs_time_grid_host": (C.c_int, [C.c_int32, C.c_double, C.POINTER(C.c_float)]),
    "tcs_schedule_host": (C.c_int, [C.c_double, C.c_double, C.c_float, C.POINTER(C.c_float), C.POINTER(C.c_float),
                                    C.POINTER(C.c_float)]),
    "tcs_launch_count": (C.c_int64, [C.c_void_p]),
    "tcs_check": (C.c_int32, [C.c_void_p]),
    "tcs_launch_mode": (C.c_int32, [C.c_void_p]),
    "tcs_build_info": (C.c_char_p, []),
    "tcs_last_error": (C.c_char_p, []),
    "tcs_debug_layer": (C.c_int64, [C.c_void_p, C.c_char_p, C.c_void_p, C.c_void_p, C.c_void_p, C.c_void_p, C.c_int32,
                                    C.c_int32, C.c_void_p, C.c_int64, C.c_void_p]),
    "tcs_score_profiled": (C.c_int, [C.c_void_p, C.c_void_p, C.c_void_p, C.c_void_p, C.c_void_p, C.c_int32, C.c_float,
                                     C.c_void_p, C.POINTER(C.c_float), C.POINTER(C.c_float), C.c_void_p]),
    "tcs_prior_default_config": (None, [C.POINTER(TcsPriorConfig)]),
    "tcs_prior_create": (C.c_int, [C.POINTER(C.c_void_p), C.POINTER(TcsPriorConfig)]),
    "tcs_prior_destroy": (None, [C.c_void_p]),
    "tcs_prior_set_weight": (C.c_int, [C.c_void_p, C.c_char_p, C.c_void_p, C.POINTER(C.c_int64), C.c_int32]),
    "tcs_prior_finalize_weights": (C.c_int, [C.c_void_p]),
    "tcs_prior_eps": (C.c_int, [C.c_void_p, C.c_void_p, C.c_void_p, C.c_void_p, C.c_void_p, C.c_int32, C.c_void_p,
                                C.c_void_p]),
    "tcs_prior_ddim_sample": (C.c_int, [C.c_void_p, C.POINTER(TcsDdimArgs), C.c_void_p]),
    "tcs_prior_schedule_host": (C.c_int, [C.c_int32, C.c_double, C.c_double, C.POINTER(C.c_float)]),
    "tcs_prior_timesteps_host": (C.c_int, [C.c_int32, C.c_int32, C.POINTER(C.c_int64), C.POINTER(C.c_int32)]),
    "tcs_prior_launch_count": (C.c_int64, [C.c_void_p]),
    "tcs_vae_create": (C.c_int, [C.POINTER(C.c_void_p), C.POINTER(TcsVaeConfig)]),
    "tcs_vae_destroy": (None, [C.c_void_p]),
    "tcs_vae_set_weight": (C.c_int, [C.c_void_p, C.c_char_p, C.c_void_p, C.POINTER(C.c_int64), C.c_int32]),
    "tcs_vae_finalize_weights": (C.c_int, [C.c_void_p]),
    "tcs_vae_decode": (C.c_int, [C.c_void_p, C.c_void_p, C.c_void_p, C.c_void_p, C.c_int32, C.c_void_p, C.c_void_p,
                                 C.c_void_p, C.c_void_p]),
    "tcs_vae_launch_count": (C.c_int64, [C.c_void_p]),
    "tcs_prior_profile": (C.c_int, [C.c_void_p, C.c_int32, C.c_int32, C.POINTER(C.c_float)]),
    "tcs_debug_linear": (C.c_int, [C.c_int32, C.c_int32, C.c_int32, C.c_int32, C.c_void_p, C.c_void_p, C.c_void_p,
                                   C.c_void_p, C.c_int32, C.c_int32, C.c_int32, C.c_void_p]),
    "tcs_debug_conv": (C.c_int, [C.c_int32, C.c_int32, C.c_int32, C.c_int32, C.c_int32, C.c_int32, C.c_int32,
                                 C.c_int32, C.c_int32, C.c_int32, C.c_void_p, C.c_void_p, C.c_void_p, C.c_void_p,
                                 C.c_void_p, C.c_void_p, C.c_int32, C.c_void_p]),
    "tcs_debug_attn_block": (C.c_int, [C.c_int32] + [C.c_void_p] * 10),
    "tcs_debug_conv_ups": (C.c_int, [C.c_int32] * 5 + [C.c_void_p] * 5),
    "tcs_debug_attn_pack": (C.c_int64, [C.c_void_p, C.c_void_p, C.c_void_p, C.c_int64]),
}

_lib: Optional[C.CDLL] = None


class TcsError(RuntimeError):
    pass


def lib() -> C.CDLL:
    global _lib
    if _lib is None:
        if not os.path.exists(LIB_PATH):
            raise TcsError(f"{LIB_PATH} is missing: build it with `python __graft_entry__.py build` "
                           "(toycrystals_b200 has no CPU or PyTorch fallback)")
        L = C.CDLL(LIB_PATH)
        for name, (res, args) in SIGNATURES.items():
            fn = getattr(L, name)
            fn.restype, fn.argtypes = res, args
        _lib = L
    return _lib


def last_error() -> str:
    return (lib().tcs_last_error() or b"").decode()


def check(status: int) -> None:
    if status == TCS_OK:
        return
    msg = last_error()
    if status == ERR_BAD_ARGUMENT:
        raise ValueError(msg)
    if status == ERR_UNSUPPORTED:
        raise NotImplementedError(msg)
    raise TcsError(f"libtcs error {status}: {msg}")
```

Before: 238.3.

## Compute first conv and GroupNorm inside second conv's A-operand producer warps

Adds a first-conv window source to the tcgen05 conv kernel. Extra helper warps recompute the 1-channel 3x3 first conv, apply the GroupNorm affine and SiLU, and write bf16 tiles straight into swizzled shared memory for down1.net.3, so the 64x64x96 activation no longer goes through global memory. The GroupNorm statistics move into a separate affine-only kernel. This cuts a full-resolution write and read-back but adds redundant halo compute, extra warps and shared memory, and a new launch.

```diff
diff --git a/include/tcs.h b/include/tcs.h
--- a/include/tcs.h
+++ b/include/tcs.h
@@ -108,6 +108,9 @@
 int tcs_debug_conv_ups(int32_t B, int32_t H_out, int32_t W_out, int32_t cin, int32_t cout, const float* in_lowres,
                        const float* weight, const float* bias, float* out, void* stream);
 
+int tcs_debug_first_conv_affine(int32_t n, int32_t dup, const float* x, const float* w9, const float* bias,
+                                const float* gamma, const float* beta, float* affine, void* stream);
+
 int64_t tcs_debug_attn_pack(const float* qkv_w, const float* proj_w, uint8_t* out, int64_t capacity);
 
 int tcs_debug_attn_block(int32_t B, const float* x, const float* gn_w, const float* gn_b, const float* qkv_w,
diff --git a/vae-diffusion-toy-crystals_b200/csrc/common.cuh b/vae-diffusion-toy-crystals_b200/csrc/common.cuh
--- a/vae-diffusion-toy-crystals_b200/csrc/common.cuh
+++ b/vae-diffusion-toy-crystals_b200/csrc/common.cuh
@@ -53,6 +53,7 @@
   int ntot;
   int split3 = 0;
   int ups = 0;
+  int first_conv = 0;
   int kx_in_n = 0;
 };
 
diff --git a/vae-diffusion-toy-crystals_b200/csrc/conv_tc.cu b/vae-diffusion-toy-crystals_b200/csrc/conv_tc.cu
--- a/vae-diffusion-toy-crystals_b200/csrc/conv_tc.cu
+++ b/vae-diffusion-toy-crystals_b200/csrc/conv_tc.cu
@@ -19,7 +19,14 @@
 constexpr int UC = 96;
 constexpr int BLK = 32;
 constexpr int TC_THREADS = 64 + 32 * EPI_WARPS + 32;
-constexpr int UPS_EXTRA_THREADS = 4 * 32;
+enum WindowSource : int { SRC_TMA = 0, SRC_UPSAMPLE = 1, SRC_FIRSTCONV = 2 };
+constexpr int UPS_WARPS = 4;
+constexpr int FC_WARPS = 4;
+__host__ __device__ constexpr int src_threads(int src) {
+  return TC_THREADS + 32 * (src == SRC_UPSAMPLE ? UPS_WARPS : src == SRC_FIRSTCONV ? FC_WARPS : 0);
+}
+constexpr int FC_XP = 20;
+constexpr uint32_t FC_PATCH_BYTES = FC_XP * FC_XP * 4;
 constexpr int MAX_STAGES = 12;
 constexpr int MAX_A_STAGES = 4;
 constexpr int KB = 64;
@@ -195,14 +202,17 @@
   uint32_t tmem_base;
 };
 
-template <int N, int EPI, int MSUB, int CG, int GEO, int UPS = 0>
-__global__ void __launch_bounds__(TC_THREADS + UPS_EXTRA_THREADS * UPS, 1)
+template <int N, int EPI, int MSUB, int CG, int GEO, int SRC = SRC_TMA>
+__global__ void __launch_bounds__(src_threads(SRC), 1)
 conv_tc_kernel(const __grid_constant__ CUtensorMap mapA0, const __grid_constant__ CUtensorMap mapA1,
                const __grid_constant__ CUtensorMap mapA2, const __grid_constant__ CUtensorMap mapA3,
                const __grid_constant__ CUtensorMap mapW, const __grid_constant__ CUtensorMap mapO,
                const __grid_constant__ CUtensorMap mapO1, const ConvTcParams p) {
   static_assert(GEO == 0 || (EPI != EPI_EPS && EPI != EPI_PLAIN), "tap-shift geometry: padded / fp32 outputs only");
+  constexpr int UPS = SRC == SRC_UPSAMPLE ? 1 : 0;
+  constexpr bool FCW = SRC == SRC_FIRSTCONV;
   static_assert(UPS == 0 || (GEO == 1 && CG == 2 && EPI == EPI_PADDED), "fused upsample: tap-shift CTA pairs, padded output");
+  static_assert(!FCW || (GEO == 1 && CG == 2 && MSUB == 2 && EPI == EPI_GN_FUSED), "first-conv windows: down1.net.3 only");
   constexpr int ACC_STRIDE = (N * MSUB <= 128) ? 128 : 256;
   static_assert(N * MSUB <= 256, "accumulator does not fit a double-buffered TMEM stage");
 
@@ -248,7 +258,7 @@
     }
     if (GEO == 1)
       for (int s = 0; s < p.a_stages; ++s) {
-        ptx::mbar_init(ptx::smem_u32(&bars.fullA[s]), UPS ? 4 * CG : 1);
+        ptx::mbar_init(ptx::smem_u32(&bars.fullA[s]), UPS ? UPS_WARPS * CG : (FCW ? FC_WARPS * CG : 1));
         ptx::mbar_init(ptx::smem_u32(&bars.emptyA[s]), p.issuers);
       }
     if (UPS)
@@ -307,7 +317,7 @@
             int ntile = tile, ncb = cb + 1;
             if (ncb == p.cblk[0]) { ncb = 0; ntile = tile + static_cast<int>(gridDim.x); }
             if (ntile < n_tiles) issue_low(ntile, ncb);
-          } else {
+          } else if constexpr (!FCW) {
           ptx::mbar_wait(ptx::smem_u32(&bars.emptyA[sa]), pa ^ 1);
           const bool stale = (p.debug & 8) && (pa || tile != static_cast<int>(blockIdx.x));
           if (lane == 0) {
@@ -418,7 +428,7 @@
           for (int src = 0; src < p.nsrc; ++src)
             for (int cb = 0; cb < p.cblk[src]; ++cb, ++blk) {
               const int ksteps = (cb == p.cblk[src] - 1 && p.ctail[src]) ? 2 : 4;
-              if (UPS) ptx::mbar_wait_cluster(ptx::smem_u32(&bars.fullA[sa]), pa);
+              if (UPS || FCW) ptx::mbar_wait_cluster(ptx::smem_u32(&bars.fullA[sa]), pa);
               else ptx::mbar_wait(ptx::smem_u32(&bars.fullA[sa]), pa);
               const uint64_t adesc = make_desc_sw128_sbo(smem_base + sa * p.a_bytes, static_cast<uint32_t>(p.P) * ROWB) +
                                      static_cast<uint64_t>(SUB_LO * 8 * (ROWB >> 4));
@@ -640,6 +650,113 @@
           }
       }
     }
+  } else if (FCW && warp >= 3 + EPI_WARPS) {
+    if constexpr (FCW) {
+      constexpr int P = 8 * MSUB + 2, RUN = 6, STRIPS = P / RUN, XR = RUN + 2;
+      static_assert(P % RUN == 0 && FC_XP == P + 2 && XR % 2 == 0, "first-conv window tiling");
+      constexpr int XPT = (FC_XP * FC_XP + 32 * FC_WARPS - 1) / (32 * FC_WARPS);
+      const int hw = warp - (3 + EPI_WARPS), ht = hw * 32 + lane;
+      float* xs = reinterpret_cast<float*>(reinterpret_cast<uint8_t*>(fs) + EPI_FUSED_BYTES);
+      auto image_of = [&](int tile, int& b, int& ty, int& tx) {
+        int mt, nt;
+        tile_to_mn<CG>(tile, p.n_ntiles, mt, nt);
+        b = mt / p.tiles_per_img;
+        const int t = mt - b * p.tiles_per_img;
+        ty = t / p.tiles_x;
+        tx = t - ty * p.tiles_x;
+      };
+      float xr[XPT];
+      auto load_patch = [&](int tile) {
+        int b, ty, tx;
+        image_of(tile, b, ty, tx);
+        const float* xi = p.fc_x + static_cast<size_t>(b / p.fc_dup) * IMG_PIX;
+#pragma unroll
+        for (int j = 0; j < XPT; ++j) {
+          const int e = ht + j * 32 * FC_WARPS, r = e / FC_XP, c = e - r * FC_XP;
+          if (e < FC_XP * FC_XP)
+            xr[j] = __ldg(xi + ((ty * 16 - 2 + r) & (IMG - 1)) * IMG + ((tx * 8 * MSUB - 2 + c) & (IMG - 1)));
+        }
+      };
+      auto helpers_sync = [&]() { asm volatile("bar.sync 5, %0;" ::"n"(32 * FC_WARPS) : "memory"); };
+      uint32_t sa = 0, pa = 0;
+      if (static_cast<int>(blockIdx.x) < n_tiles) load_patch(blockIdx.x);
+      for (int tile = blockIdx.x; tile < n_tiles; tile += gridDim.x) {
+        int b, ty, tx;
+        image_of(tile, b, ty, tx);
+        helpers_sync();
+#pragma unroll
+        for (int j = 0; j < XPT; ++j) {
+          const int e = ht + j * 32 * FC_WARPS;
+          if (e < FC_XP * FC_XP) xs[e] = xr[j];
+        }
+        helpers_sync();
+        if (tile + static_cast<int>(gridDim.x) < n_tiles) load_patch(tile + gridDim.x);
+        const float2* aff = p.fc_affine + static_cast<size_t>(b) * N;
+        for (int cb = 0; cb < p.cblk[0]; ++cb) {
+          const bool tail = cb == p.cblk[0] - 1 && p.ctail[0];
+          const int cp = tail ? (lane & 15) : lane;
+          const int ch = cb * KB + 2 * cp;
+          float2 w2[9];
+#pragma unroll
+          for (int k = 0; k < 9; ++k) w2[k] = make_float2(__ldg(p.fc_w9 + ch * 9 + k), __ldg(p.fc_w9 + (ch + 1) * 9 + k));
+          const float2 a0 = __ldg(aff + ch), a1 = __ldg(aff + ch + 1);
+          const float sc0 = 0.5f * a0.x, sc1 = 0.5f * a1.x, sh0 = 0.5f * a0.y, sh1 = 0.5f * a1.y;
+          ptx::mbar_wait_sleep(ptx::smem_u32(&bars.emptyA[sa]), pa ^ 1);
+          const uint32_t abase = smem_base + sa * p.a_bytes + ((cp & 3) << 2);
+          if (!(p.debug & 64)) {
+            const int nseg = tail ? 8 : 4, npass = tail ? 3 * nseg / 2 : 3 * nseg;
+            for (int ip = hw; ip < npass; ip += FC_WARPS) {
+              const int item = tail ? 2 * ip + (lane >> 4) : ip;
+              const int strip = item % STRIPS, seg = item / STRIPS;
+              const int c0 = strip * RUN, rb = seg * 18 / nseg, re = (seg + 1) * 18 / nseg;
+              auto load_row = [&](float (&v)[XR], int pr) {
+                const float2* src = reinterpret_cast<const float2*>(xs + pr * FC_XP + c0);
+#pragma unroll
+                for (int k = 0; k < XR / 2; ++k) { const float2 t = src[k]; v[2 * k] = t.x; v[2 * k + 1] = t.y; }
+              };
+              auto out_row = [&](const float (&A)[XR], const float (&Bv)[XR], float (&C)[XR], int r) {
+                load_row(C, r + 2);
+                float cx[RUN], cy[RUN];
+#pragma unroll
+                for (int j = 0; j < RUN; ++j) cx[j] = cy[j] = 0.f;
+#pragma unroll
+                for (int ky = 0; ky < 3; ++ky) {
+                  const float* xv = ky == 0 ? A : (ky == 1 ? Bv : C);
+#pragma unroll
+                  for (int kx = 0; kx < 3; ++kx)
+#pragma unroll
+                    for (int j = 0; j < RUN; ++j)
+                      fma2(cx[j], cy[j], w2[ky * 3 + kx].x, w2[ky * 3 + kx].y, xv[j + kx], xv[j + kx], cx[j], cy[j]);
+                }
+#pragma unroll
+                for (int j = 0; j < RUN; ++j) {
+                  float h0, h1, t0, t1, y0, y1;
+                  fma2(h0, h1, cx[j], cy[j], sc0, sc1, sh0, sh1);
+                  asm("tanh.approx.f32 %0, %1;" : "=f"(t0) : "f"(h0));
+                  asm("tanh.approx.f32 %0, %1;" : "=f"(t1) : "f"(h1));
+                  fma2(y0, y1, h0, h1, t0, t1, h0, h1);
+                  const uint32_t q = r * P + c0 + j;
+                  asm volatile("st.shared.b32 [%0], %1;" ::"r"(abase + q * ROWB + (((cp >> 2) ^ (q & 7)) << 4)),
+                               "r"(pack_bf16x2(y0, y1)) : "memory");
+                }
+              };
+              float X0[XR], X1[XR], X2[XR];
+              load_row(X0, rb);
+              load_row(X1, rb + 1);
+              for (int r = rb; r < re; r += 3) {
+                out_row(X0, X1, X2, r);
+                if (r + 1 < re) out_row(X1, X2, X0, r + 1);
+                if (r + 2 < re) out_row(X2, X0, X1, r + 2);
+              }
+            }
+          }
+          ptx::fence_proxy_async();
+          __syncwarp();
+          if (lane == 0) ptx::mbar_arrive_release_rank0(ptx::smem_u32(&bars.fullA[sa]));
+          if (++sa == static_cast<uint32_t>(p.a_stages)) { sa = 0; pa ^= 1; }
+        }
+      }
+    }
   } else if (warp >= 2 && warp < 2 + EPI_WARPS) {
     const int e = warp - 2, grp = e / GRP_WARPS, ew = e % GRP_WARPS, q = warp & 3, h = ew >> 2;
     const int row = q * 32 + lane;
@@ -1207,23 +1324,23 @@
   return (g.ksize == 3 && g.stride == 1 && !g.kx_in_n && epi != EPI_EPS && epi != EPI_PLAIN && g.H % 16 == 0) ? 1 : 0;
 }
 
-template <int N, int EPI, int MSUB, int CG, int GEO, int UPS = 0>
+template <int N, int EPI, int MSUB, int CG, int GEO, int SRC = SRC_TMA>
 static int set_smem_attr() {
   static bool attr_done = false;
   if (!attr_done) {
-    TCS_CUDA(cudaFuncSetAttribute(conv_tc_kernel<N, EPI, MSUB, CG, GEO, UPS>, cudaFuncAttributeMaxDynamicSharedMemorySize, static_cast<int>(TC_SMEM_MAX)));
+    TCS_CUDA(cudaFuncSetAttribute(conv_tc_kernel<N, EPI, MSUB, CG, GEO, SRC>, cudaFuncAttributeMaxDynamicSharedMemorySize, static_cast<int>(TC_SMEM_MAX)));
     attr_done = true;
   }
   return TCS_OK;
 }
 
-template <int N, int EPI, int MSUB, int CG, int GEO, int UPS = 0>
+template <int N, int EPI, int MSUB, int CG, int GEO, int SRC = SRC_TMA>
 static int max_ctas_t(const ConvTcPlan& pl, int* out) {
-  TCS_CHECK((set_smem_attr<N, EPI, MSUB, CG, GEO, UPS>()));
-  auto kern = conv_tc_kernel<N, EPI, MSUB, CG, GEO, UPS>;
+  TCS_CHECK((set_smem_attr<N, EPI, MSUB, CG, GEO, SRC>()));
+  auto kern = conv_tc_kernel<N, EPI, MSUB, CG, GEO, SRC>;
   if (CG == 2) {
     cudaLaunchConfig_t cfg{};
-    cfg.gridDim = dim3(2); cfg.blockDim = dim3(TC_THREADS + UPS_EXTRA_THREADS * UPS); cfg.dynamicSmemBytes = pl.smem; cfg.stream = nullptr;
+    cfg.gridDim = dim3(2); cfg.blockDim = dim3(src_threads(SRC)); cfg.dynamicSmemBytes = pl.smem; cfg.stream = nullptr;
     cudaLaunchAttribute at[1];
     at[0].id = cudaLaunchAttributeClusterDimension;
     at[0].val.clusterDim.x = 2; at[0].val.clusterDim.y = 1; at[0].val.clusterDim.z = 1;
@@ -1233,7 +1350,7 @@
     *out = 2 * nclusters;
   } else {
     int per_sm = 0, dev = 0, sms = 0;
-    TCS_CUDA(cudaOccupancyMaxActiveBlocksPerMultiprocessor(&per_sm, kern, TC_THREADS, pl.smem));
+    TCS_CUDA(cudaOccupancyMaxActiveBlocksPerMultiprocessor(&per_sm, kern, src_threads(SRC), pl.smem));
     TCS_CUDA(cudaGetDevice(&dev));
     TCS_CUDA(cudaDeviceGetAttribute(&sms, cudaDevAttrMultiProcessorCount, dev));
     *out = per_sm * sms;
@@ -1241,14 +1358,14 @@
   return TCS_OK;
 }
 
-template <int N, int EPI, int MSUB, int CG, int GEO, int UPS = 0>
+template <int N, int EPI, int MSUB, int CG, int GEO, int SRC = SRC_TMA>
 static int launch_t(const ConvTcPlan& pl, cudaStream_t st) {
-  auto kern = conv_tc_kernel<N, EPI, MSUB, CG, GEO, UPS>;
-  TCS_CHECK((set_smem_attr<N, EPI, MSUB, CG, GEO, UPS>()));
+  auto kern = conv_tc_kernel<N, EPI, MSUB, CG, GEO, SRC>;
+  TCS_CHECK((set_smem_attr<N, EPI, MSUB, CG, GEO, SRC>()));
   if (EPI == EPI_GN_FUSED)
     TCS_CUDA(cudaMemsetAsync(pl.p.epi.partials, 0, sizeof(unsigned long long) * 16 * pl.p.n_mtiles, st));
   cudaLaunchConfig_t cfg{};
-  cfg.gridDim = dim3(pl.grid); cfg.blockDim = dim3(TC_THREADS + UPS_EXTRA_THREADS * UPS); cfg.dynamicSmemBytes = pl.smem; cfg.stream = st;
+  cfg.gridDim = dim3(pl.grid); cfg.blockDim = dim3(src_threads(SRC)); cfg.dynamicSmemBytes = pl.smem; cfg.stream = st;
   cudaLaunchAttribute at[2];
   int na = 0;
   if (EPI == EPI_GN_FUSED && (CG == 1 || pl.coop_cluster)) {
@@ -1274,9 +1391,10 @@
     else return max_ctas_t<NN, EE, MM, 1, 0>(pl, out);                                  \
   }
 #define TCS_TC_GEO1(NN, EE, MM)                                                        \
-  if (pl.geo == 1 && pl.cg == 2 && !pl.ups && pl.N == NN && pl.epi == EE && pl.msub == MM) return max_ctas_t<NN, EE, MM, 2, 1>(pl, out);
-  if (pl.geo == 1 && pl.cg == 2 && pl.ups && pl.epi == EPI_PADDED && pl.N == 96 && pl.msub == 2) return max_ctas_t<96, EPI_PADDED, 2, 2, 1, 1>(pl, out);
-  if (pl.geo == 1 && pl.cg == 2 && pl.ups && pl.epi == EPI_PADDED && pl.N == 192 && pl.msub == 1) return max_ctas_t<192, EPI_PADDED, 1, 2, 1, 1>(pl, out);
+  if (pl.geo == 1 && pl.cg == 2 && !pl.ups && !pl.fc && pl.N == NN && pl.epi == EE && pl.msub == MM) return max_ctas_t<NN, EE, MM, 2, 1>(pl, out);
+  if (pl.geo == 1 && pl.cg == 2 && pl.ups && pl.epi == EPI_PADDED && pl.N == 96 && pl.msub == 2) return max_ctas_t<96, EPI_PADDED, 2, 2, 1, SRC_UPSAMPLE>(pl, out);
+  if (pl.geo == 1 && pl.cg == 2 && pl.ups && pl.epi == EPI_PADDED && pl.N == 192 && pl.msub == 1) return max_ctas_t<192, EPI_PADDED, 1, 2, 1, SRC_UPSAMPLE>(pl, out);
+  if (pl.geo == 1 && pl.cg == 2 && pl.fc && pl.epi == EPI_GN_FUSED && pl.N == 96 && pl.msub == 2) return max_ctas_t<96, EPI_GN_FUSED, 2, 2, 1, SRC_FIRSTCONV>(pl, out);
   TCS_TC_CASE(96, EPI_RAW_STATS, 2)
   TCS_TC_CASE(96, EPI_PADDED, 2)
   TCS_TC_CASE(96, EPI_PLAIN, 2)
@@ -1305,9 +1423,10 @@
     else return launch_t<NN, EE, MM, 1, 0>(pl, st);                                     \
   }
 #define TCS_TC_GEO1(NN, EE, MM)                                                        \
-  if (pl.geo == 1 && pl.cg == 2 && !pl.ups && pl.N == NN && pl.epi == EE && pl.msub == MM) return launch_t<NN, EE, MM, 2, 1>(pl, st);
-  if (pl.geo == 1 && pl.cg == 2 && pl.ups && pl.epi == EPI_PADDED && pl.N == 96 && pl.msub == 2) return launch_t<96, EPI_PADDED, 2, 2, 1, 1>(pl, st);
-  if (pl.geo == 1 && pl.cg == 2 && pl.ups && pl.epi == EPI_PADDED && pl.N == 192 && pl.msub == 1) return launch_t<192, EPI_PADDED, 1, 2, 1, 1>(pl, st);
+  if (pl.geo == 1 && pl.cg == 2 && !pl.ups && !pl.fc && pl.N == NN && pl.epi == EE && pl.msub == MM) return launch_t<NN, EE, MM, 2, 1>(pl, st);
+  if (pl.geo == 1 && pl.cg == 2 && pl.ups && pl.epi == EPI_PADDED && pl.N == 96 && pl.msub == 2) return launch_t<96, EPI_PADDED, 2, 2, 1, SRC_UPSAMPLE>(pl, st);
+  if (pl.geo == 1 && pl.cg == 2 && pl.ups && pl.epi == EPI_PADDED && pl.N == 192 && pl.msub == 1) return launch_t<192, EPI_PADDED, 1, 2, 1, SRC_UPSAMPLE>(pl, st);
+  if (pl.geo == 1 && pl.cg == 2 && pl.fc && pl.epi == EPI_GN_FUSED && pl.N == 96 && pl.msub == 2) return launch_t<96, EPI_GN_FUSED, 2, 2, 1, SRC_FIRSTCONV>(pl, st);
   TCS_TC_CASE(96, EPI_RAW_STATS, 2)
   TCS_TC_CASE(96, EPI_PADDED, 2)
   TCS_TC_CASE(96, EPI_PLAIN, 2)
@@ -1381,6 +1500,10 @@
   p.a_load_bytes = 0;
   p.ups = p.l_stages = 0;
   p.l_bytes = p.l_load_bytes = 0;
+  p.fc = 0;
+  p.fc_x = p.fc_w9 = nullptr;
+  p.fc_affine = nullptr;
+  p.fc_dup = 1;
   if (pl.geo) {
     if (g.W % (8 * pl.msub) || g.H % 16) return fail(TCS_ERR_UNSUPPORTED, "conv_tc: image is not a multiple of the 16 x 8 tile");
     const int NB = pl.N / pl.cg;
@@ -1398,8 +1521,10 @@
       p.l_load_bytes = 10u * static_cast<uint32_t>(p.P / 2 + 1) * ROWB;
       p.l_bytes = (p.l_load_bytes + 1023u) & ~1023u;
     }
+    if (g.first_conv) p.fc = pl.fc = 1;
     const size_t slab_bytes = g.ups ? EPI_SLAB_BYTES / SLAB_BUFS : EPI_SLAB_BYTES;
-    const size_t budget1 = TC_SMEM_MAX - 1024 - slab_bytes - bias_bytes_of(g.ntot) - EPI_FUSED_BYTES -
+    const size_t fc_bytes = g.first_conv ? FC_PATCH_BYTES : 0;
+    const size_t budget1 = TC_SMEM_MAX - 1024 - slab_bytes - bias_bytes_of(g.ntot) - EPI_FUSED_BYTES - fc_bytes -
                            static_cast<size_t>(p.l_stages) * p.l_bytes;
     const bool want3 = getenv("TCS_UPS_A_STAGES") ? atoi(getenv("TCS_UPS_A_STAGES")) == 3 : pl.msub == 2;
     if (g.ups && want3 && budget1 >= 3 * static_cast<size_t>(p.a_bytes) + 2 * static_cast<size_t>(3u * NB * ROWB))
@@ -1411,11 +1536,15 @@
     p.nstage = static_cast<int>(rest / p.stage_bytes);
     if (p.nstage > MAX_STAGES) p.nstage = MAX_STAGES;
     if (getenv("TCS_NSTAGE") && atoi(getenv("TCS_NSTAGE")) < p.nstage) p.nstage = atoi(getenv("TCS_NSTAGE"));
-    if (getenv("TCS_PLAN_LOG")) fprintf(stderr, "[conv_tc plan] H=%d N=%d K=%d ups=%d tb=%d nstage=%d stage_bytes=%u a_bytes=%u l_bytes=%u\n", g.H, pl.N, p.kstages, p.ups, p.tb, p.nstage, p.stage_bytes, p.a_bytes, p.l_bytes);
+    if (getenv("TCS_PLAN_LOG")) fprintf(stderr, "[conv_tc plan] H=%d N=%d K=%d ups=%d fc=%d tb=%d nstage=%d stage_bytes=%u a_bytes=%u l_bytes=%u\n", g.H, pl.N, p.kstages, p.ups, p.fc, p.tb, p.nstage, p.stage_bytes, p.a_bytes, p.l_bytes);
     if (p.nstage < 2) return fail(TCS_ERR_UNSUPPORTED, "conv_tc: weight stage does not fit shared memory twice");
     pl.smem = static_cast<size_t>(p.a_stages) * p.a_bytes + static_cast<size_t>(p.l_stages) * p.l_bytes +
-              static_cast<size_t>(p.nstage) * p.stage_bytes + 1024 + slab_bytes + bias_bytes_of(g.ntot) + EPI_FUSED_BYTES;
-  }
+              static_cast<size_t>(p.nstage) * p.stage_bytes + 1024 + slab_bytes + bias_bytes_of(g.ntot) + EPI_FUSED_BYTES +
+              fc_bytes;
+  }
+  if (g.first_conv && !(pl.geo == 1 && pl.cg == 2 && pl.msub == 2 && epi == EPI_GN_FUSED && g.nsrc == 1 && !g.split3 &&
+                        !g.ups && g.H == IMG && g.W == IMG && g.csrc[0] == 96 && g.ntot == 96))
+    return fail(TCS_ERR_UNSUPPORTED, "conv_tc: first-conv windows are built for down1.net.3 (64x64, 96 -> 96, fused GroupNorm) only");
   if (g.ups && !(pl.geo == 1 && pl.cg == 2 && epi == EPI_PADDED && g.nsrc == 1 && !g.split3))
     return fail(TCS_ERR_UNSUPPORTED, "conv_tc: the fused upsample needs a 3x3 stride-1 layer with one padded bf16 source and a padded output");
   p.epi = ea;
diff --git a/vae-diffusion-toy-crystals_b200/csrc/conv_tc.cuh b/vae-diffusion-toy-crystals_b200/csrc/conv_tc.cuh
--- a/vae-diffusion-toy-crystals_b200/csrc/conv_tc.cuh
+++ b/vae-diffusion-toy-crystals_b200/csrc/conv_tc.cuh
@@ -34,6 +34,11 @@
   int ups;
   int l_stages;
   uint32_t l_bytes, l_load_bytes;
+  int fc;
+  const float* fc_x;
+  const float* fc_w9;
+  const float2* fc_affine;
+  int fc_dup;
   int debug;
   EpiArgs epi;
 };
@@ -45,6 +50,7 @@
   CUtensorMap mapO1;
   int geo = 0;
   int ups = 0;
+  int fc = 0;
   ConvTcParams p;
   int N;
   int epi;
diff --git a/vae-diffusion-toy-crystals_b200/csrc/kernels.cuh b/vae-diffusion-toy-crystals_b200/csrc/kernels.cuh
--- a/vae-diffusion-toy-crystals_b200/csrc/kernels.cuh
+++ b/vae-diffusion-toy-crystals_b200/csrc/kernels.cuh
@@ -24,10 +24,11 @@
                       const int* step_ptr, int trow_off, const float* cvec, int n, int dup, float* raw,
                       float* partials, cudaStream_t st);
 constexpr int FIRST_CONV_SLOTS = 32;
+int launch_first_conv_affine(const float* x, const float* w9, const float* tvec, int tvec_stride, const int* step_ptr,
+                             int trow_off, const float* cvec, int n, int dup, const float* gamma, const float* beta,
+                             float2* affine, cudaStream_t st);
 template <typename T>
-int launch_first_conv_gn(const float* x, const float* w9, const float* tvec, int tvec_stride, const int* step_ptr,
-                         int trow_off, const float* cvec, int n, int dup, const float* gamma, const float* beta, T* out,
-                         cudaStream_t st);
+int launch_first_conv_gn(const float* x, const float* w9, const float2* affine, int n, int dup, T* out, cudaStream_t st);
 
 template <typename T>
 int launch_gn_apply(const void* in, int in_padded, const float* partials, int slots, const float* gamma,
diff --git a/vae-diffusion-toy-crystals_b200/csrc/kernels_simt.cu b/vae-diffusion-toy-crystals_b200/csrc/kernels_simt.cu
--- a/vae-diffusion-toy-crystals_b200/csrc/kernels_simt.cu
+++ b/vae-diffusion-toy-crystals_b200/csrc/kernels_simt.cu
@@ -110,29 +110,25 @@
   *reinterpret_cast<__nv_bfloat162*>(p) = __floats2bfloat162_rn(a, b);
 }
 
-constexpr int FC_SPLIT = 2;
-template <typename T>
-__global__ void __launch_bounds__(384, 2) first_conv_gn_kernel(const float* __restrict__ x, const float* __restrict__ w9,
-                                                           const float* __restrict__ tvec, int tvec_stride,
-                                                           const int* __restrict__ step_ptr, int trow_off,
-                                                           const float* __restrict__ cvec, int dup,
-                                                           const float* __restrict__ gamma, const float* __restrict__ beta,
-                                                           T* __restrict__ out) {
-  constexpr bool FAST = sizeof(T) == 2;
+__global__ void __launch_bounds__(384) first_conv_affine_kernel(const float* __restrict__ x, const float* __restrict__ w9,
+                                                                const float* __restrict__ tvec, int tvec_stride,
+                                                                const int* __restrict__ step_ptr, int trow_off,
+                                                                const float* __restrict__ cvec, int dup,
+                                                                const float* __restrict__ gamma,
+                                                                const float* __restrict__ beta, float2* __restrict__ affine) {
   constexpr int P = IMG + 4;
-  __shared__ float2 xs[P][P];
+  __shared__ float xs[P][P];
   __shared__ double racc[12][14];
   __shared__ double R[5][5];
   __shared__ double S1;
   __shared__ double csum[96][2][2];
   __shared__ float s_mean[2][GN_GROUPS], s_rstd[2][GN_GROUPS];
-  const int i = blockIdx.x / FC_SPLIT, band = blockIdx.x % FC_SPLIT;
-  const int t = threadIdx.x, op = t % 48, pg = t / 48, oc = 2 * op;
+  const int i = blockIdx.x;
+  const int t = threadIdx.x;
   const int warp = t >> 5, lane = t & 31;
   for (int e = t; e < P * P; e += 384) {
     const int r = e / P, c = e - r * P;
-    const float xval = x[(static_cast<size_t>(i) * IMG + ((r - 2 + IMG) & (IMG - 1))) * IMG + ((c - 2 + IMG) & (IMG - 1))];
-    xs[r][c] = make_float2(xval, xval);
+    xs[r][c] = x[(static_cast<size_t>(i) * IMG + ((r - 2 + IMG) & (IMG - 1))) * IMG + ((c - 2 + IMG) & (IMG - 1))];
   }
   __syncthreads();
   {
@@ -141,12 +137,12 @@
     for (int k = 0; k < 14; ++k) acc[k] = 0.0;
     for (int p = t; p < IMG_PIX; p += 384) {
       const int yy = (p >> 6) + 2, xx = (p & 63) + 2;
-      const double x0 = xs[yy][xx].x;
+      const double x0 = xs[yy][xx];
       acc[13] += x0;
 #pragma unroll
       for (int k = 0; k < 13; ++k) {
         const int dy = (k + 2) / 5, dx = (k + 2) % 5 - 2;
-        acc[k] += x0 * static_cast<double>(xs[yy + dy][xx + dx].x);
+        acc[k] += x0 * static_cast<double>(xs[yy + dy][xx + dx]);
       }
     }
 #pragma unroll
@@ -195,26 +191,52 @@
     s_mean[u][g] = static_cast<float>(mean);
     s_rstd[u][g] = static_cast<float>(1.0 / sqrt(var + static_cast<double>(GN_EPS)));
   }
+  __syncthreads();
+  if (t < 96 * dup) {
+    const int c = t % 96, u = t / 96, g = c / 12;
+    const size_t b = static_cast<size_t>(i) * dup + u;
+    const float bias = tvec[static_cast<size_t>(trow) * 96 + c] + cvec[b * 96 + c];
+    const float sc = s_rstd[u][g] * gamma[c];
+    const float sh = (bias - s_mean[u][g]) * sc + beta[c];
+    affine[b * 96 + c] = make_float2(sc, sh);
+  }
+}
+
+int launch_first_conv_affine(const float* x, const float* w9, const float* tvec, int tvec_stride, const int* step_ptr,
+                             int trow_off, const float* cvec, int n, int dup, const float* gamma, const float* beta,
+                             float2* affine, cudaStream_t st) {
+  if (n <= 0) return TCS_OK;
+  first_conv_affine_kernel<<<n, 384, 0, st>>>(x, w9, tvec, tvec_stride, step_ptr, trow_off, cvec, dup, gamma, beta, affine);
+  TCS_CUDA(cudaGetLastError());
+  return TCS_OK;
+}
+
+constexpr int FC_SPLIT = 2;
+template <typename T>
+__global__ void __launch_bounds__(384, 2) first_conv_gn_kernel(const float* __restrict__ x, const float* __restrict__ w9,
+                                                           const float2* __restrict__ affine, int dup,
+                                                           T* __restrict__ out) {
+  constexpr bool FAST = sizeof(T) == 2;
+  constexpr int P = IMG + 4;
+  __shared__ float2 xs[P][P];
+  const int i = blockIdx.x / FC_SPLIT, band = blockIdx.x % FC_SPLIT;
+  const int t = threadIdx.x, op = t % 48, pg = t / 48, oc = 2 * op;
+  for (int e = t; e < P * P; e += 384) {
+    const int r = e / P, c = e - r * P;
+    const float xval = x[(static_cast<size_t>(i) * IMG + ((r - 2 + IMG) & (IMG - 1))) * IMG + ((c - 2 + IMG) & (IMG - 1))];
+    xs[r][c] = make_float2(xval, xval);
+  }
   float w0[9], w1[9];
 #pragma unroll
   for (int k = 0; k < 9; ++k) { w0[k] = w9[oc * 9 + k]; w1[k] = w9[(oc + 1) * 9 + k]; }
-  float b0[2], b1[2];
+  float sc0[2], sh0[2], sc1[2], sh1[2];
+#pragma unroll
   for (int u = 0; u < 2; ++u) {
-    const int uu = u < dup ? u : 0;
-    b0[u] = tvec[static_cast<size_t>(trow) * 96 + oc] + cvec[(static_cast<size_t>(i) * dup + uu) * 96 + oc];
-    b1[u] = tvec[static_cast<size_t>(trow) * 96 + oc + 1] + cvec[(static_cast<size_t>(i) * dup + uu) * 96 + oc + 1];
-  }
-  __syncthreads();
-  const int g = op / 6;
-  float sc0[2], sh0[2], sc1[2], sh1[2];
-  {
-    const float ga0 = gamma[oc], ga1 = gamma[oc + 1], be0 = beta[oc], be1 = beta[oc + 1];
-#pragma unroll
-    for (int u = 0; u < 2; ++u) {
-      sc0[u] = s_rstd[u][g] * ga0; sh0[u] = (b0[u] - s_mean[u][g]) * sc0[u] + be0;
-      sc1[u] = s_rstd[u][g] * ga1; sh1[u] = (b1[u] - s_mean[u][g]) * sc1[u] + be1;
-    }
-  }
+    const size_t b = static_cast<size_t>(i) * dup + (u < dup ? u : 0);
+    const float2 a0 = affine[b * 96 + oc], a1 = affine[b * 96 + oc + 1];
+    sc0[u] = a0.x; sh0[u] = a0.y; sc1[u] = a1.x; sh1[u] = a1.y;
+  }
+  __syncthreads();
   constexpr int PO = IMG + 2;
   const int p_begin = band * (IMG_PIX / FC_SPLIT), p_end = p_begin + IMG_PIX / FC_SPLIT;
   (void)p_end;
@@ -310,17 +332,14 @@
 }
 
 template <typename T>
-int launch_first_conv_gn(const float* x, const float* w9, const float* tvec, int tvec_stride, const int* step_ptr,
-                         int trow_off, const float* cvec, int n, int dup, const float* gamma, const float* beta, T* out,
-                         cudaStream_t st) {
+int launch_first_conv_gn(const float* x, const float* w9, const float2* affine, int n, int dup, T* out, cudaStream_t st) {
   if (n <= 0) return TCS_OK;
-  first_conv_gn_kernel<T><<<n * FC_SPLIT, 384, 0, st>>>(x, w9, tvec, tvec_stride, step_ptr, trow_off, cvec, dup, gamma,
-                                                        beta, out);
-  TCS_CUDA(cudaGetLastError());
-  return TCS_OK;
-}
-template int launch_first_conv_gn<float>(const float*, const float*, const float*, int, const int*, int, const float*, int, int, const float*, const float*, float*, cudaStream_t);
-template int launch_first_conv_gn<__nv_bfloat16>(const float*, const float*, const float*, int, const int*, int, const float*, int, int, const float*, const float*, __nv_bfloat16*, cudaStream_t);
+  first_conv_gn_kernel<T><<<n * FC_SPLIT, 384, 0, st>>>(x, w9, affine, dup, out);
+  TCS_CUDA(cudaGetLastError());
+  return TCS_OK;
+}
+template int launch_first_conv_gn<float>(const float*, const float*, const float2*, int, int, float*, cudaStream_t);
+template int launch_first_conv_gn<__nv_bfloat16>(const float*, const float*, const float2*, int, int, __nv_bfloat16*, cudaStream_t);
 
 __global__ void __launch_bounds__(256) gn_finalize_kernel(const float* __restrict__ partials, int slots, double count,
                                                          float2* __restrict__ stats) {
diff --git a/vae-diffusion-toy-crystals_b200/csrc/tcs_api.cu b/vae-diffusion-toy-crystals_b200/csrc/tcs_api.cu
--- a/vae-diffusion-toy-crystals_b200/csrc/tcs_api.cu
+++ b/vae-diffusion-toy-crystals_b200/csrc/tcs_api.cu
@@ -95,6 +95,8 @@
   DevBuf attn_wpack;
   bool fuse_ups = false;
   ConvTcPlan plan_us[2];
+  bool first_in_window = false;
+  ConvTcPlan plan_fc;
   bool split3 = false;
   size_t esz = 4;
   cudaStream_t stream = nullptr;
@@ -114,6 +116,7 @@
 
   int chunk = 0;
   DevBuf raw64, raw32, raw16, partials, gnstats;
+  DevBuf fc_affine;
   DevBuf p64_h1, p64_a, p64_b;
   DevBuf p32_96a, p32_96b, p32_192a, p32_192h2, p32_192b;
   DevBuf p16_a, p16_b, p16_c, qkv, atty;
@@ -201,6 +204,7 @@
   TCS_CHECK(h->raw16.ensure(MB * 256 * 192 * 4));
   TCS_CHECK(h->partials.ensure(MB * 128 * 16 * 4));
   TCS_CHECK(h->gnstats.ensure(MB * 8 * 8));
+  TCS_CHECK(h->fc_affine.ensure(MB * 96 * sizeof(float2)));
   const size_t P64 = MB * 66 * 66 * 96 * e, P32a = MB * 34 * 34 * 96 * e, P32b = MB * 34 * 34 * 192 * e,
                P16 = MB * 18 * 18 * 192 * e;
   TCS_CHECK(h->p64_h1.ensure(P64)); TCS_CHECK(h->p64_a.ensure(P64)); TCS_CHECK(h->p64_b.ensure(P64));
@@ -333,6 +337,23 @@
       TCS_CHECK(rc);
     }
   }
+  if (h->first_in_window) {
+    const ConvWiring w = wiring(h, C_D1B);
+    ConvGeom g = geom_of(C_D1B, h->chunk, w.in_pad);
+    g.first_conv = 1;
+    EpiArgs ea{};
+    ea.bias = h->dw.at(std::string(kConv[C_D1B].key) + ".bias");
+    ea.out = w.out; ea.partials = h->partials.as<float>(); ea.residual = nullptr; ea.ldo = w.ldo;
+    ea.slots = slots_of(h, C_D1B);
+    ea.overflow = h->status.as<int>();
+    ea.gamma = h->dw.at(std::string(w.gn) + ".weight");
+    ea.beta = h->dw.at(std::string(w.gn) + ".bias");
+    const int rc = conv_tc_make_plan(&h->plan_fc, g, w.s0, nullptr, h->wpack[C_D1B].as<__nv_bfloat16>(), EPI_GN_FUSED, ea, h->sm_count);
+    if (rc == TCS_ERR_UNSUPPORTED) h->first_in_window = false;
+    else TCS_CHECK(rc);
+    h->plan_fc.p.fc_w9 = h->d_w9;
+    h->plan_fc.p.fc_affine = h->fc_affine.as<float2>();
+  }
   for (int id = 0; id < C_COUNT; ++id) {
     if (!h->plan[id].coop_cluster) continue;
     ConvTcPlan pl = h->plan[id];
@@ -349,6 +370,7 @@
       break;
     }
   }
+  h->plan_fc.coop_cluster = h->plan[C_D1B].coop_cluster;
   TCS_CUDA(cudaMemsetAsync(h->status.p, 0, 4, h->stream));
   return TCS_OK;
 }
@@ -430,20 +452,41 @@
 #define GN(key, raw, slots, res, C, out) \
   { h->launches += 2; TCS_CHECK(launch_gn_apply<T>(raw, 0, part, slots, gnw(key), gnb(key), B, res, res, C, 1, out, h->gnstats.as<float2>(), st)); }
 
-  if (h->fuse_first && !(tap && tap->id == 0)) {
+  const bool first_in_window = h->first_in_window && sizeof(T) == 2 && !(tap && tap->id <= 1);
+  if (first_in_window || (h->fuse_first && !(tap && tap->id == 0))) {
     ++h->launches;
-    TCS_CHECK(launch_first_conv_gn<T>(a.x, h->d_w9, a.tvec, a.tvec_stride, a.step_ptr, a.trow_off, a.cvec, a.ns, a.dup,
-                                      gnw("down1.net.1"), gnb("down1.net.1"), h->p64_a.as<T>(), st));
+    TCS_CHECK(launch_first_conv_affine(a.x, h->d_w9, a.tvec, a.tvec_stride, a.step_ptr, a.trow_off, a.cvec, a.ns, a.dup,
+                                       gnw("down1.net.1"), gnb("down1.net.1"), h->fc_affine.as<float2>(), st));
+  }
+  if (first_in_window) {
+    tap_idx += 2;
+    if (tap && tap->id == tap_idx) return fail(TCS_ERR_UNSUPPORTED, "raw conv output does not exist when GroupNorm is fused");
     ++tap_idx;
+    ++h->launches;
+    ConvTcPlan pl = h->plan_fc;
+    pl.p.n_mtiles = B * pl.p.tiles_per_img;
+    pl.p.fc_x = a.x;
+    pl.p.fc_dup = a.dup;
+    pl.grid = conv_tc_grid(pl, B, h->sm_count);
+    if (h->profiling) TCS_CUDA(cudaEventRecord(h->prof_ev[2 * C_D1B], st));
+    TCS_CHECK(conv_tc_launch(pl, st));
+    if (h->profiling) TCS_CUDA(cudaEventRecord(h->prof_ev[2 * C_D1B + 1], st));
+    TAP(1, wiring(h, C_D1B).act, 64, 64, 96);
   } else {
-    ++h->launches;
-    TCS_CHECK(launch_first_conv(a.x, h->d_w9, a.tvec, a.tvec_stride, a.step_ptr, a.trow_off, a.cvec, a.ns, a.dup,
-                                h->raw64.as<float>(), part, st));
-    TAP(0, h->raw64.p, 64, 64, 96);
-    GN("down1.net.1", h->raw64.p, FIRST_CONV_SLOTS, 64, 96, h->p64_a.as<T>());
-  }
-  TAP(1, h->p64_a.p, 64, 64, 96);
-  CONV_GN(C_D1B, h->raw64.p, 64, 96);
+    if (h->fuse_first && !(tap && tap->id == 0)) {
+      ++h->launches;
+      TCS_CHECK(launch_first_conv_gn<T>(a.x, h->d_w9, h->fc_affine.as<float2>(), a.ns, a.dup, h->p64_a.as<T>(), st));
+      ++tap_idx;
+    } else {
+      ++h->launches;
+      TCS_CHECK(launch_first_conv(a.x, h->d_w9, a.tvec, a.tvec_stride, a.step_ptr, a.trow_off, a.cvec, a.ns, a.dup,
+                                  h->raw64.as<float>(), part, st));
+      TAP(0, h->raw64.p, 64, 64, 96);
+      GN("down1.net.1", h->raw64.p, FIRST_CONV_SLOTS, 64, 96, h->p64_a.as<T>());
+    }
+    TAP(1, h->p64_a.p, 64, 64, 96);
+    CONV_GN(C_D1B, h->raw64.p, 64, 96);
+  }
   TCS_CHECK(run_conv<T>(h, C_DS1, B, st));
   TAP(1, h->p32_96a.p, 32, 32, 96);
   CONV_GN(C_D2A, h->raw32.p, 32, 192);
@@ -590,9 +633,10 @@
   const size_t E64 = padded_elems(h, 64, 96), E32a = padded_elems(h, 32, 96), E32b = padded_elems(h, 32, 192),
                E16 = padded_elems(h, 16, 192);
   if (!(tap && tap->id == 0)) {
-    ++h->launches;
-    TCS_CHECK(launch_first_conv_gn<float>(a.x, h->d_w9, a.tvec, a.tvec_stride, a.step_ptr, a.trow_off, a.cvec, a.ns, a.dup,
-                                          gnw("down1.net.1"), gnb("down1.net.1"), h->p64_a.as<float>(), st));
+    h->launches += 2;
+    TCS_CHECK(launch_first_conv_affine(a.x, h->d_w9, a.tvec, a.tvec_stride, a.step_ptr, a.trow_off, a.cvec, a.ns, a.dup,
+                                       gnw("down1.net.1"), gnb("down1.net.1"), h->fc_affine.as<float2>(), st));
+    TCS_CHECK(launch_first_conv_gn<float>(a.x, h->d_w9, h->fc_affine.as<float2>(), a.ns, a.dup, h->p64_a.as<float>(), st));
     ++tap_idx;
   } else {
     ++h->launches;
@@ -822,6 +866,8 @@
     const char* e = getenv("TCS_FUSE_GN");
     h->fuse_gn = h->use_tc && !h->split3 && cfg->fuse_gn != 0 && !(e && atoi(e) == 0);
     h->fuse_first = !(e && atoi(e) == 0);
+    const char* ef = getenv("TCS_FIRST_IN_WINDOW");
+    h->first_in_window = h->fuse_gn && !(ef && atoi(ef) == 0);
     const char* eu = getenv("TCS_FUSE_UPS");
     h->fuse_ups = h->use_tc && !h->split3 && !(eu && atoi(eu) == 0);
     const char* ea = getenv("TCS_FUSE_ATTN");
@@ -1428,6 +1474,20 @@
   g.ups = 1;
   return debug_conv_t<__nv_bfloat16>(true, g, in_lowres, nullptr, weight, bias, out, nullptr, EPI_PADDED,
                                      static_cast<cudaStream_t>(stream));
+}
+
+int tcs_debug_first_conv_affine(int32_t n, int32_t dup, const float* x, const float* w9, const float* bias,
+                                const float* gamma, const float* beta, float* affine, void* stream) {
+  if (n < 1 || (dup != 1 && dup != 2) || !x || !w9 || !bias || !gamma || !beta || !affine)
+    return fail(TCS_ERR_BAD_ARGUMENT, "tcs_debug_first_conv_affine: bad argument");
+  cudaStream_t st = static_cast<cudaStream_t>(stream);
+  DevBuf zero;
+  TCS_CHECK(zero.ensure(96 * sizeof(float)));
+  TCS_CUDA(cudaMemsetAsync(zero.p, 0, 96 * sizeof(float), st));
+  TCS_CHECK(launch_first_conv_affine(x, w9, zero.as<float>(), 0, nullptr, 0, bias, n, dup, gamma, beta,
+                                     reinterpret_cast<float2*>(affine), st));
+  TCS_CUDA(cudaStreamSynchronize(st));
+  return TCS_OK;
 }
 
 int64_t tcs_debug_attn_pack(const float* qkv_w, const float* proj_w, uint8_t* out, int64_t capacity) {
diff --git a/vae-diffusion-toy-crystals_b200/toycrystals_b200/_cabi.py b/vae-diffusion-toy-crystals_b200/toycrystals_b200/_cabi.py
--- a/vae-diffusion-toy-crystals_b200/toycrystals_b200/_cabi.py
+++ b/vae-diffusion-toy-crystals_b200/toycrystals_b200/_cabi.py
@@ -101,6 +101,7 @@
     "tcs_debug_attn_block": (C.c_int, [C.c_int32] + [C.c_void_p] * 10),
     "tcs_debug_conv_ups": (C.c_int, [C.c_int32] * 5 + [C.c_void_p] * 5),
     "tcs_debug_attn_pack": (C.c_int64, [C.c_void_p, C.c_void_p, C.c_void_p, C.c_int64]),
+    "tcs_debug_first_conv_affine": (C.c_int, [C.c_int32] * 2 + [C.c_void_p] * 7),
 }
 
 _lib: Optional[C.CDLL] = None
```

After: 233.5, median of 6. 0.98x the previous value.
